# illini-robomaster/irmv_detection

Hardware: AMD Instinct MI355X
Metric: end-to-end FPS (preprocess→NMS→PnP) 640×640 YOLOv8n, 1/2/4/8 MI355X (higher is better)
Workload: dtype f16

## Files before the change

### include/irmv_hip.h

```cpp
#ifndef IRMV_HIP_H
#define IRMV_HIP_H

#include <stddef.h>
#include <stdint.h>

#ifdef __cplusplus
extern "C" {
#endif

#define IRMV_OK 0
#define IRMV_ERR_ARG (-1)
#define IRMV_ERR_HIP (-2)
#define IRMV_ERR_MODEL (-3)

#define IRMV_RESIZE_STRETCH 0
#define IRMV_RESIZE_LETTERBOX 1

#define IRMV_ARMOR_SMALL 0
#define IRMV_ARMOR_LARGE 1

#define IRMV_POINTS_AUTO 0
#define IRMV_POINTS_KEYPOINT_HEAD 1
#define IRMV_POINTS_CLASSICAL 2

// ... 100 lines not shown
int irmv_engine_num_streams(const irmv_engine *e);
int irmv_engine_sync_launch(const irmv_engine *e);

int irmv_engine_numa_node(const irmv_engine *e);
int irmv_engine_numa_placed(const irmv_engine *e);
int irmv_numa_device_node(int device, int *node);
int irmv_numa_bind_thread(int node);
int irmv_numa_page_node(const void *p);
int irmv_numa_parse_cpulist(const char *s, int *cpus, int cap);

uint8_t *irmv_engine_src_buffer(irmv_engine *e, int slot);
void *irmv_engine_src_device_buffer(irmv_engine *e, int slot);
int irmv_engine_set_window(irmv_engine *e, int slot, int x0, int y0);
int irmv_engine_get_window(const irmv_engine *e, int slot, int *x0, int *y0, int *w, int *h);
typedef struct irmv_window_map_t {
    int32_t bx0, by0;
    uint64_t band_offset;
    uint64_t band_bytes;
    double cx, cy;
    int32_t reserved[4];
} irmv_window_map_t;
int irmv_window_map(const irmv_engine_cfg *cfg, int x0, int y0, irmv_window_map_t *out);

int irmv_engine_src_format(const irmv_engine *e);
size_t irmv_engine_src_bytes(const irmv_engine *e);

#define IRMV_SUBMIT_H2D 1u
#define IRMV_SUBMIT_ASYNC_UPLOAD 2u

int irmv_engine_submit(irmv_engine *e, int first_slot, int count, uint32_t flags);
int irmv_engine_wait(irmv_engine *e);
int irmv_engine_wait_upload(irmv_engine *e, int first_slot, int count);
int irmv_engine_wait_slots(irmv_engine *e, int first_slot, int count);
int irmv_engine_results(irmv_engine *e, int slot, irmv_det *out, int cap, int *n);
int irmv_engine_detect(irmv_engine *e, int slot, irmv_det *out, int cap, int *n);
double irmv_engine_last_detect_ms(const irmv_engine *e);

int irmv_engine_rotated_image(irmv_engine *e, int slot, uint8_t *dst_hwc);

int irmv_engine_set_bayer_isp(irmv_engine *e, const uint16_t gain_q8[3], const uint8_t *lut);
int irmv_engine_get_bayer_isp(const irmv_engine *e, uint16_t gain_q8[3], uint8_t *lut);

int irmv_engine_extract_armors(irmv_engine *e, int slot, const float *xyxy, int n, irmv_det *out);
int irmv_engine_set_extract_params(irmv_engine *e, int binary_threshold, float light_min_ratio, float light_max_ratio,
                                   float light_max_angle, const double center_distances[4]);
int irmv_engine_point_source(const irmv_engine *e);

int irmv_engine_read_input(irmv_engine *e, int slot, float *chw);
int irmv_engine_read_head(irmv_engine *e, int slot, float *head);
int irmv_engine_write_head(irmv_engine *e, int slot, const float *head);
int irmv_engine_run_post(irmv_engine *e, int first_slot, int count);
int irmv_engine_debug_poke_candidate_counts(irmv_engine *e, int value);
int irmv_engine_debug_read_cand_bits(irmv_engine *e, int slot, uint32_t *words, int cap, int *n, int *sparse);
int irmv_engine_debug_read_head_rows(irmv_engine *e, int slot, float *rec, size_t bytes);
int irmv_engine_debug_read_head_raw(irmv_engine *e, int slot, float *head);
int irmv_engine_read_tap(irmv_engine *e, int slot, const char *name, float *nhwc, int shape[3]);
int irmv_engine_read_raw(irmv_engine *e, int slot, irmv_raw_dets *out);
int irmv_engine_num_anchors(const irmv_engine *e);
int irmv_engine_head_channels(const irmv_engine *e);
int irmv_engine_net_dims(const irmv_engine *e, int *width, int *height);

typedef struct irmv_conv_seg {
    char tensor[32];
    int32_t coff, C, shift;
} irmv_conv_seg;

typedef struct irmv_conv_op {
    int32_t op;
    char layer[32];
    int32_t ks, stride, act, out_f32, cin, cout, cout_pad;
    int32_t Hin, Win, Hout, Wout;
    irmv_conv_seg s0, s1;
    irmv_conv_seg res;
    char out_tensor[32];
    int32_t out_coff;
    int32_t out_lazy;
    int32_t fused;
    int32_t tune_fused;
    char fuse_layer[32];
    char fuse_tensor[32];
    int32_t fuse_coff, fuse_cout, fuse_cout_pad;
    int32_t reserved;
    char kname[48], kname_one[48];
} irmv_conv_op;

typedef struct irmv_conv_cand {
    char name[48];
    int32_t mt, nt, flags, ipw;
    int32_t forced, reserved;
} irmv_conv_cand;

#define IRMV_DECLINED 1

int irmv_engine_conv_ops(irmv_engine *e, irmv_conv_op *ops, int cap, int *n);
int irmv_engine_conv_candidates(irmv_engine *e, int op, int tune_count, irmv_conv_cand *cands, int cap, int *n);
#define IRMV_RUN_POISON 1u
#define IRMV_RUN_POISON_ONLY 2u
int irmv_engine_run_conv_candidate(irmv_engine *e, int op, int tune_count, int cand, int first_slot, int count, uint32_t flags);
int irmv_engine_read_tensor(irmv_engine *e, const char *name, int first_slot, int count, void *dst, size_t bytes);

typedef struct irmv_graph_op {
    int32_t op;
    char kind[16];
    char layer[48];
    char kname[48];
    irmv_conv_seg s0, s1;
// ... 81 lines not shown
```

### irmv_detection_amd/_build.py

```python
from __future__ import annotations

import os
import shutil
import subprocess

_HERE = os.path.dirname(os.path.abspath(__file__))
CSRC = os.path.join(_HERE, "csrc")
LIB_DIR = os.path.join(_HERE, "lib")
LIB_PATH = os.path.join(LIB_DIR, "libirmv_hip.so")
INCLUDE = os.path.join(os.path.dirname(_HERE), "include")

SOURCES = [
    ("k_pre.hip", []),
    ("k_bayer.hip", []),
    ("k_window.hip", []),
    ("k_front.hip", []),
    ("k_c2f.hip", []),
    ("k_bneck.hip", []),
    ("k_kpt.hip", []),
    ("k_conv.hip", []),
    ("k_post.hip", ["-ffp-contract=off"]),
    ("k_light.hip", ["-ffp-contract=off"]),
    ("k_shuffle.hip", []),
    ("k_debug.hip", []),
    ("engine.cpp", ["-x", "hip"]),
    ("engine_graph.cpp", ["-x", "hip"]),
    ("engine_tune.cpp", ["-x", "hip"]),
    ("engine_plan.cpp", ["-x", "hip"]),
    ("engine_step.cpp", ["-x", "hip"]),
    ("engine_hooks.cpp", ["-x", "hip"]),
]
COMMON = ["-O3", "-std=c++17", "-fPIC", "--offload-arch=gfx950", "-Wall", "-Wno-unused-function",
          "-mllvm", "-amdgpu-mfma-vgpr-form", "-I", INCLUDE]


def source_hash() -> str:
    import hashlib
    h = hashlib.sha256()
    names = sorted(set([s for s, _ in SOURCES] + ["irmv_common.hpp", "pnp_device.hpp", "numa.hpp", "engine_internal.hpp"]))
    for n in names:
        pth = os.path.join(CSRC, n)
        if os.path.exists(pth):
            h.update(n.encode() + b"\0" + open(pth, "rb").read())
    h.update(open(os.path.join(INCLUDE, "irmv_hip.h"), "rb").read())
    h.update(" ".join(COMMON[:-2]).encode())
    for src, extra in SOURCES:
        h.update((src + " " + " ".join(extra)).encode())
    return h.hexdigest()


def hipcc() -> str:
    for cand in (shutil.which("hipcc"), "/opt/rocm/bin/hipcc"):
        if cand and os.path.exists(cand):
            return cand
    raise RuntimeError("hipcc not found: the HIP extension cannot be built")


def _stale(target: str, deps) -> bool:
    if not os.path.exists(target):
        return True
    t = os.path.getmtime(target)
    return any(os.path.getmtime(d) > t for d in deps)


COMM_PATH = os.path.join(LIB_DIR, "libirmv_comm.so")


def build_comm(force: bool = False, verbose: bool = False) -> str:
    os.makedirs(LIB_DIR, exist_ok=True)
    src = os.path.join(CSRC, "comm.cpp")
    deps = [src, os.path.join(INCLUDE, "irmv_comm.h"), os.path.join(INCLUDE, "irmv_hip.h"), __file__]
    if force or _stale(COMM_PATH, deps):
        rocm_lib = os.path.join(os.path.dirname(os.path.dirname(os.path.realpath(hipcc()))), "lib")
        cmd = [hipcc(), "-O2", "-std=c++17", "-fPIC", "-shared", "-Wall", "-I", INCLUDE, src, "-o", COMM_PATH,
               "-L", rocm_lib, "-lrccl", "-Wl,-rpath," + rocm_lib]
        if verbose:
            print(" ".join(cmd))
        subprocess.check_call(cmd)
    return COMM_PATH


def build(force: bool = False, verbose: bool = False) -> str:
    os.makedirs(LIB_DIR, exist_ok=True)
    headers = [os.path.join(CSRC, "irmv_common.hpp"), os.path.join(CSRC, "pnp_device.hpp"), os.path.join(CSRC, "numa.hpp"), os.path.join(CSRC, "engine_internal.hpp"), os.path.join(INCLUDE, "irmv_hip.h"), __file__]
    objs = []
    cc = hipcc()
    for src, extra in SOURCES:
        sp = os.path.join(CSRC, src)
        obj = os.path.join(LIB_DIR, os.path.splitext(src)[0] + ".o")
        if force or _stale(obj, [sp] + headers):
            cmd = [cc] + COMMON + extra + os.environ.get("IRMV_EXTRA_HIPCC_FLAGS", "").split() + ["-c", sp, "-o", obj]
            if verbose:
                print(" ".join(cmd))
            subprocess.check_call(cmd)
        objs.append(obj)
    if force or _stale(LIB_PATH, objs):
        cmd = [cc, "-shared", "-fPIC", "--offload-arch=gfx950", "-o", LIB_PATH] + objs
        if verbose:
            print(" ".join(cmd))
        subprocess.check_call(cmd)
    return LIB_PATH


if __name__ == "__main__":
    print(build(force=False, verbose=True))
    print(build_comm(force=False, verbose=True))
```

### irmv_detection_amd/capi.py

```python
from __future__ import annotations

import ctypes as C
import os

from . import _build

OK, ERR_ARG, ERR_HIP, ERR_MODEL = 0, -1, -2, -3
RESIZE_STRETCH, RESIZE_LETTERBOX = 0, 1
ARMOR_SMALL, ARMOR_LARGE = 0, 1
SUBMIT_H2D = 1
SUBMIT_ASYNC_UPLOAD = 2
POINTS_AUTO, POINTS_KEYPOINT_HEAD, POINTS_CLASSICAL = 0, 1, 2
SRC_HWC8, SRC_BAYER_RGGB8, SRC_BAYER_BGGR8, SRC_BAYER_GRBG8, SRC_BAYER_GBRG8 = 0, 1, 2, 3, 4
BAYER_FORMATS = {"RGGB": SRC_BAYER_RGGB8, "BGGR": SRC_BAYER_BGGR8, "GRBG": SRC_BAYER_GRBG8, "GBRG": SRC_BAYER_GBRG8}
DEMOSAIC_BILINEAR, DEMOSAIC_MHC = 0, 1
DEMOSAIC_ALGOS = {"bilinear": DEMOSAIC_BILINEAR, "mhc": DEMOSAIC_MHC}
NUM_CLASSES = 14
MAX_DET_CAP = 256
CAND_CAP = 8192


class IrmvError(RuntimeError):
    def __init__(self, code: int, msg: str):
        super().__init__(f"irmv_hip error {code}: {msg}")
# ... 107 lines not shown


DECLINED = 1
RUN_POISON, RUN_POISON_ONLY = 1, 2


_P = C.c_void_p
SYMBOLS = [
    ("irmv_last_error", C.c_char_p, []),
    ("irmv_version", C.c_char_p, []),
    ("irmv_device_count", C.c_int, [C.POINTER(C.c_int)]),
    ("irmv_device_synchronize", C.c_int, [C.c_int]),
    ("irmv_engine_cfg_default", None, [C.POINTER(EngineCfg)]),
    ("irmv_engine_create", C.c_int, [C.POINTER(EngineCfg), C.POINTER(_P)]),
    ("irmv_engine_destroy", None, [_P]),
    ("irmv_engine_num_slots", C.c_int, [_P]),
    ("irmv_engine_max_det", C.c_int, [_P]),
    ("irmv_engine_num_streams", C.c_int, [_P]),
    ("irmv_engine_sync_launch", C.c_int, [_P]),
    ("irmv_engine_numa_node", C.c_int, [_P]),
    ("irmv_engine_numa_placed", C.c_int, [_P]),
    ("irmv_numa_device_node", C.c_int, [C.c_int, C.POINTER(C.c_int)]),
    ("irmv_numa_bind_thread", C.c_int, [C.c_int]),
    ("irmv_numa_page_node", C.c_int, [C.c_void_p]),
    ("irmv_numa_parse_cpulist", C.c_int, [C.c_char_p, C.POINTER(C.c_int), C.c_int]),
    ("irmv_engine_src_buffer", C.POINTER(C.c_uint8), [_P, C.c_int]),
    ("irmv_engine_src_device_buffer", C.c_void_p, [_P, C.c_int]),
    ("irmv_engine_set_window", C.c_int, [_P, C.c_int, C.c_int, C.c_int]),
    ("irmv_engine_get_window", C.c_int, [_P, C.c_int, C.POINTER(C.c_int), C.POINTER(C.c_int), C.POINTER(C.c_int), C.POINTER(C.c_int)]),
    ("irmv_window_map", C.c_int, [C.POINTER(EngineCfg), C.c_int, C.c_int, C.POINTER(WindowMap)]),
    ("irmv_engine_src_format", C.c_int, [_P]),
    ("irmv_engine_src_bytes", C.c_size_t, [_P]),
    ("irmv_engine_submit", C.c_int, [_P, C.c_int, C.c_int, C.c_uint32]),
    ("irmv_engine_wait", C.c_int, [_P]),
    ("irmv_engine_wait_slots", C.c_int, [_P, C.c_int, C.c_int]),
    ("irmv_engine_wait_upload", C.c_int, [_P, C.c_int, C.c_int]),
    ("irmv_engine_set_extract_params", C.c_int, [_P, C.c_int, C.c_float, C.c_float, C.c_float, C.POINTER(C.c_double)]),
    ("irmv_engine_point_source", C.c_int, [_P]),
    ("irmv_engine_results", C.c_int, [_P, C.c_int, C.POINTER(Det), C.c_int, C.POINTER(C.c_int)]),
    ("irmv_engine_detect", C.c_int, [_P, C.c_int, C.POINTER(Det), C.c_int, C.POINTER(C.c_int)]),
    ("irmv_engine_last_detect_ms", C.c_double, [_P]),
    ("irmv_engine_rotated_image", C.c_int, [_P, C.c_int, C.POINTER(C.c_uint8)]),
    ("irmv_engine_extract_armors", C.c_int, [_P, C.c_int, C.POINTER(C.c_float), C.c_int, C.POINTER(Det)]),
    ("irmv_engine_set_bayer_isp", C.c_int, [_P, C.POINTER(C.c_uint16), C.POINTER(C.c_uint8)]),
    ("irmv_engine_get_bayer_isp", C.c_int, [_P, C.POINTER(C.c_uint16), C.POINTER(C.c_uint8)]),
    ("irmv_engine_light_trace", C.c_int, [_P, C.c_int, C.POINTER(C.c_float), C.c_int, C.POINTER(LightTrace), C.POINTER(Det)]),
    ("irmv_light_limits", C.c_int, [C.POINTER(C.c_int32)]),
    ("irmv_engine_read_input", C.c_int, [_P, C.c_int, C.POINTER(C.c_float)]),
    ("irmv_engine_read_head", C.c_int, [_P, C.c_int, C.POINTER(C.c_float)]),
    ("irmv_engine_write_head", C.c_int, [_P, C.c_int, C.POINTER(C.c_float)]),
    ("irmv_engine_run_post", C.c_int, [_P, C.c_int, C.c_int]),
    ("irmv_engine_debug_poke_candidate_counts", C.c_int, [_P, C.c_int]),
    ("irmv_engine_debug_read_cand_bits", C.c_int, [_P, C.c_int, C.POINTER(C.c_uint32), C.c_int, C.POINTER(C.c_int), C.POINTER(C.c_int)]),
    ("irmv_engine_debug_read_head_rows", C.c_int, [_P, C.c_int, C.POINTER(C.c_float), C.c_size_t]),
    ("irmv_engine_debug_read_head_raw", C.c_int, [_P, C.c_int, C.POINTER(C.c_float)]),
    ("irmv_engine_read_tap", C.c_int, [_P, C.c_int, C.c_char_p, C.POINTER(C.c_float), C.POINTER(C.c_int)]),
    ("irmv_engine_read_raw", C.c_int, [_P, C.c_int, C.POINTER(RawDets)]),
    ("irmv_engine_num_anchors", C.c_int, [_P]),
    ("irmv_engine_head_channels", C.c_int, [_P]),
    ("irmv_engine_net_dims", C.c_int, [_P, C.POINTER(C.c_int), C.POINTER(C.c_int)]),
    ("irmv_engine_conv_ops", C.c_int, [_P, C.POINTER(ConvOp), C.c_int, C.POINTER(C.c_int)]),
    ("irmv_engine_conv_candidates", C.c_int, [_P, C.c_int, C.c_int, C.POINTER(ConvCand), C.c_int, C.POINTER(C.c_int)]),
    ("irmv_engine_run_conv_candidate", C.c_int, [_P, C.c_int, C.c_int, C.c_int, C.c_int, C.c_int, C.c_uint32]),
    ("irmv_engine_read_tensor", C.c_int, [_P, C.c_char_p, C.c_int, C.c_int, C.c_void_p, C.c_size_t]),
    ("irmv_engine_ops", C.c_int, [_P, C.POINTER(GraphOp), C.c_int, C.POINTER(C.c_int)]),
    ("irmv_engine_run_op", C.c_int, [_P, C.c_int, C.c_int, C.c_int, C.c_uint32]),
    ("irmv_sppf_slab", C.c_int, [C.c_int, C.c_int, C.c_int, C.c_int]),
    ("irmv_front_plan", C.c_int, [C.POINTER(EngineCfg), C.POINTER(FrontPlan)]),
    ("irmv_engine_profile", C.c_int, [_P, C.c_int, C.c_int, C.POINTER(KernelStat), C.c_int, C.POINTER(C.c_int)]),
    ("irmv_debug_lds_fill", C.c_int, [C.c_uint32]),
    ("irmv_debug_lds_probe", C.c_int, [C.c_uint32, C.c_uint32, C.POINTER(C.c_uint32), C.c_int, C.POINTER(C.c_int)]),
    ("irmv_pnp_create", C.c_int, [C.c_int, C.POINTER(C.c_double), C.POINTER(C.c_double), C.POINTER(_P)]),
    ("irmv_pnp_destroy", None, [_P]),
    ("irmv_pnp_solve", C.c_int, [_P, C.POINTER(C.c_float), C.c_int, C.c_int, C.POINTER(C.c_double),
                                 C.POINTER(C.c_double), C.POINTER(C.c_int32)]),
]

_lib = None


def lib_path() -> str:
    return os.environ.get("IRMV_LIB_PATH") or _build.LIB_PATH


def load():
    global _lib
    if _lib is None:
        path = lib_path()
        if not os.path.exists(path):
            raise IrmvError(ERR_HIP, f"{path} is missing: build the HIP extension first "
                                     "(python -m irmv_detection_amd._build); there is no CPU fallback")
        L = C.CDLL(path)
        for name, res, args in SYMBOLS:
            if os.environ.get("IRMV_LIB_PATH") and not hasattr(L, name):
                continue
            fn = getattr(L, name)
            fn.restype = res
            fn.argtypes = args
        _lib = L
    return _lib


def check(rc: int, allow=()):
    if rc != OK and rc not in allow:
        raise IrmvError(rc, load().irmv_last_error().decode(errors="replace"))
    return rc
# ... 80 lines not shown
```

### irmv_detection_amd/csrc/engine.cpp

```cpp
#include "engine_internal.hpp"

static thread_local std::string g_err;
int irmv::fail(int code, const std::string &msg) { g_err = msg; return code; }

extern "C" const char *irmv_last_error(void) { return g_err.c_str(); }
extern "C" const char *irmv_version(void)
{
    static char buf[96];
    static std::once_flag once;
    std::call_once(once, [] {
        int v = 0;
        if (hipRuntimeGetVersion(&v) != hipSuccess) v = 0;
        snprintf(buf, sizeof buf, "irmv_hip 0.3 (gfx950; HIP runtime %d)", v);
    });
    return buf;
}
extern "C" int irmv_device_synchronize(int device)
{
    HIP_TRY(hipSetDevice(device));
    HIP_TRY(hipDeviceSynchronize());
    return IRMV_OK;
}
extern "C" int irmv_device_count(int *count)
{
// ... 168 lines not shown
    cfg->src_width = 1280;
    cfg->src_height = 1024;
    cfg->net_size = 640;
    cfg->resize_mode = IRMV_RESIZE_STRETCH;
    cfg->rotate180 = 1;
    cfg->swap_rb = 0;
    cfg->score_thr = 0.25f;
    cfg->iou_thr = 0.45f;
    cfg->max_det = 100;
    cfg->pre_nms_cap = 4096;
    cfg->num_slots = 3;
    cfg->armor_size = IRMV_ARMOR_SMALL;
    const double K[9] = {957.669211, 0, 345.943891, 0, 969.127115, 284.057302, 0, 0, 1};
    const double D[5] = {-0.405274, 0.126058, -0.026939, -0.006503, 0.0};
    memcpy(cfg->camera_matrix, K, sizeof K);
    memcpy(cfg->dist_coeffs, D, sizeof D);
    cfg->point_source = IRMV_POINTS_AUTO;
    cfg->binary_threshold = 150;
    cfg->light_min_ratio = 0.1f; cfg->light_max_ratio = 0.4f; cfg->light_max_angle = 40.0f;
    cfg->armor_min_small_center_distance = 0.8; cfg->armor_max_small_center_distance = 3.2;
    cfg->armor_min_large_center_distance = 3.2; cfg->armor_max_large_center_distance = 5.5;
    cfg->src_format = IRMV_SRC_HWC8;
    cfg->bayer_gain_q8[0] = cfg->bayer_gain_q8[1] = cfg->bayer_gain_q8[2] = 256;
}

static EngineSwitches read_switches()
{
    auto set = [](const char *name) { return getenv(name) != nullptr; };
    auto starts = [](const char *name, char c) { const char *v = getenv(name); return v && v[0] == c; };
    auto off = [&](const char *name) { return starts(name, '0'); };
    auto is1 = [&](const char *name) { return starts(name, '1'); };
    EngineSwitches s;
    TuneSwitches &t = s.tune;
    t.untuned = off("IRMV_AUTOTUNE"); t.verbose = set("IRMV_AUTOTUNE_VERBOSE"); t.warn = set("IRMV_TUNE_WARN");
    const char *s2 = getenv("IRMV_FORCE_S2"), *wres = getenv("IRMV_FORCE_WRES");
    t.has_s2 = s2 != nullptr; t.force_s2 = s2 ? s2 : "";
    t.has_wres = wres != nullptr; t.force_wres = wres ? wres : "";
    t.force_pw = set("IRMV_FORCE_PW"); t.force_pwn = set("IRMV_FORCE_PWN"); t.force_cm = set("IRMV_FORCE_CM");
    t.force_w8 = set("IRMV_FORCE_W8"); t.force_nt8 = set("IRMV_FORCE_NT8"); t.force_pf4 = set("IRMV_FORCE_PF4");
    t.no_pw = set("IRMV_NO_PW"); t.no_pwn = set("IRMV_NO_PWN"); t.no_pf2 = set("IRMV_NO_PF2"); t.no_pf4 = set("IRMV_NO_PF4");
    t.no_cm = set("IRMV_NO_CM"); t.no_w8 = set("IRMV_NO_W8"); t.no_nt8 = set("IRMV_NO_NT8"); t.no_wres = set("IRMV_NO_WRES");
    t.no_deep = is1("IRMV_NO_DEEP");
    s.front.fastx = !off("IRMV_FRONT_FASTX"); s.front.direct = !off("IRMV_FRONT_DIRECT"); s.front.tall = !off("IRMV_FRONT_TILE8");
    s.fused_front = !off("IRMV_FUSED_FRONT"); s.fused_c2f = !off("IRMV_FUSED_C2F"); s.bneck64 = !off("IRMV_BNECK64"); s.kpt3 = !off("IRMV_KPT3");
    s.fused_head = !off("IRMV_FUSED_HEAD");
    s.merge_head0 = off("IRMV_MERGE_HEAD0") ? 0 : (is1("IRMV_MERGE_HEAD0") ? 1 : -1);
    s.group_head = !off("IRMV_GROUP_HEAD"); s.group_verbose = set("IRMV_GROUP_VERBOSE"); s.group_force = set("IRMV_GROUP_FORCE");
    if (const char *ns = getenv("IRMV_STREAMS")) { s.has_streams = true; s.streams = atoi(ns); }
    s.numa = !off("IRMV_NUMA");
    s.inline_copies = is1("IRMV_INLINE_COPIES"); s.graph_upload = !off("IRMV_GRAPH_UPLOAD"); s.window_upload = !off("IRMV_WINDOW_UPLOAD");
    if (const char *uk = getenv("IRMV_UPLOAD_KERNEL")) s.upload_kernel_blocks = atoi(uk);
    s.sync_launch = starts("IRMV_SYNC_LAUNCH", 'e') ? 1 : (starts("IRMV_SYNC_LAUNCH", 'g') ? 0 : -1);
    s.split_scan = !off("IRMV_SPLIT_SCAN"); s.emit_scan = !off("IRMV_EMIT_SCAN");
    s.sparse_head = !off("IRMV_SPARSE_HEAD"); s.sparse_branch = !off("IRMV_SPARSE_BRANCH");
    s.zero_copy_results = !off("IRMV_ZERO_COPY_RESULTS"); s.post_keys_only = is1("IRMV_POST_KEYS_ONLY");
    s.nms_classwalk = !off("IRMV_NMS_CLASSWALK");
    s.nms_prefilter = off("IRMV_NMS_PREFILTER") ? 0 : 1;
    if (const char *pe = getenv("IRMV_NMS_PRE")) { int hi = 0, lo = 0; if (sscanf(pe, "%d,%d", &hi, &lo) == 2 && hi >= 64 && hi <= 512 && lo >= 32 && lo < hi) s.nms_prefilter = hi | (lo << 16); }
    if (const char *st = getenv("IRMV_NMS_STAMPS")) { s.nms_stamps = true; s.nms_stamps_slots = atoi(st); }
    return s;
}

constexpr size_t kCfgSizeV1 = offsetof(irmv_engine_cfg, src_format);
constexpr size_t kCfgSizeV2 = offsetof(irmv_engine_cfg, reserved2);
static_assert(offsetof(irmv_engine_cfg, net_height) < kCfgSizeV2 && kCfgSizeV2 < sizeof(irmv_engine_cfg), "three distinct cfg sizes");
static_assert(offsetof(irmv_engine_cfg, win_width) == offsetof(irmv_engine_cfg, reserved2) + 4 && offsetof(irmv_engine_cfg, win_height) + 2 == sizeof(irmv_engine_cfg),
              "win_width / win_height fill the tail of irmv_engine_cfg");

static irmv_engine_cfg window_view(const irmv_engine_cfg &c)
{
    irmv_engine_cfg v = c;
    if (c.win_width > 0 && c.win_height > 0) { v.src_width = c.win_width; v.src_height = c.win_height; }
    v.win_width = v.win_height = 0;
    return v;
}

static int resolve_cfg(const irmv_engine_cfg *cfg_in, irmv_engine_cfg *full)
{
    const size_t sz = cfg_in->struct_size;
    if (sz != sizeof(irmv_engine_cfg) && sz != kCfgSizeV1 && sz != kCfgSizeV2) return fail(IRMV_ERR_ARG, "irmv_engine_cfg size mismatch");
    if (sz != sizeof(irmv_engine_cfg)) {
        irmv_engine_cfg_default(full);
        memcpy(full, cfg_in, sz == kCfgSizeV1 ? kCfgSizeV1 : offsetof(irmv_engine_cfg, net_height));
        full->struct_size = sizeof *full;
        full->bayer_demosaic = IRMV_DEMOSAIC_BILINEAR;
    } else {
        *full = *cfg_in;
    }
    const irmv_engine_cfg *cfg = full;
    if (cfg->src_format < IRMV_SRC_HWC8 || cfg->src_format > IRMV_SRC_BAYER_GBRG8) return fail(IRMV_ERR_ARG, "unknown src_format (IRMV_SRC_*)");
    if (cfg->bayer_demosaic > IRMV_DEMOSAIC_MHC) return fail(IRMV_ERR_ARG, "unknown bayer_demosaic (IRMV_DEMOSAIC_*)");
    if (cfg->bayer_demosaic == IRMV_DEMOSAIC_MHC) {
        if (cfg->src_format == IRMV_SRC_HWC8) return fail(IRMV_ERR_ARG, "bayer_demosaic = IRMV_DEMOSAIC_MHC needs a Bayer src_format (IRMV_SRC_BAYER_*8)");
        if (cfg->src_width < 4 || cfg->src_height < 4) return fail(IRMV_ERR_ARG, "bayer_demosaic = IRMV_DEMOSAIC_MHC needs src_width >= 4 and src_height >= 4 (reflect-101 at radius 2)");
    }
    if (cfg->src_format != IRMV_SRC_HWC8) {
        if (cfg->src_width % 2 || cfg->src_height % 2) return fail(IRMV_ERR_ARG, "a Bayer src_format (IRMV_SRC_BAYER_*8) needs an even src_width and src_height");
        for (int i = 0; i < 3; i++)
            if (cfg->bayer_gain_q8[i] > 1023) return fail(IRMV_ERR_ARG, "bayer_gain_q8 must be in [0, 1023] (Q8, 256 = 1.0)");
    }
    if (cfg->net_size < 64 || cfg->net_size % 32 != 0 || cfg->net_size > 2048) return fail(IRMV_ERR_ARG, "net_size must be a multiple of 32 in [64, 2048]");
    if (cfg->net_height != 0 && (cfg->net_height < 64 || cfg->net_height % 32 != 0 || cfg->net_height > 2048))
        return fail(IRMV_ERR_ARG, "net_height must be 0 (square) or a multiple of 32 in [64, 2048]");
    if (cfg->src_width < 2 || cfg->src_height < 2 || cfg->src_width > 4096) return fail(IRMV_ERR_ARG, "src size out of range (width <= 4096)");
    if ((uint64_t)cfg->src_width * (uint64_t)cfg->src_height * 3u > IRMV_MAX_FRAME_BYTES)
        return fail(IRMV_ERR_ARG, "src frame too large: 3 * src_width * src_height must not exceed 4294967296 bytes (32-bit byte offsets into a frame)");
    if (cfg->win_width < 0 || cfg->win_width > cfg->src_width) return fail(IRMV_ERR_ARG, "win_width must be 0 (no window) or in [1, src_width]");
// ... 319 lines not shown
```

### irmv_detection_amd/csrc/engine_graph.cpp

```cpp
#include "engine_internal.hpp"

#pragma pack(push, 1)
struct BlobHeader { char magic[4]; uint32_t version, nc, nk, reg_max, n_layers, dtype, reserved; };
struct BlobLayer { char name[32]; uint32_t cin, cout, k, stride, act, pad; uint64_t w_off, b_off; };
#pragma pack(pop)

static uint16_t float_to_half_bits(float f)
{
    uint32_t x;
    memcpy(&x, &f, 4);
    const uint32_t sign = (x >> 16) & 0x8000u;
    x &= 0x7fffffffu;
    if (x >= 0x7f800000u) return (uint16_t)(sign | 0x7c00u | ((x > 0x7f800000u) ? 0x200u : 0u));
    if (x >= 0x477ff000u) return (uint16_t)(sign | 0x7c00u);
    if (x < 0x33000001u) return (uint16_t)sign;
    if (x < 0x38800000u) {
        const int shift = 126 - (int)(x >> 23);
        const uint32_t man = (x & 0x7fffffu) | 0x800000u;
        uint32_t h = man >> shift;
        const uint32_t rem = man & ((1u << shift) - 1u), half = 1u << (shift - 1);
        if (rem > half || (rem == half && (h & 1u))) h++;
        return (uint16_t)(sign | h);
    }
    uint32_t h = ((x >> 23) - 112u) << 10 | ((x >> 13) & 0x3ffu);
// ... 614 lines not shown
            m.cin = PC[i]; m.cout = cm; m.k = 3; m.stride = 1; m.act = 1;
            m.w = e->merged_w.back().data(); m.b = e->merged_b.back().data();
            e->layers.push_back(m);
            TRY(new_tensor(e, "22.s0." + std::to_string(i), PH[i], PW[i], cm, false, &t_s0[i]));
            TRY(add_conv(e, m.name, SegRef{P[i], 0, PC[i], 0}, SegRef{}, PH[i], PW[i], t_s0[i], 0));
            Op &mo = e->ops.back();
            const double real = nbr == 3 ? 144.0 : 128.0;
            mo.flops *= real / cm;
            mo.level = i;
        }
    }
    for (int b = 0; b < nbr; b++)
        for (int i = 0; i < 3; i++) {
            const std::string pre = std::string("model.22.") + br[b] + "." + std::to_string(i);
            const std::string tn = std::string("22.") + br[b] + "." + std::to_string(i);
            int t1 = -1, t2;
            TRY(new_tensor(e, tn + ".1", PH[i], PW[i], mid[b], false, &t2));
            if (e->merge_head0) {
                TRY(add_conv(e, pre + ".1", SegRef{t_s0[i], coff0[b], mid[b], 0}, SegRef{}, PH[i], PW[i], t2, 0));
            } else {
                TRY(new_tensor(e, tn + ".0", PH[i], PW[i], mid[b], false, &t1));
                TRY(add_conv(e, pre + ".0", SegRef{P[i], 0, PC[i], 0}, SegRef{}, PH[i], PW[i], t1, 0));
                TRY(add_conv(e, pre + ".1", SegRef{t1, 0, mid[b], 0}, SegRef{}, PH[i], PW[i], t2, 0));
            }
            TRY(add_conv(e, pre + ".2", SegRef{t2, 0, mid[b], 0}, SegRef{}, PH[i], PW[i], e->head_t[i], off[b]));
            for (size_t k = e->ops.size() - (e->merge_head0 ? 2 : 3); k < e->ops.size(); k++) e->ops[k].level = i;
            {
                const int i1 = (int)e->ops.size() - 2, i2 = i1 + 1;
                const Op &o1 = e->ops[i1], &o2 = e->ops[i2];
                if (e->sw.fused_head && o1.cout == 64 && o1.cin % 32 == 0 && o1.pair && o1.res_t < 0 && o1.cfg.stride == 1 &&
                    o2.cin == 64 && o2.ksteps == 2 && o2.cfg.ks == 1 && o2.cfg.out_f32 && o2.cfg.act == 0 && (o2.cout_pad == 16 || o2.cout_pad == 64))
                    e->ops[i1].fuse_next = i2;
                if (e->sw.fused_head && o1.cfg.cin16 && o1.cout_pad == 16 && !o1.pair && o1.res_t < 0 && o1.cfg.stride == 1 && o1.cfg.act == 1 && o2.w_k16)
                    e->ops[i1].fuse_next = i2;
            }
            if (b == 2 && !e->merge_head0) TRY(fuse_kpt3(e, i));
        }
    return IRMV_OK;
}

static int build_post_stage(irmv_engine *e)
{
    const irmv_engine_cfg &c = e->cfg;
    const int net_w = c.net_size, net_h = c.net_height, S = c.num_slots;
    const int px = e->front.box[0], py = e->front.box[2], nw = e->front.box[1] - px, nh = e->front.box[3] - py;
    TRY(dev_alloc(e, (void **)&e->boxes, (size_t)S * e->A * 16));
    TRY(dev_alloc(e, (void **)&e->keys, (size_t)S * e->A * e->nc * 8));
    if (e->sw.split_scan) {
        TRY(dev_alloc(e, (void **)&e->cand_counts, (size_t)S * sizeof(int)));
        HIP_TRY(hipMemset(e->cand_counts, 0, (size_t)S * sizeof(int)));
        e->cand_words = (e->A + 31) / 32;
        TRY(dev_alloc(e, (void **)&e->cand_bits, (size_t)S * e->cand_words * sizeof(unsigned int)));
        HIP_TRY(hipMemset(e->cand_bits, 0, (size_t)S * e->cand_words * sizeof(unsigned int)));
    }
    e->head_stale.assign((size_t)S, 0);
    e->branch_stale.assign((size_t)S, 0);
    TRY(dev_alloc(e, (void **)&e->dets_dev, (size_t)S * c.max_det * sizeof(DevDet)));
    TRY(dev_alloc(e, (void **)&e->fout_dev, (size_t)S * sizeof(DevFrameOut)));
    HIP_TRY(hipMemset(e->dets_dev, 0, (size_t)S * c.max_det * sizeof(DevDet)));
    HIP_TRY(hipMemset(e->fout_dev, 0, (size_t)S * sizeof(DevFrameOut)));
    HIP_TRY(hipHostMalloc((void **)&e->dets_host, (size_t)S * c.max_det * sizeof(DevDet), hipHostMallocMapped | hipHostMallocCoherent));
    HIP_TRY(hipHostMalloc((void **)&e->fout_host, (size_t)S * sizeof(DevFrameOut), hipHostMallocMapped | hipHostMallocCoherent));
    HIP_TRY(hipHostGetDevicePointer((void **)&e->dets_host_dev, e->dets_host, 0));
    HIP_TRY(hipHostGetDevicePointer((void **)&e->fout_host_dev, e->fout_host, 0));
    log_range(e, "pinned dets_host", e->dets_host, (size_t)S * c.max_det * sizeof(DevDet));
    log_range(e, "pinned fout_host", e->fout_host, (size_t)S * sizeof(DevFrameOut));
    memset(e->dets_host, 0, (size_t)S * c.max_det * sizeof(DevDet));
    memset(e->fout_host, 0, (size_t)S * sizeof(DevFrameOut));
    if (e->sw.split_scan) {
        Op op; op.kind = OP_SCAN; op.layer = "scan_decode"; snprintf(op.kname, sizeof op.kname, "scan_decode");
        op.bytes = (double)e->A * 64.0; e->ops.push_back(op);
    }
    { Op op; op.kind = OP_NMS; op.layer = "decode_nms_kpt_pnp"; snprintf(op.kname, sizeof op.kname, "nms_pnp");
      op.bytes = (double)e->A * 64.0; e->ops.push_back(op); }
    if (c.point_source == IRMV_POINTS_KEYPOINT_HEAD && e->nk < 8) return fail(IRMV_ERR_MODEL, "point_source = keypoint head, but the model has none");
    e->classical = c.point_source == IRMV_POINTS_CLASSICAL || (c.point_source == IRMV_POINTS_AUTO && e->nk < 8);
    e->zero_copy_results = !e->classical && e->sw.zero_copy_results;
    if (e->classical) {
        Op op; op.kind = OP_LIGHT; op.layer = "extract_armors"; snprintf(op.kname, sizeof op.kname, "light_extract");
        e->ops.push_back(op);
    }
    const size_t SL = e->classical ? (size_t)S : 1;
    e->light_pool = std::max<size_t>((size_t)8 * c.src_width * c.src_height, (size_t)(c.src_width + 2) * (c.src_height + 2) + 16);
    TRY(dev_alloc(e, (void **)&e->light_labels, SL * e->light_pool));
    TRY(dev_alloc(e, (void **)&e->light_points, SL * c.max_det * kLightPointsCap * 2 * sizeof(short)));
    TRY(dev_alloc(e, (void **)&e->light_hulls, SL * c.max_det * kLightPointsCap * 4 * sizeof(short)));
    TRY(dev_alloc(e, (void **)&e->light_boxes, (size_t)c.max_det * 16));
    TRY(dev_alloc(e, (void **)&e->light_dets_dev, (size_t)c.max_det * sizeof(DevDet)));
    HIP_TRY(hipHostMalloc((void **)&e->light_dets_host, (size_t)c.max_det * sizeof(DevDet), hipHostMallocDefault));
    log_range(e, "pinned light_dets", e->light_dets_host, (size_t)c.max_det * sizeof(DevDet));

    PostArgs &p = e->post;
    p.net_w = net_w; p.net_h = net_h; p.A = e->A; p.nc = e->nc; p.nk = e->nk;
    p.logit_thr = (float)std::log((double)c.score_thr / (1.0 - (double)c.score_thr));
    p.iou_thr = c.iou_thr;
    p.max_det = c.max_det;
    p.pre_nms_cap = c.pre_nms_cap;
    p.classwalk = e->sw.nms_classwalk ? 1 : 0;
    p.prefilter = e->sw.nms_prefilter;
    if (c.resize_mode == IRMV_RESIZE_STRETCH) {
        p.scale_x = (float)c.src_width / (float)net_w;
        p.scale_y = (float)c.src_height / (float)net_h;
        p.off_x = p.off_y = 0.f;
    } else {
        p.scale_x = (float)c.src_width / (float)nw;
        p.scale_y = (float)c.src_height / (float)nh;
// ... 115 lines not shown
```

### irmv_detection_amd/csrc/engine_hooks.cpp

```cpp
#include "engine_internal.hpp"

static float half_bits_to_float(uint16_t h)
{
    const uint32_t sign = ((uint32_t)h & 0x8000u) << 16;
    uint32_t exp = (h >> 10) & 0x1fu, man = h & 0x3ffu, x;
    if (exp == 0) {
        if (man == 0) x = sign;
        else {
            int e = -1;
            do { e++; man <<= 1; } while (!(man & 0x400u));
            x = sign | ((uint32_t)(112 - e) << 23) | ((man & 0x3ffu) << 13);
        }
    } else if (exp == 31) x = sign | 0x7f800000u | (man << 13);
    else x = sign | ((exp + 112u) << 23) | (man << 13);
    float f;
    memcpy(&f, &x, 4);
    return f;
}

extern "C" int irmv_engine_debug_poke_candidate_counts(irmv_engine *e, int value)
{
    if (!e) return fail(IRMV_ERR_ARG, "engine is null");
    if (!e->cand_counts) return fail(IRMV_ERR_ARG, "this engine keeps no candidate counters");
    TRY(irmv_engine_wait(e));
    HIP_TRY(hipSetDevice(e->cfg.device));
    std::vector<int> v((size_t)e->cfg.num_slots, value);
    HIP_TRY(hipMemcpy(e->cand_counts, v.data(), v.size() * sizeof(int), hipMemcpyHostToDevice));
    return IRMV_OK;
}

extern "C" int irmv_engine_debug_read_cand_bits(irmv_engine *e, int slot, uint32_t *words, int cap, int *n, int *sparse)
{
    TRY(check_range(e, slot, 1));
    if (!n || !sparse) return fail(IRMV_ERR_ARG, "n / sparse is null");
    *sparse = e->sparse_head ? 1 : 0;
    *n = e->sparse_head ? e->cand_words : 0;
    if (!words || *n == 0) return IRMV_OK;
    if (cap < *n) return fail(IRMV_ERR_ARG, "read_cand_bits: buffer too small");
    TRY(irmv_engine_wait(e));
    HIP_TRY(hipSetDevice(e->cfg.device));
    HIP_TRY(hipMemcpy(words, e->cand_bits + (size_t)slot * e->cand_words, (size_t)e->cand_words * sizeof(unsigned int), hipMemcpyDeviceToHost));
    return IRMV_OK;
}

extern "C" int irmv_engine_rotated_image(irmv_engine *e, int slot, uint8_t *dst)
{
    TRY(check_range(e, slot, 1));
    if (!dst) return fail(IRMV_ERR_ARG, "dst is null");
    HIP_TRY(hipSetDevice(e->cfg.device));
    TRY(load_frame(e, slot, e->stream));
    launch_rotate180(e->src_dev + (size_t)slot * e->frame_bytes, e->rot_dev, e->cfg.src_width, e->cfg.src_height, e->stream);
    HIP_TRY(hipMemcpyAsync(dst, e->rot_dev, e->frame_bytes, hipMemcpyDeviceToHost, e->stream));
    HIP_TRY(hipStreamSynchronize(e->stream));
    return IRMV_OK;
}

static_assert(sizeof(irmv_light_rec) == sizeof(LightTraceRec) && sizeof(irmv_light_trace) == sizeof(LightTrace) &&
                  offsetof(irmv_light_trace, starts) == offsetof(LightTrace, starts) && offsetof(irmv_light_trace, points) == offsetof(LightTrace, points) &&
                  offsetof(irmv_light_trace, recs) == offsetof(LightTrace, recs) && offsetof(irmv_light_rec, length) == offsetof(LightTraceRec, length) &&
                  IRMV_LIGHT_MAX_CONTOURS == kLightMaxContours && IRMV_LIGHT_POINTS_CAP == kLightPointsCap,
              "irmv_light_trace is LightTrace");

static int extract_armors(irmv_engine *e, int slot, const float *xyxy, int n, irmv_light_trace *trace, irmv_det *out)
{
    TRY(check_range(e, slot, 1));
    if (n < 0 || n > e->cfg.max_det || (n > 0 && (!xyxy || !out))) return fail(IRMV_ERR_ARG, "n must be 0..max_det with xyxy/out set");
    if (n == 0) return IRMV_OK;
    HIP_TRY(hipSetDevice(e->cfg.device));
    TRY(irmv_engine_wait(e));
    hipStream_t st = e->stream;
    if (trace && !e->light_trace_dev) TRY(dev_alloc(e, (void **)&e->light_trace_dev, (size_t)e->cfg.max_det * sizeof(LightTrace)));
    if (trace) HIP_TRY(hipMemsetAsync(e->light_trace_dev, 0, (size_t)n * sizeof(LightTrace), st));
    TRY(load_frame(e, slot, st));
    const float ox = e->window ? (float)e->win_org[slot].x : 0.f, oy = e->window ? (float)e->win_org[slot].y : 0.f;
    std::vector<float> local;
    if (e->window) {
        local.assign(xyxy, xyxy + (size_t)n * 4);
        for (size_t j = 0; j < local.size(); j++) local[j] -= (j & 1) ? oy : ox;
        HIP_TRY(hipMemcpyAsync(e->light_boxes, local.data(), (size_t)n * 16, hipMemcpyHostToDevice, st));
        HIP_TRY(hipStreamSynchronize(st));
    } else {
        HIP_TRY(hipMemcpyAsync(e->light_boxes, xyxy, (size_t)n * 16, hipMemcpyHostToDevice, st));
    }
    LightArgs a = light_args(e, slot);
    a.dets = e->light_dets_dev;
    a.labels = e->light_labels;
    a.points = e->light_points;
    a.hulls = e->light_hulls;
    a.num_dets = nullptr;
    a.n_boxes = n;
    a.boxes = e->light_boxes;
    a.trace = trace ? e->light_trace_dev : nullptr;
    launch_light_extract(a, n, 1, st);
    HIP_TRY(hipGetLastError());
// ... 487 lines not shown
```

### irmv_detection_amd/csrc/engine_internal.hpp

```cpp
#pragma once
#include <hip/hip_runtime.h>

#include <algorithm>
#include <chrono>
#include <cmath>
#include <cstdio>
#include <cstring>
#include <fstream>
#include <map>
#include <mutex>
#include <set>
#include <memory>
#include <string>
#include <vector>

#include "../../include/irmv_hip.h"
#include "irmv_common.hpp"
#include "numa.hpp"

using namespace irmv;

namespace irmv { int fail(int code, const std::string &msg); }
#define HIP_TRY(expr)                                                                                 \
    do {                                                                                              \
// ... 8 lines not shown
        if (_rc) return _rc; \
    } while (0)

struct LayerW {
    std::string name;
    int cin, cout, k, stride, act;
    int groups;
    const uint16_t *w;
    const float *b;
};

struct Tensor {
    std::string name;
    void *base = nullptr;
    size_t slot_elems = 0;
    int H = 0, W = 0, C = 0;
    bool f32 = false;
    size_t esize() const { return f32 ? 4 : 2; }
    void *slot(int s) const { return static_cast<char *>(base) + (size_t)s * slot_elems * esize(); }
};

struct SegRef { int t = -1, coff = 0, C = 0, shift = 0; };

struct FrontSwitches { bool fastx = true, direct = true, tall = true; };

struct TuneSwitches {
    bool untuned, verbose, warn;
    bool has_s2, has_wres;
    std::string force_s2, force_wres;
    bool force_pw, force_pwn, force_cm, force_w8, force_nt8, force_pf4;
    bool no_pw, no_pwn, no_pf2, no_pf4, no_cm, no_w8, no_nt8, no_wres, no_deep;
};

struct EngineSwitches {
    TuneSwitches tune{};
    FrontSwitches front;
    bool fused_front = true, fused_c2f = true;
    bool bneck64 = true;
    bool kpt3 = true;
    bool fused_head = true;
    int merge_head0 = -1;
    bool group_head = true;
    bool group_verbose = false;
    bool group_force = false;
    bool has_streams = false; int streams = 0;
    bool numa = true;
    bool inline_copies = false;
    bool graph_upload = true;
    int upload_kernel_blocks = 256;
    bool window_upload = true;
    int sync_launch = -1;
    bool split_scan = true;
    bool emit_scan = true, sparse_head = true, sparse_branch = true;
    bool zero_copy_results = true;
    bool post_keys_only = false;
    bool nms_classwalk = true;
    int nms_prefilter = 1;
    bool nms_stamps = false; int nms_stamps_slots = 0;
};

enum OpKind { OP_PRE, OP_CONV0, OP_CONV, OP_POOL, OP_NMS, OP_LIGHT, OP_FRONT, OP_C2F2, OP_C2F32, OP_DW, OP_SHUF, OP_SCAN, OP_BNECK, OP_KPT3, OP_DEMOSAIC, OP_CROP };

struct Op {
    OpKind kind;
    std::string layer;
    ConvCfg cfg{};
    ConvCfg cfg_one{};
    char kname_one[48] = {0};
    SegRef s0, s1;
    int Hin = 0, Win = 0, Hout = 0, Wout = 0, cin = 0, cout = 0, cout_pad = 0, ksteps = 0;
    int out_t = -1, out_coff = 0, res_t = -1, res_coff = 0;
    half_t *w_packed = nullptr;
    half_t *w_k16 = nullptr;
    half_t *w_lds[4] = {nullptr, nullptr, nullptr, nullptr};
    float *bias = nullptr;
    double flops = 0, bytes = 0;
    double w_bytes = 0;
    double out_bytes = 0;
    bool pair = false;
    int level = -1;
    char kname[48] = {0};
    int sub[4] = {-1, -1, -1, -1};
    int mode = 0;
    bool shortcut = false;
    int fuse_next = -1;
    bool fused_away = false;
    int group = -1;
    int bneck = -1;
    int kpt3 = -1;
    bool gated_first = false;
    int tune_fuse[2] = {-1, -1};
};

enum StepKind { STEP_BATCH, STEP_ONE, STEP_MATERIALIZE, STEP_POST };

struct Launch {
    int op = -1, group = -1;
    bool cfg_one = false;
    bool fused = false;
    unsigned scan = 0;
    bool keys_only = false;
    bool sparse = false;
    int gate = 0;
    bool once = false;
    std::string name, layer;
    double flops = 0, bytes = 0, launch_bytes = 0;
};

struct GraphKey {
    int first, count;
    StepKind kind;
    bool upload;
    bool operator<(const GraphKey &o) const { return std::tie(first, count, kind, upload) < std::tie(o.first, o.count, o.kind, o.upload); }
};

struct SlotGroup {
    int first = 0, count = 0;
    hipEvent_t h2d = nullptr, out = nullptr;
    hipStream_t compute = nullptr;
    bool in_flight = false;
    bool async_up = false;
};

struct irmv_engine {
    irmv_engine_cfg cfg{};
    int nc = 0, nk = 0, A = 0, no = 0;
    int backbone = 0;
    int num_cus = 256;
    int numa_node = -1;
    bool numa_placed = false;
    struct HeadGroup { std::vector<int> members; int family = 0, nt = 1; ConvCfg cfg{}; char name[48] = {0}; };
    std::vector<HeadGroup> head_groups;
    bool emit_scan = false;
    int *cand_counts = nullptr;
    bool sparse_head = false;
    unsigned int *cand_bits = nullptr;
    int cand_words = 0;
    std::vector<char> head_stale;
    bool sparse_branch = false;
    std::vector<char> branch_stale;
    int lvl_hw[3] = {0, 0, 0}, lvl_base[3] = {0, 0, 0};
    size_t frame_bytes = 0;
    size_t src_bytes = 0;
    hipStream_t stream = nullptr;
    hipStream_t extra_streams[7] = {nullptr, nullptr, nullptr, nullptr, nullptr, nullptr, nullptr};
    int num_streams = 1;
    hipStream_t h2d_stream = nullptr;
    std::map<std::pair<int, int>, SlotGroup> groups;
    std::vector<SlotGroup *> slot_owner;
    uint8_t *src_host = nullptr;
    int sync_launch = 0;
    uint8_t *src_host_dev = nullptr;
    uint8_t *src_dev = nullptr;
    uint8_t *raw_dev = nullptr;
    BayerArgs bayer{};
    uint8_t *isp_table_dev = nullptr;
    bool bayer_table = false, bayer_mhc = false;
    uint16_t isp_gain[3] = {256, 256, 256};
    uint8_t isp_lut[kBayerTableBytes] = {0};
    uint8_t *rot_dev = nullptr;
    bool window = false;
    int full_w = 0, full_h = 0;
    size_t full_bytes = 0;
    uint8_t *full_dev = nullptr;
    int2 *win_dev = nullptr;
    std::vector<int2> win_org;
    std::vector<int2> sub_org;
    PnpConst pnp_base{};
    AxisTap *tap_x = nullptr, *tap_y = nullptr;
    std::vector<Tensor> tensors;
    std::map<std::string, int> tensor_idx;
    std::vector<Op> ops;
    std::vector<Launch> plans[STEP_POST + 1];
    std::vector<void *> dev_allocs;
    int head_t[3] = {-1, -1, -1};
    float *head_all = nullptr;
    PnpConst *pnp_dev = nullptr;
    long long *dbg_dev = nullptr;
    std::set<std::string> lazy_tensors;
    bool fused_front = false;
    irmv_front_plan_t front{};
    bool classical = false;
    signed char *light_labels = nullptr;
    size_t light_pool = 0;
    short *light_points = nullptr, *light_hulls = nullptr;
    float *light_boxes = nullptr;
    DevDet *light_dets_dev = nullptr, *light_dets_host = nullptr;
    LightTrace *light_trace_dev = nullptr;
    float *boxes = nullptr;
    unsigned long long *keys = nullptr;
    DevDet *dets_dev = nullptr, *dets_host = nullptr, *dets_host_dev = nullptr;
    DevFrameOut *fout_dev = nullptr, *fout_host = nullptr, *fout_host_dev = nullptr;
    bool zero_copy_results = false;
    half_t *conv0_w = nullptr;
    float *conv0_b = nullptr;
    PostArgs post{};
    std::map<GraphKey, hipGraphExec_t> graphs;
    double last_detect_ms = 0;
    std::vector<uint8_t> blob;
    std::vector<LayerW> layers;
    std::vector<std::vector<uint16_t>> dequant;
    std::vector<std::vector<uint16_t>> merged_w;
    std::vector<std::vector<float>> merged_b;
    bool merge_head0 = false;
    EngineSwitches sw{};

    ~irmv_engine();
};

constexpr int kProfileRepeat = 4;

struct TuneEntry { int mt, nt, flags, ipw; };
struct TuneCand { ConvCfg c; bool forced; };
struct ConvView { ConvArgs a; bool want_fuse, lds_ok; };

inline int stream_share(const irmv_engine *e, int count) { return (count + e->num_streams - 1) / e->num_streams; }
inline uint8_t *upload_dev(const irmv_engine *e) { return e->raw_dev ? e->raw_dev : (e->window ? e->full_dev : e->src_dev); }
inline const char *demosaic_kname(const irmv_engine *e) { return e->bayer_mhc ? "bayer_demosaic_mhc" : (e->bayer_table ? "bayer_demosaic_lut" : "bayer_demosaic"); }
inline ConvWeights conv_weights(const Op &op) { return {op.w_packed, {op.w_lds[0], op.w_lds[1], op.w_lds[2], op.w_lds[3]}, op.w_k16}; }
inline bool run_conv(const Op &op, const ConvCfg &c, const ConvArgs &a, int count, hipStream_t s) { return launch_conv(c, a, conv_weights(op), count, s); }

namespace irmv {
void log_range(const irmv_engine *e, const char *what, const void *p, size_t bytes);
bool upload_aligned(size_t src_bytes, int first, int count);
void front_plan(const irmv_engine_cfg &c, const FrontSwitches &sw, irmv_front_plan_t *p, std::vector<AxisTap> &tx, std::vector<AxisTap> &ty);
int write_window(irmv_engine *e, int slot);
int write_isp_table(irmv_engine *e);
int dev_alloc(irmv_engine *e, void **p, size_t bytes);
int load_blob(irmv_engine *e);
int build_engine(irmv_engine *e);
TuneEntry tune_entry(const ConvCfg &c);
std::vector<TuneCand> tune_candidates(const Op &op, const ConvArgs &a, int count, bool want_fuse, bool lds_ok, const TuneSwitches &sw, int num_cus);
ConvView conv_view(const irmv_engine *e, const Op &op, int first, int count);
int autotune_convs(irmv_engine *e);
int build_head_groups(irmv_engine *e);
int choose_sync_launch(irmv_engine *e);
void finalize_head_fusion(irmv_engine *e);
void build_step_plans(irmv_engine *e);
void fill_conv_args(const irmv_engine *e, const Op &op, int first, int count, ConvArgs &a, bool fused = false);
LightArgs light_args(const irmv_engine *e, int first);
PostArgs post_args(const irmv_engine *e, int first);
bool launch_head_group(const irmv_engine *e, const irmv_engine::HeadGroup &g, int first, const PostArgs *pa, unsigned scan, hipStream_t s);
int launch_op(irmv_engine *e, const Launch &l, int first, int count, const PostArgs &pa, unsigned scan, bool crop_pinned, hipStream_t s);
int enqueue_step(irmv_engine *e, StepKind kind, int first, int count, hipStream_t s, int reps, const std::vector<hipEvent_t> *ev, bool crop_pinned = false);
void mark_stepped(irmv_engine *e, int first, int count);
int copy_out(irmv_engine *e, int first, int count, hipStream_t st = nullptr);
int check_range(const irmv_engine *e, int first, int count);
int load_frame(irmv_engine *e, int slot, hipStream_t st);
void det_pose(const irmv_engine *e, const DevDet &d, float ox, float oy, irmv_det &o);
int ensure_dense_head(irmv_engine *e, int slot);
}
```

### irmv_detection_amd/csrc/engine_plan.cpp

```cpp
#include "engine_internal.hpp"

static bool is_cls_final_carrier(const Op &op) { return op.fuse_next >= 0 && op.level >= 0 && op.layer.rfind("model.22.cv3.", 0) == 0; }

void irmv::finalize_head_fusion(irmv_engine *e)
{
    for (Op &op : e->ops) {
        if (op.fuse_next < 0) continue;
        const bool k16 = op.cfg.cin16 && !op.cfg.lds && !op.cfg_one.lds && !op.cfg.deep && !op.cfg_one.deep && op.cfg.nt == 1 && op.cfg_one.nt == 1 && e->ops[op.fuse_next].w_k16;
        const bool ok = k16 || (op.cfg.lds && op.cfg.nt == 4 && op.cfg_one.lds && op.cfg_one.nt == 4);
        if (!ok) { op.fuse_next = -1; continue; }
        e->ops[op.fuse_next].fused_away = true;
        e->lazy_tensors.insert(e->tensors[op.out_t].name);
        const size_t l = strlen(op.kname), l1 = strlen(op.kname_one);
        snprintf(op.kname + l, sizeof op.kname - l, "+1x1");
        snprintf(op.kname_one + l1, sizeof op.kname_one - l1, "+1x1");
    }
    int fused = 0;
    for (const Op &op : e->ops) fused += is_cls_final_carrier(op);
    e->emit_scan = e->sw.split_scan && fused == 3 && e->sw.emit_scan;
    e->sparse_head = e->emit_scan && e->cand_bits && e->sw.sparse_head;
    e->sparse_branch = e->sparse_head && e->sw.sparse_branch;
}

static bool is_box_final_carrier(const Op &op) { return op.fuse_next >= 0 && op.level >= 0 && op.layer.rfind("model.22.cv2.", 0) == 0; }

static void sparse_head_plan(irmv_engine *e, std::vector<Launch> &plan)
{
    int last_cls = -1;
    bool lvl_cls[3] = {false, false, false};
    for (size_t i = 0; i < plan.size(); i++)
        if (plan[i].scan && plan[i].group < 0) { last_cls = (int)i; lvl_cls[e->ops[plan[i].op].level] = true; }
    auto box_carrier = [&](const Launch &l) {
        const Op &op = e->ops[l.op];
        return l.group < 0 && l.fused && op.kind == OP_CONV && is_box_final_carrier(op) && op.level < 3 && lvl_cls[op.level];
    };
    std::vector<char> first_conv(plan.size(), 0);
    if (e->sparse_branch)
        for (size_t i = 0; i < plan.size(); i++) {
            const Launch &f = plan[i];
            const Op &fo = e->ops[f.op];
            if (f.group >= 0 || f.fused || f.scan || fo.kind != OP_CONV || !(f.cfg_one ? fo.cfg_one : fo.cfg).wr || fo.res_t >= 0) continue;
            int carrier = -1;
            for (size_t j = i + 1; j < plan.size(); j++) {
                const Op &co = e->ops[plan[j].op];
                if (box_carrier(plan[j]) && co.level == fo.level && co.s0.t == fo.out_t && co.s1.C == 0 && co.s0.coff == fo.out_coff && co.Hin == fo.Hout && co.Win == fo.Wout) carrier = plan[j].op;
            }
            bool other = false;
            for (int k = 0; k < (int)e->ops.size(); k++) {
                const Op &o = e->ops[k];
                if (k == carrier || k == f.op) continue;
                other = other || o.s0.t == fo.out_t || o.s1.t == fo.out_t || o.res_t == fo.out_t || o.out_t == fo.out_t;
            }
            first_conv[i] = carrier >= 0 && !other;
        }
    std::vector<Launch> out, moved;
    for (size_t i = 0; i < plan.size(); i++) {
        Launch &l = plan[i];
        Op &op = e->ops[l.op];
        if (l.scan) {
            if (l.group < 0) l.bytes -= e->ops[op.fuse_next].out_bytes;
            else for (size_t m = 0; m < e->head_groups[l.group].members.size(); m++)
                if (l.scan >> m & 1u) l.bytes -= e->ops[e->ops[e->head_groups[l.group].members[m]].fuse_next].out_bytes;
        }
        const bool cls_first = op.level >= 0 && op.level < 3 && lvl_cls[op.level];
        const bool box = box_carrier(l);
        const bool kpt = op.kind == OP_KPT3 && cls_first && (int)i > last_cls;
        if (box || kpt) {
            l.sparse = true;
            l.bytes -= box ? e->ops[op.fuse_next].out_bytes : op.out_bytes;
            if (e->sparse_branch) l.gate = 1;
        }
        if (first_conv[i]) {
            l.gate = 2;
            op.gated_first = true;
            e->lazy_tensors.insert(e->tensors[op.out_t].name);
        }
        if ((box || first_conv[i]) && (int)i < last_cls) moved.push_back(l); else out.push_back(l);
        if ((int)i == last_cls) { out.insert(out.end(), moved.begin(), moved.end()); moved.clear(); }
    }
    plan.swap(out);
}

void irmv::build_step_plans(irmv_engine *e)
{
    for (int k = STEP_BATCH; k <= STEP_POST; k++) {
        const bool one = k == STEP_ONE, mat = k == STEP_MATERIALIZE, post = k == STEP_POST, step = !mat && !post;
        auto emits = [&](const Op &op) { return step && e->emit_scan && is_cls_final_carrier(op); };
        for (int i = 0; i < (int)e->ops.size(); i++) {
            const Op &op = e->ops[i];
            if (post && op.kind != OP_NMS && op.kind != OP_LIGHT && op.kind != OP_SCAN) continue;
            if (op.kind == OP_SCAN && e->emit_scan && !post) continue;
            const bool grouped = one && op.kind == OP_CONV && op.group >= 0;
            if (grouped && e->head_groups[op.group].members[0] != i) continue;
            const bool bneck = one && e->sw.bneck64;
            if (op.kind == OP_BNECK ? !bneck : (op.bneck >= 0 && bneck)) continue;
            if (op.kind == OP_KPT3 ? !step : (op.kpt3 >= 0 && step)) continue;
            if (mat ? !(op.fused_away || op.fuse_next >= 0 || op.gated_first || ((op.bneck >= 0 || op.kpt3 >= 0) && op.kind == OP_CONV)) : op.fused_away) continue;
            Launch l; l.op = i;
            l.once = op.kind == OP_LIGHT || (e->sw.split_scan && (op.kind == OP_SCAN || op.kind == OP_NMS));
            l.keys_only = op.kind == OP_NMS && ((e->emit_scan && !post) || (post && e->sw.post_keys_only));
            l.layer = op.layer;
            if (grouped) {
                const irmv_engine::HeadGroup &g = e->head_groups[op.group];
                l.group = op.group;
                l.name = g.name;
                l.layer += " ... (" + std::to_string(g.members.size()) + " convs)";
                for (size_t m = 0; m < g.members.size(); m++) {
                    const Op &mo = e->ops[g.members[m]];
                    if (emits(mo)) l.scan |= 1u << m;
                    l.flops += mo.flops + (mo.fuse_next >= 0 ? e->ops[mo.fuse_next].flops : 0.0);
                    l.bytes += mo.bytes;
                }
            } else {
                l.cfg_one = op.kind == OP_CONV && (one || mat) && stream_share(e, e->cfg.num_slots) > 1;
                l.fused = !mat && op.fuse_next >= 0;
                l.scan = emits(op) ? 1u : 0u;
                l.name = l.cfg_one ? op.kname_one : op.kname;
                const Op *nx = l.fused ? &e->ops[op.fuse_next] : nullptr;
                l.flops = op.flops + (nx ? nx->flops : 0.0);
                l.launch_bytes = op.w_bytes + (nx ? nx->w_bytes : 0.0);
                l.bytes = op.bytes + (nx ? nx->out_bytes - op.out_bytes + nx->w_bytes : 0.0) - l.launch_bytes;
            }
            e->plans[k].push_back(l);
        }
        if (step && e->sparse_head) sparse_head_plan(e, e->plans[k]);
    }
}
```

### irmv_detection_amd/csrc/engine_step.cpp

```cpp
#include "engine_internal.hpp"

void irmv::fill_conv_args(const irmv_engine *e, const Op &op, int first, int count, ConvArgs &a, bool fused)
{
    a = ConvArgs{};
    auto seg = [&](const SegRef &s) {
        ConvSeg cs{nullptr, 0, 0, 0};
        if (s.t < 0 || s.C == 0) return cs;
        const Tensor &t = e->tensors[s.t];
        cs.p = static_cast<const half_t *>(t.slot(first)) + s.coff;
        cs.ld = t.C;
        cs.C = s.C;
        cs.shift = s.shift;
        return cs;
    };
    a.s0 = seg(op.s0);
    a.s1 = seg(op.s1);
    a.Hin = op.Hin; a.Win = op.Win; a.Hout = op.Hout; a.Wout = op.Wout;
    a.M = count * op.Hout * op.Wout;
    a.Cin = op.cin;
    a.w = op.w_packed;
    a.bias = op.bias;
    const Tensor &ot = e->tensors[op.out_t];
    a.out = static_cast<char *>(ot.slot(first)) + (size_t)op.out_coff * ot.esize();
    a.out_ld = ot.C;
// ... 26 lines not shown
    const irmv_engine_cfg &c = e->cfg;
    a.frames = e->src_dev + (size_t)first * e->frame_bytes;
    a.frame_bytes = e->frame_bytes;
    a.cols = c.src_width; a.rows = c.src_height; a.rotate180 = c.rotate180;
    a.dets = e->dets_dev + (size_t)first * c.max_det;
    a.max_det = c.max_det;
    a.num_dets = reinterpret_cast<const int *>(e->fout_dev + first);
    a.num_dets_stride = (int)(sizeof(DevFrameOut) / sizeof(int));
    a.n_boxes = 0;
    a.boxes = nullptr;
    a.labels = e->light_labels + (size_t)first * e->light_pool;
    a.label_pool = e->light_pool;
    a.points = e->light_points + (size_t)first * c.max_det * kLightPointsCap * 2;
    a.points_cap = kLightPointsCap;
    a.hulls = e->light_hulls + (size_t)first * c.max_det * kLightPointsCap * 4;
    a.binary_threshold = c.binary_threshold;
    a.light_min_ratio = c.light_min_ratio; a.light_max_ratio = c.light_max_ratio; a.light_max_angle = c.light_max_angle;
    a.min_small_cd = c.armor_min_small_center_distance; a.max_small_cd = c.armor_max_small_center_distance;
    a.min_large_cd = c.armor_min_large_center_distance; a.max_large_cd = c.armor_max_large_center_distance;
    a.pnp = e->pnp_dev;
    a.first = first; a.pnp_stride = e->post.pnp_stride;
    a.pnp_armor_size = c.armor_size;
    return a;
}

static BayerArgs bayer_args(const irmv_engine *e, int first)
{
    BayerArgs a = e->bayer;
    a.raw = e->raw_dev + (size_t)first * e->src_bytes; a.dst = (e->window ? e->full_dev : e->src_dev) + (size_t)first * e->full_bytes;
    return a;
}

static void launch_bayer(const irmv_engine *e, int first, int count, hipStream_t s)
{
    if (e->bayer_table) launch_demosaic_table(bayer_args(e, first), e->isp_table_dev, e->bayer_mhc, count, s);
    else launch_demosaic(bayer_args(e, first), count, s);
}

PostArgs irmv::post_args(const irmv_engine *e, int first)
{
    PostArgs p = e->post;
    p.head_all = e->head_all;
    p.slots_total = e->cfg.num_slots;
    p.first = first;
    p.boxes = e->boxes + (size_t)first * e->A * 4;
    p.keys = e->keys + (size_t)first * e->A * e->nc;
    p.key_cap = e->A * e->nc;
    p.dets = (e->zero_copy_results ? e->dets_host_dev : e->dets_dev) + (size_t)first * e->cfg.max_det;
    p.fout = (e->zero_copy_results ? e->fout_host_dev : e->fout_dev) + first;
    if (p.dbg) p.dbg += (size_t)first * 16;
    p.counts = e->sw.split_scan ? e->cand_counts + first : nullptr;
    p.cand_bits = e->sparse_head ? e->cand_bits + (size_t)first * e->cand_words : nullptr;
    p.cand_words = e->cand_words;
    return p;
}

static CropArgs crop_args(const irmv_engine *e, int first, bool pinned)
{
    CropArgs a{};
    a.src = pinned ? e->src_host_dev : e->full_dev; a.src_slot_bytes = e->full_bytes;
    a.dst = e->src_dev; a.dst_slot_bytes = e->frame_bytes;
    a.win = e->win_dev; a.first = first;
    a.full_w = e->full_w; a.full_h = e->full_h; a.win_w = e->cfg.src_width; a.win_h = e->cfg.src_height;
    return a;
}

static void launch_crop(const irmv_engine *e, int first, int count, bool pinned, hipStream_t s) { launch_window_crop(crop_args(e, first, pinned), count, s); }

static PreArgs pre_args(const irmv_engine *e, const Op &op, int first)
{
    PreArgs a;
    a.src = e->src_dev + (size_t)first * e->frame_bytes;
    a.dst = static_cast<half_t *>(e->tensors[op.out_t].slot(first));
    a.tx = e->tap_x; a.ty = e->tap_y;
    a.sw = e->cfg.src_width; a.sh = e->cfg.src_height; a.net_w = e->cfg.net_size; a.net_h = e->cfg.net_height; a.swap_rb = e->cfg.swap_rb;
    a.src_slot_bytes = e->frame_bytes;
    return a;
}

static FrontArgs front_args(const irmv_engine *e, const Op &op, int first)
{
    FrontArgs a;
    a.src = e->src_dev + (size_t)first * e->frame_bytes;
    a.src_slot_bytes = e->frame_bytes;
    a.tx = e->tap_x; a.ty = e->tap_y;
    a.vx0 = e->front.box[0]; a.vx1 = e->front.box[1]; a.vy0 = e->front.box[2]; a.vy1 = e->front.box[3];
    a.sw = e->cfg.src_width; a.sh = e->cfg.src_height; a.net_w = e->cfg.net_size; a.net_h = e->cfg.net_height; a.swap_rb = e->cfg.swap_rb;
    a.fastx = e->front.fastx; a.fx_i0 = e->front.fx_i0; a.fx_step = e->front.fx_step;
    a.w0 = e->conv0_w; a.b0 = e->conv0_b;
    a.w1 = op.w_packed; a.b1 = op.bias;
    const Tensor &ot = e->tensors[op.out_t];
    a.out = static_cast<half_t *>(ot.slot(first));
    a.out_ld = ot.C;
    a.tiles_x = e->front.tiles_x; a.tiles_y = e->front.tiles_y; a.tile_y = e->front.tile_y; a.stage_bytes = e->front.stage_bytes;
    return a;
}

static C2fArgs c2f2_args(const irmv_engine *e, const Op &op, int first)
{
    C2fArgs a;
    const Tensor &xt = e->tensors[op.s0.t], &ot = e->tensors[op.out_t];
    a.x = static_cast<const half_t *>(xt.slot(first)); a.x_ld = xt.C;
    a.out = static_cast<half_t *>(ot.slot(first)); a.out_ld = ot.C;
    a.H = xt.H; a.W = xt.W;
    a.tiles_x = (xt.W + kC2fTile - 1) / kC2fTile; a.tiles_y = (xt.H + kC2fTile - 1) / kC2fTile;
    const Op &c1 = e->ops[op.sub[0]], &m1 = e->ops[op.sub[1]], &m2 = e->ops[op.sub[2]], &c2 = e->ops[op.sub[3]];
    a.w_cv1 = c1.w_packed; a.w_m1 = m1.w_packed; a.w_m2 = m2.w_packed; a.w_cv2 = c2.w_packed;
    a.b_cv1 = c1.bias; a.b_m1 = m1.bias; a.b_m2 = m2.bias; a.b_cv2 = c2.bias;
    return a;
}

static C2f32Args c2f32_args(const irmv_engine *e, const Op &op, int first, int count)
{
    C2f32Args a{};
    const Tensor &ct = e->tensors[op.res_t];
    const Tensor &ot = e->tensors[op.out_t];
    if (op.sub[0] >= 0) {
        ConvArgs ca;
        fill_conv_args(e, e->ops[op.sub[0]], first, count, ca, false);
        a.s0 = ca.s0; a.s1 = ca.s1; a.cin1 = ca.Cin;
        a.w_cv1 = e->ops[op.sub[0]].w_packed; a.b_cv1 = e->ops[op.sub[0]].bias;
    } else {
        a.cin1 = 32;
    }
    a.cat = static_cast<half_t *>(ct.slot(first)); a.cat_ld = ct.C; a.prev_coff = 64;
    a.out = static_cast<half_t *>(ot.slot(first)); a.out_ld = ot.C;
    a.H = op.Hin; a.W = op.Win;
    a.tiles_x = (op.Win + kC2f32TileW - 1) / kC2f32TileW; a.tiles_y = (op.Hin + kC2f32TileH - 1) / kC2f32TileH;
    a.w_m1 = e->ops[op.sub[1]].w_packed; a.b_m1 = e->ops[op.sub[1]].bias;
    a.w_m2 = e->ops[op.sub[2]].w_packed; a.b_m2 = e->ops[op.sub[2]].bias;
    if (op.sub[3] >= 0) { a.w_cv2 = e->ops[op.sub[3]].w_packed; a.b_cv2 = e->ops[op.sub[3]].bias; }
    return a;
}

static BneckArgs bneck_args(const irmv_engine *e, const Op &op, int first)
{
    const Op &m1 = e->ops[op.sub[0]], &m2 = e->ops[op.sub[1]];
    const Tensor &ct = e->tensors[op.res_t];
    BneckArgs a{};
    a.yin = static_cast<const half_t *>(ct.slot(first)) + m1.s0.coff; a.yin_ld = ct.C;
    a.ynext = static_cast<half_t *>(ct.slot(first)) + m2.out_coff; a.ynext_ld = ct.C;
    a.cat = static_cast<const half_t *>(ct.slot(first)); a.cat_ld = ct.C;
    a.H = op.Hin; a.W = op.Win;
    a.tiles_x = (op.Win + kBneckTile - 1) / kBneckTile; a.tiles_y = (op.Hin + kBneckTile - 1) / kBneckTile;
    a.w_m1 = m1.w_lds[0]; a.b_m1 = m1.bias; a.w_m2 = m2.w_lds[0]; a.b_m2 = m2.bias;
    if (op.sub[2] >= 0) {
        const Op &c2 = e->ops[op.sub[2]];
        const Tensor &ot = e->tensors[c2.out_t];
        a.out = static_cast<half_t *>(ot.slot(first)) + c2.out_coff; a.out_ld = ot.C;
        a.w_cv2 = c2.w_packed; a.b_cv2 = c2.bias;
    }
    return a;
}

static Kpt3Args kpt3_args(const irmv_engine *e, const Op &op, const Launch &l, int first, const PostArgs &pa)
{
    const Op &o0 = e->ops[op.sub[0]], &o1 = e->ops[op.sub[1]], &o2 = e->ops[op.sub[2]];
    const Tensor &xt = e->tensors[o0.s0.t], &ht = e->tensors[o2.out_t];
    Kpt3Args a{};
    a.x = static_cast<const half_t *>(xt.slot(first)) + o0.s0.coff; a.x_ld = xt.C;
    a.H = op.Hin; a.W = op.Win;
    a.tiles_x = (op.Win + kKpt3Tile - 1) / kKpt3Tile; a.tiles_y = (op.Hin + kKpt3Tile - 1) / kKpt3Tile;
    a.w1 = o0.w_lds[0]; a.b1 = o0.bias;
    a.w2 = o1.w_packed; a.b2 = o1.bias;
    a.w3 = o2.w_k16; a.b3 = o2.bias;
    a.out = static_cast<float *>(ht.slot(first)) + o2.out_coff; a.out_ld = ht.C;
    if (l.sparse) { a.cand_bits = pa.cand_bits; a.cand_words = pa.cand_words; a.abase = e->lvl_base[op.level]; a.tile_gate = l.gate; }
    return a;
}

static DwArgs dw_args(const irmv_engine *e, const Op &op, int first)
{
    DwArgs a;
    const Tensor &xt = e->tensors[op.s0.t], &ot = e->tensors[op.out_t];
    a.x = static_cast<const half_t *>(xt.slot(first)) + op.s0.coff; a.x_ld = xt.C;
    a.y = static_cast<half_t *>(ot.slot(first)) + op.out_coff; a.y_ld = ot.C;
    a.w = op.w_packed; a.b = op.bias;
    a.Hin = op.Hin; a.Win = op.Win; a.Hout = op.Hout; a.Wout = op.Wout; a.C = op.cout; a.stride = op.cfg.stride;
    return a;
}

static ShufArgs shuf_args(const irmv_engine *e, const Op &op, int first, int count)
{
    ShufArgs a;
    const Tensor &at = e->tensors[op.s0.t], &bt = e->tensors[op.s1.t], &ot = e->tensors[op.out_t];
    a.a = static_cast<const half_t *>(at.slot(first)) + op.s0.coff; a.a_ld = at.C;
    a.b = static_cast<const half_t *>(bt.slot(first)) + op.s1.coff; a.b_ld = bt.C;
    a.out = static_cast<half_t *>(ot.slot(first)); a.out_ld = ot.C;
    a.bc = op.s0.C;
    a.pixels = (size_t)count * op.Hin * op.Win;
    return a;
}

static Conv0Args conv0_args(const irmv_engine *e, const Op &op, int first, int count)
{
    Conv0Args a;
    a.x = static_cast<const half_t *>(e->tensors[op.s0.t].slot(first));
    a.y = static_cast<half_t *>(e->tensors[op.out_t].slot(first));
    a.w = e->conv0_w; a.b = e->conv0_b; a.net_w = e->cfg.net_size; a.net_h = e->cfg.net_height; a.batch = count;
    return a;
}


static void scan_args_for(const irmv_engine *e, const Op &op, const PostArgs &pa, ConvArgs &a)
{
    a.scan_keys = pa.keys; a.scan_counts = pa.counts; a.scan_thr = pa.logit_thr; a.scan_nc = pa.nc;
    a.scan_key_cap = pa.key_cap;
    a.scan_abase = e->lvl_base[op.level];
    a.cand_bits = pa.cand_bits; a.cand_words = pa.cand_words;
}

bool irmv::launch_head_group(const irmv_engine *e, const irmv_engine::HeadGroup &g, int first, const PostArgs *pa, unsigned scan, hipStream_t s)
{
    ConvArgs a[kMultiMax];
    ConvWeights w[kMultiMax];
    const int n = (int)g.members.size();
    for (int k = 0; k < n; k++) {
        const Op &op = e->ops[g.members[k]];
        fill_conv_args(e, op, first, 1, a[k], true);
        if (scan >> k & 1u) scan_args_for(e, op, *pa, a[k]);
        w[k] = conv_weights(op);
    }
    return g.family == 0 ? launch_conv_lds_multi(g.nt, a, w, n, 1, s) : launch_conv_direct_multi(g.cfg, a, n, s);
}

int irmv::launch_op(irmv_engine *e, const Launch &l, int first, int count, const PostArgs &pa, unsigned scan, bool crop_pinned, hipStream_t s)
{
    const Op &op = e->ops[l.op];
    switch (op.kind) {
    case OP_DEMOSAIC: launch_bayer(e, first, count, s); break;
    case OP_CROP: launch_crop(e, first, count, crop_pinned, s); break;
    case OP_PRE: launch_preprocess(pre_args(e, op, first), count, s); break;
    case OP_FRONT: if (!launch_front(front_args(e, op, first), count, s)) return fail(IRMV_ERR_HIP, "fused front kernel: LDS request refused"); break;
    case OP_C2F2: launch_c2f2(c2f2_args(e, op, first), count, s); break;
    case OP_C2F32: if (!launch_c2f32(op.mode, op.shortcut, c2f32_args(e, op, first, count), count, s)) return fail(IRMV_ERR_ARG, "no fused C2f kernel for " + op.layer); break;
    case OP_BNECK:
        if (!launch_bneck64(op.mode, op.sub[2] >= 0 ? e->ops[op.sub[2]].ksteps : 6, op.shortcut, bneck_args(e, op, first), count, s)) return fail(IRMV_ERR_ARG, "no fused bottleneck kernel for " + op.layer);
        break;
    case OP_KPT3: if (!launch_kpt3(kpt3_args(e, op, l, first, pa), op.cin, count, s)) return fail(IRMV_ERR_ARG, "no fused keypoint-branch kernel for " + op.layer); break;
    case OP_DW: launch_dwconv3x3(dw_args(e, op, first), count, s); break;
    case OP_SHUF: launch_shuffle_cat(shuf_args(e, op, first, count), s); break;
    case OP_CONV0: launch_conv0(conv0_args(e, op, first, count), s); break;
    case OP_POOL: { const Tensor &t = e->tensors[op.out_t]; launch_sppf_pool(static_cast<half_t *>(t.slot(first)), count, t.H, t.W, t.C / 4, s); break; }
    case OP_CONV: {
        if (l.group >= 0) {
            if (!launch_head_group(e, e->head_groups[l.group], first, &pa, scan, s)) return fail(IRMV_ERR_ARG, "grouped launch refused: " + l.name);
            break;
        }
        ConvArgs a;
        fill_conv_args(e, op, first, count, a, l.fused);
        if (scan) scan_args_for(e, op, pa, a);
        if (l.sparse || l.gate) { a.cand_bits = pa.cand_bits; a.cand_words = pa.cand_words; a.scan_abase = e->lvl_base[op.level]; a.tile_gate = l.gate; }
        if (!run_conv(op, l.cfg_one ? op.cfg_one : op.cfg, a, count, s)) return fail(IRMV_ERR_ARG, std::string("no conv kernel for ") + op.kname + " (" + op.layer + ")");
        break;
    }
    case OP_SCAN: launch_scan_decode(pa, count, s); break;
    case OP_NMS: { PostArgs pn = pa; pn.keys_only = l.keys_only ? 1 : 0; launch_nms_pnp(pn, count, s); break; }
    case OP_LIGHT: launch_light_extract(light_args(e, first), e->cfg.max_det, count, s); break;
    }
    HIP_TRY(hipGetLastError());
    return IRMV_OK;
}

int irmv::enqueue_step(irmv_engine *e, StepKind kind, int first, int count, hipStream_t s, int reps, const std::vector<hipEvent_t> *ev, bool crop_pinned)
{
    const std::vector<Launch> &plan = e->plans[kind];
    const PostArgs pa = post_args(e, first);
    PostArgs mute = pa;
    mute.logit_thr = INFINITY;
    for (size_t i = 0; i < plan.size(); i++) {
        const Launch &l = plan[i];
        if (ev) HIP_TRY(hipEventRecord((*ev)[2 * i], s));
        const int n = l.once ? 1 : reps;
        for (int rep = 0; rep < n; rep++) {
            const bool last = rep == n - 1, muted = !last && l.scan && e->sparse_head;
            TRY(launch_op(e, l, first, count, muted ? mute : pa, last || muted ? l.scan : 0u, crop_pinned, s));
        }
        if (ev) HIP_TRY(hipEventRecord((*ev)[2 * i + 1], s));
    }
    return IRMV_OK;
}

void irmv::mark_stepped(irmv_engine *e, int first, int count)
{
    if (e->sparse_head) std::fill(e->head_stale.begin() + first, e->head_stale.begin() + first + count, 1);
    if (e->sparse_branch) std::fill(e->branch_stale.begin() + first, e->branch_stale.begin() + first + count, 1);
    if (e->window) std::copy(e->win_org.begin() + first, e->win_org.begin() + first + count, e->sub_org.begin() + first);
}

constexpr int kBandUploadMaxSlots = 8;
static int copy_in(irmv_engine *e, int first, int count, hipStream_t st, bool bands = false)
{
    if (bands && e->window && !e->raw_dev && count <= kBandUploadMaxSlots) {
        const size_t pitch = (size_t)e->full_w * 3, len = (size_t)e->cfg.src_height * pitch;
        for (int s = first; s < first + count; s++) {
            const int by0 = e->cfg.rotate180 ? e->full_h - e->win_org[s].y - e->cfg.src_height : e->win_org[s].y;
            const size_t off = (size_t)s * e->src_bytes + (size_t)by0 * pitch;
            HIP_TRY(hipMemcpyAsync(e->full_dev + off, e->src_host + off, len, hipMemcpyHostToDevice, st));
        }
        return IRMV_OK;
    }
    HIP_TRY(hipMemcpyAsync(upload_dev(e) + (size_t)first * e->src_bytes, e->src_host + (size_t)first * e->src_bytes,
                           e->src_bytes * count, hipMemcpyHostToDevice, st));
    return IRMV_OK;
}
// ... 241 lines not shown
```

### irmv_detection_amd/csrc/irmv_common.hpp

```cpp
#pragma once

#include <hip/hip_runtime.h>

#include <cstdint>
#include <cstdlib>

namespace irmv {

typedef _Float16 half_t;
typedef _Float16 half8 __attribute__((ext_vector_type(8)));
typedef _Float16 half4 __attribute__((ext_vector_type(4)));
typedef float f32x4 __attribute__((ext_vector_type(4)));

constexpr float kActScale = 1.44269504088896341f;
constexpr float kActUnscale = 0.693147180559945309f;
typedef unsigned int u32x4_t __attribute__((ext_vector_type(4)));
__device__ __forceinline__ float silu_rcp(float y) { return __builtin_amdgcn_rcpf(1.0f + __builtin_amdgcn_exp2f(-y)); }
__device__ __forceinline__ unsigned int silu_pack2(float y0, float y1)
{
    const float r0 = silu_rcp(y0), r1 = silu_rcp(y1);
    unsigned int o;
    asm("v_fma_mixlo_f16 %0, %1, %2, 0" : "=v"(o) : "v"(y0), "v"(r0));
    asm("v_fma_mixhi_f16 %0, %1, %2, 0" : "+v"(o) : "v"(y1), "v"(r1));
    return o;
}
__device__ __forceinline__ half8 silu_pack8(float y0, float y1, float y2, float y3, float y4, float y5, float y6, float y7)
{
    return __builtin_bit_cast(half8, (u32x4_t){silu_pack2(y0, y1), silu_pack2(y2, y3), silu_pack2(y4, y5), silu_pack2(y6, y7)});
}
__device__ __forceinline__ half4 silu_pack4(float y0, float y1, float y2, float y3)
{
    typedef unsigned int u32x2_t __attribute__((ext_vector_type(2)));
    return __builtin_bit_cast(half4, (u32x2_t){silu_pack2(y0, y1), silu_pack2(y2, y3)});
}
__device__ __forceinline__ void mfma_operand_fence(half4 &x) { asm volatile("s_nop 1" : "+v"(x)); }
__device__ __forceinline__ void mfma_operand_fence(half8 &x, half8 &y) { asm volatile("s_nop 1" : "+v"(x), "+v"(y)); }
__device__ __forceinline__ half_t silu_add_res(float y, float res)
{
    float p = y * silu_rcp(y);
    asm("" : "+v"(p));
    float s = p + res;
    asm("" : "+v"(s));
    return (half_t)s;
}

__device__ __forceinline__ void tile_image(int id, int tiles, int batch, int xcd, int &tile, int &image)
{
    const int full = xcd ? (batch >> 3) * 8 * tiles : 0;
    if (id < full) {
        const int j = id >> 3;
        image = (j / tiles) * 8 + (id & 7);
        tile = j % tiles;
    } else {
        const int r = id - full;
        image = (full / tiles) + r / tiles;
        tile = r % tiles;
    }
}

inline int xcd_image_order()
{
    const char *v = getenv("IRMV_XCD_IMAGES");
    return (v && v[0] == '0') ? 0 : 1;
}

inline int wres_stagger()
{
    const char *v = getenv("IRMV_WRES_STAGGER");
    return (v && v[0] == '0') ? 0 : 1;
}

constexpr int kHeadRec = 96;
constexpr int kClsOff = 64;
constexpr int kKptOff = 80;
constexpr int kCandCap = 8192;
constexpr int kMaxDetCap = 256;

struct AxisTap { int32_t i0, i1, w1, pad; };

struct PreArgs {
    const uint8_t *src;
    half_t *dst;
    const AxisTap *tx, *ty;
    int sw, sh, net_w, net_h, swap_rb;
    size_t src_slot_bytes;
};
void launch_preprocess(const PreArgs &a, int batch, hipStream_t s);
void launch_rotate180(const uint8_t *src, uint8_t *dst, int sw, int sh, hipStream_t s);
void launch_upload_frames(const uint8_t *src_host_mapped, uint8_t *dst, size_t bytes, int blocks, hipStream_t s);

constexpr int kBayerBandRows = 8;
constexpr int kBayerTableBytes = 3 * 256;
struct BayerArgs {
    const uint8_t *raw;
    uint8_t *dst;
    size_t raw_slot_bytes, dst_slot_bytes;
    int W, H;
    int ry, rx;
    uint32_t gain[3];
};
void launch_demosaic(const BayerArgs &a, int batch, hipStream_t s);
void launch_demosaic_table(const BayerArgs &a, const uint8_t *table, bool mhc, int batch, hipStream_t s);

struct CropArgs {
    const uint8_t *src;
    uint8_t *dst;
    size_t src_slot_bytes, dst_slot_bytes;
    const int2 *win;
    int first;
    int full_w, full_h, win_w, win_h;
// ... 71 lines not shown
    int shift;
};

constexpr int kC2f32TileH = 8, kC2f32TileW = 16;
struct C2f32Args {
    ConvSeg s0, s1;
    int cin1;
    half_t *cat;
    int cat_ld, prev_coff;
    half_t *out;
    int out_ld;
    int H, W, tiles_x, tiles_y;
    const half_t *w_cv1, *w_m1, *w_m2, *w_cv2;
    const float *b_cv1, *b_m1, *b_m2, *b_cv2;
};
size_t c2f32_lds_bytes(int mode);
bool launch_c2f32(int mode, bool shortcut, const C2f32Args &a, int batch, hipStream_t s);

constexpr int kBneckTile = 8;
struct BneckArgs {
    const half_t *yin;
    int yin_ld;
    half_t *ynext;
    int ynext_ld;
    const half_t *cat;
    int cat_ld;
    half_t *out;
    int out_ld;
    int H, W, tiles_x, tiles_y;
    const half_t *w_m1, *w_m2;
    const float *b_m1, *b_m2;
    const half_t *w_cv2;
    const float *b_cv2;
};
size_t bneck64_lds_bytes(int mode, int ks2);
bool launch_bneck64(int mode, int ks2, bool shortcut, const BneckArgs &a, int batch, hipStream_t s);

constexpr int kKpt3Tile = 10;
struct Kpt3Args {
    const half_t *x;
    int x_ld;
    int H, W, tiles_x, tiles_y;
    const half_t *w1;
    const float *b1;
    const half_t *w2;
    const float *b2;
    const half_t *w3;
    const float *b3;
    float *out;
    int out_ld;
    const unsigned int *cand_bits;
    int cand_words, abase;
    int tile_gate;
};
bool kpt3_eligible(int cin);
bool launch_kpt3(const Kpt3Args &a, int cin, int batch, hipStream_t s);

struct ConvArgs {
    ConvSeg s0, s1;
    int Hin, Win;
    int Hout, Wout;
    int M;
    int Cin;
    const half_t *w;
    const float *bias;
    void *out;
    int out_ld;
    const half_t *res;
    int res_ld;
    int cout_pad;
    int ksteps;
    int pair;
    const half_t *w2;
    const float *bias2;
    float *out2;
    int out2_ld, n2;
    unsigned long long *scan_keys;
    int *scan_counts;
    float scan_thr;
    int scan_nc, scan_abase, scan_key_cap;
    unsigned int *cand_bits;
    int cand_words;
    int tile_gate;
};

constexpr int kMultiMax = 6;
struct LdsMember {
    ConvArgs a;
    const half_t *wl;
    int tiles_x, tiles_y, twc_log2, patch_bytes, batch, tile2d;
    int gx, gy;
};
struct LdsMultiArgs {
    int n;
    int start[kMultiMax + 1];
    LdsMember m[kMultiMax];
};
struct DirectMultiArgs {
    int n;
    int start[kMultiMax + 1], gx[kMultiMax], gy[kMultiMax];
    ConvArgs a[kMultiMax];
};

struct ConvCfg {
    int ks, stride, mt, nt; bool cin16; int act; bool out_f32; bool lds; int ipw;
    bool deep;
    bool ct;
    bool pw;
    bool pf2;
    bool pf4;
    bool w8;
    int cm;
    bool wr;
    bool pp;
};
struct ConvWeights { const half_t *w_packed; const half_t *w_lds[4]; const half_t *w_k16; };
struct ConvLaunch;
bool resolve_conv(const ConvCfg &cfg, const ConvArgs &a, const ConvWeights &w, int batch, ConvLaunch *out = nullptr);
bool launch_conv(const ConvCfg &cfg, const ConvArgs &a, const ConvWeights &w, int batch, hipStream_t s);
const char *conv_cfg_name(const ConvCfg &cfg, char *buf, int n);
bool conv_pw_eligible(const ConvCfg &cfg, const ConvArgs &a);
bool conv_lds_fits(const ConvArgs &a, const ConvWeights &w, int stride, int mt, int nt);
int conv_wres_tiles(const ConvArgs &a, int stride, bool pp);
bool launch_conv_lds_multi(int nt, const ConvArgs *a, const ConvWeights *w, int n, int batch, hipStream_t s);
bool launch_conv_direct_multi(const ConvCfg &cfg, const ConvArgs *a, int n, hipStream_t s);

void launch_sppf_pool(half_t *buf, int batch, int H, int W, int C, hipStream_t s);
int sppf_slab(int batch, int H, int W, int C);

struct DevDet {
    float box_net[4];
    float xyxy[4];
    float score;
    int32_t cls, anchor, pnp_ok;
    float kpts_net[8];
    float kpts[8];
    double rvec[3], tvec[3], quat[4];
    int32_t armor_valid;
    int32_t armor_size;
    int32_t n_lights;
    int32_t pad_;
};
struct DevFrameOut { int32_t num_dets, n_candidates, overflow, pad; };

struct PnpConst {
    double fx, fy, cx, cy, k1, k2, p1, p2, k3;
    double hy[2], hz[2];
};

struct PostArgs {
    const float *head_all;
    int slots_total, first;
    float *boxes;
    unsigned long long *keys;
    int key_cap;
    DevDet *dets;
    DevFrameOut *fout;
    int net_w, net_h, A, nc, nk;
    float logit_thr, iou_thr;
    int max_det, pre_nms_cap;
    float scale_x, scale_y, off_x, off_y;
    int armor_size;
    const PnpConst *pnp;
    long long *dbg;
    int keys_only;
    int prefilter;
    int classwalk;
    int *counts;
    unsigned int *cand_bits;
    int cand_words;
    int pnp_stride;
};
void launch_nms_pnp(const PostArgs &a, int batch, hipStream_t s);
constexpr int kScanBlocks = 16;
constexpr size_t kScanLdsMax = 159 * 1024;
void launch_scan_decode(const PostArgs &a, int batch, hipStream_t s);
constexpr int kLightLdsPoints = 256;
constexpr int kLightLdsImage = 40 * 1024;
constexpr int kLightMaxContours = 1024;
constexpr int kLightPointsCap = 4096;

struct LightTraceRec {
    float corners[8];
    float top[2], bottom[2], center[2];
    double length;
    int32_t measured, ok, hull_edges, in_lds;
};
struct LightTrace {
    int32_t n_contours, n_found, n_points, too_large;
    int32_t pool_fit, in_lds, rx, ry, rw, rh;
    int32_t max_contours, points_cap, lds_image, lds_points;
    uint64_t label_pool, pool_offset;
    int32_t starts[kLightMaxContours + 1];
    int16_t points[kLightPointsCap][2];
    int32_t pad_;
    LightTraceRec recs[kLightMaxContours];
};

struct LightArgs {
    const uint8_t *frames;
    size_t frame_bytes;
    int cols, rows, rotate180;
    DevDet *dets;
    int max_det;
    const int *num_dets;
    int num_dets_stride, n_boxes;
    const float *boxes;
    signed char *labels;
    size_t label_pool;
    short *points;
    int points_cap;
    short *hulls;
    int binary_threshold;
    float light_min_ratio, light_max_ratio, light_max_angle;
    double min_small_cd, max_small_cd, min_large_cd, max_large_cd;
    const PnpConst *pnp;
    int pnp_armor_size;
    LightTrace *trace;
    int first, pnp_stride;
};
void launch_light_extract(const LightArgs &a, int n_boxes_max, int batch, hipStream_t s);

constexpr int kDebugLdsWords = 160 * 1024 / 4;
// ... 9 lines not shown
```

### irmv_detection_amd/csrc/k_conv.hip

```cpp
#include "irmv_common.hpp"

#include <algorithm>
#include <cstdio>
#include <cstring>
#include <iterator>
#include <mutex>
#include <type_traits>

namespace irmv {

template <int MT, int NT>
struct PrefetchDepth { static constexpr int value = (MT * NT >= 8) ? 2 : ((MT * NT >= 4) ? 3 : 4); };
template <int MT, int NT>
struct DeepPrefetchDepth { static constexpr int value = (MT + NT <= 2) ? 12 : ((MT + NT <= 3) ? 10 : 6); };


template <int KS, int STRIDE, int MT, int NT, bool CIN16, int ACT, bool OUT_F32, bool CT = false, bool DEEP = false>
__device__ __forceinline__ void conv_mfma_body(const ConvArgs &a, int wg_x, int wg_y, int grid_x, int grid_y)
{
    constexpr int PAD = KS / 2;
    constexpr int PF = DEEP ? DeepPrefetchDepth<MT, NT>::value : PrefetchDepth<MT, NT>::value;
    static_assert(!CT || (KS == 3 && !CIN16), "chunk-major order is the 3x3 LDS family's");
    const int lane = threadIdx.x & 63, wave = threadIdx.x >> 6;
    const int g = lane >> 4, r = lane & 15;
// ... 585 lines not shown
}

template <int KS, int NBW>
static void launch_pwn_inst(const ConvLaunch &l, hipStream_t s)
{
    static unsigned long long attr_done = 0;
    static int per_cu[64], cus[64];
    const ConvArgs &a = l.a;
    const size_t lds = l.g.bytes;
    int dev = 0;
    (void)hipGetDevice(&dev);
    dev &= 63;
    once_per_device(attr_done, [lds, dev] {
        (void)hipFuncSetAttribute(reinterpret_cast<const void *>(conv1x1_pwn_kernel<KS, NBW>), hipFuncAttributeMaxDynamicSharedMemorySize, 160 * 1024);
        int nb = 0, nc = 0;
        per_cu[dev] = 1; cus[dev] = 256;
        if (hipOccupancyMaxActiveBlocksPerMultiprocessor(&nb, reinterpret_cast<const void *>(conv1x1_pwn_kernel<KS, NBW>), 512, lds) == hipSuccess && nb >= 1) per_cu[dev] = nb > 2 ? 2 : nb;
        if (hipDeviceGetAttribute(&nc, hipDeviceAttributeMultiprocessorCount, dev) == hipSuccess && nc > 0) cus[dev] = nc;
    });
    const int groups = a.cout_pad / 64 / NBW;
    const int units = (a.M + 15) / 16;
    int wg = (cus[dev] * per_cu[dev] + groups - 1) / groups;
    if (wg > (units + 7) / 8) wg = (units + 7) / 8;
    if (wg < 1) wg = 1;
    hipLaunchKernelGGL((conv1x1_pwn_kernel<KS, NBW>), dim3(wg, groups), dim3(512), lds, s, a, wg);
}

static constexpr struct { int ksteps, nbw; ConvLauncher launch; } k_pw[] = {
    {4, 1, launch_pw_inst<4>}, {6, 1, launch_pw_inst<6>}, {8, 1, launch_pw_inst<8>}, {12, 1, launch_pw_inst<12>}, {16, 1, launch_pw_inst<16>},
    {4, 2, launch_pwn_inst<4, 2>}, {6, 2, launch_pwn_inst<6, 2>}, {8, 2, launch_pwn_inst<8, 2>}, {12, 2, launch_pwn_inst<12, 2>}, {16, 2, launch_pwn_inst<16, 2>},
    {4, 4, launch_pwn_inst<4, 4>}, {6, 4, launch_pwn_inst<6, 4>}, {8, 4, launch_pwn_inst<8, 4>},
};

static ConvLauncher pick_pw(const ConvCfg &c, const ConvArgs &a, LdsGeom &g)
{
    const int nbw = c.ipw > 1 ? c.ipw : 1;
    if (!conv_pw_eligible(c, a) || a.cout_pad % (64 * nbw) != 0) return nullptr;
    for (const auto &v : k_pw)
        if (v.ksteps == a.ksteps && v.nbw == nbw) {
            g.bytes = (size_t)nbw * 4 * a.ksteps * 1024 + (nbw > 1 ? (size_t)nbw * 64 * 4 : 0);
            return v.launch;
        }
    return nullptr;
}

constexpr int lds_pmax(int stride, int mt, bool tile2d, int wr = 0, int pf = 0)
{
    return pf == 2 ? (stride == 1 ? 4 : 8) : (wr ? 4 : ((tile2d && stride == 1) ? (mt == 4 ? 8 : 4) : 12));
}

#ifndef IRMV_LDS_WAVES
#define IRMV_LDS_WAVES 2
#endif
template <int STRIDE, int MT, int NT, bool TILE2D, int N2, int PF = 0, int CM = 0, int NWV = 4, int WR = 0, bool PP = false>
__device__ __forceinline__ void conv3x3_lds_body(const ConvArgs &a, const half_t *wl, int tiles_x, int tiles_y, int twc_log2, int a_patch_bytes, int ipw, int batch,
                                                 int wg_x, int wg_y, int grid_x, int grid_y, int stagger = 0)
{
    extern __shared__ __attribute__((aligned(16))) unsigned char smem[];
    const int lane = threadIdx.x & 63, wave = threadIdx.x >> 6, tid = threadIdx.x;
    constexpr bool PF2 = PF != 0;
    constexpr int NPF = PF == 2 ? 4 : (PF == 1 ? 2 : 1);
    constexpr int NTH = 64 * NWV;
    static_assert(!PP || (WR > 0 && NWV % 2 == 0), "ping-pong groups share resident weights");
    constexpr int NWP = PP ? NWV / 2 : NWV;
    constexpr int NTP = 64 * NWP;
    const int sub = PP ? wave / NWP : 0, wv = wave - sub * NWP, tidp = tid - sub * NTP;
    const int g = lane >> 4, r = lane & 15;
    const int bx = wg_x, by = wg_y;
    (void)grid_x; (void)grid_y;
    const int wg_tiles = PP ? (tiles_x * tiles_y + 1) / 2 : tiles_x * tiles_y;
    const int grp = bx / wg_tiles;
    int tile = PP ? 2 * (bx - grp * wg_tiles) + sub : bx - grp * wg_tiles;
    const bool active = tile < tiles_x * tiles_y;
    if (!active) tile = 0;
    const int img = grp * ipw, nimg = min(ipw, batch - img);
    const int nblk = by;
    const int HWo = a.Hout * a.Wout;
    bool gated = false;
    unsigned int l_mask = 0u;
    int l_pos = 0;
    int n_mine = nimg, n_max = nimg;
    if constexpr (WR > 0) {
        auto gate_images = [&](int t) -> unsigned int {
            const int h = a.tile_gate - 1;
            int nseg, lo0, len, pitch;
            if constexpr (TILE2D) {
                const int TWc = 1 << twc_log2, RH = NWP * MT * (16 >> twc_log2);
                const int tyi = t / tiles_x, txi = t - tyi * tiles_x;
                const int ya = max(tyi * RH - h, 0), yb = min(tyi * RH + RH + h, a.Hout);
                const int xa = max(txi * TWc - h, 0), xb = min(txi * TWc + TWc + h, a.Wout);
                nseg = yb - ya; lo0 = ya * a.Wout + xa; len = xb - xa; pitch = a.Wout;
            } else {
                constexpr int TPX = 16 * NWP * MT;
                const int lo = max(t * TPX - h * (a.Wout + 1), 0), hi = min(min(t * TPX + TPX, HWo) + h * (a.Wout + 1), HWo);
                nseg = 1; lo0 = lo; len = hi - lo; pitch = 0;
            }
            const int wps = (len + 62) >> 5, items = nseg * wps;
            unsigned int m = 0u;
            for (int j0 = 0; j0 < items; j0 += 64) {
                const int it = j0 + lane, sg = it / wps, bl = a.scan_abase + lo0 + sg * pitch, wd = (bl >> 5) + (it - sg * wps);
                const int s0 = max(bl - wd * 32, 0), s1 = min(bl + len - wd * 32, 32);
                const bool item = it < items && s1 > s0;
                const unsigned int bm = item ? (0xffffffffu >> (32 - (s1 - s0))) << s0 : 0u;
                for (int i0 = 0; i0 < nimg; i0 += 16) {
                    unsigned int cw[16];
#pragma unroll
                    for (int i = 0; i < 16; i++) cw[i] = i0 + i < nimg ? a.cand_bits[(unsigned int)((img + i0 + i) * a.cand_words + (item ? wd : 0))] : 0u;
#pragma unroll
                    for (int i = 0; i < 16; i++) m |= __ballot((cw[i] & bm) != 0u) != 0ull ? 1u << ((i0 + i) & 31) : 0u;
                }
            }
            return (unsigned int)__builtin_amdgcn_readfirstlane((int)m);
        };
        gated = a.tile_gate != 0 && a.cand_bits != nullptr && nimg <= 32;
        if (gated) {
            l_mask = (unsigned int)__builtin_amdgcn_readfirstlane((int)(active ? gate_images(tile) : 0u));
            n_mine = n_max = __builtin_popcount(l_mask);
            if constexpr (PP) {
                const int other = 2 * (bx - grp * wg_tiles) + 1 - sub;
                const unsigned int o_mask = gate_images(other < tiles_x * tiles_y ? other : 0);
                n_max = __builtin_amdgcn_readfirstlane(other < tiles_x * tiles_y ? max(n_mine, __builtin_popcount(o_mask)) : n_mine);
            }
            if (n_max == 0) return;
        }
    }
    int PW, PR, iy_base, ix_base;
    int poff[MT], mloc[MT];
    bool mv[MT];
    if constexpr (TILE2D) {
        const int TWc = 1 << twc_log2, trows = 16 >> twc_log2;
        const int RH = NWP * MT * trows;
        const int tyi = tile / tiles_x, txi = tile - tyi * tiles_x;
        const int y0 = tyi * RH, x0 = txi * TWc;
        PW = TWc * STRIDE + 2; PR = RH * STRIDE + 2;
        iy_base = y0 * STRIDE - 1; ix_base = x0 * STRIDE - 1;
#pragma unroll
        for (int mt = 0; mt < MT; mt++) {
            const int ly = (wv * MT + mt) * trows + (r >> twc_log2), lx = r & (TWc - 1);
            const int oy = y0 + ly, ox = x0 + lx;
            mv[mt] = active && oy < a.Hout && ox < a.Wout;
            mloc[mt] = mv[mt] ? oy * a.Wout + ox : 0;
            poff[mt] = ((ly * STRIDE) * PW + lx * STRIDE) * pix_stride(STRIDE) + g * 16;
        }
    } else {
        constexpr int TPX = 16 * NWP * MT;
        const int m0 = tile * TPX, m1 = min(m0 + TPX, HWo);
        const int y0 = m0 / a.Wout, y1 = (m1 - 1) / a.Wout;
        PW = a.Win + 2; PR = (y1 - y0) * STRIDE + 3;
        iy_base = y0 * STRIDE - 1; ix_base = -1;
#pragma unroll
        for (int mt = 0; mt < MT; mt++) {
            const int m = m0 + (wv * MT + mt) * 16 + r;
            mv[mt] = active && m < m1;
            mloc[mt] = mv[mt] ? m : m0;
            const int oy = mloc[mt] / a.Wout, ox = mloc[mt] - oy * a.Wout;
            poff[mt] = (((oy - y0) * STRIDE) * PW + ox * STRIDE) * pix_stride(STRIDE) + g * 16;
        }
    }
    constexpr int NPL = WR > 0 ? WR : 1;
    static_assert(WR == 0 || (!PF2 && CM == 0), "resident weights: image-major steps, one step of staging lead");
    constexpr int NPB = PP ? 2 * NPL : NPL;
    unsigned char *s_patch = smem + (size_t)sub * NPL * a_patch_bytes;
    half8 *s_w = reinterpret_cast<half8 *>(smem + (size_t)NPB * a_patch_bytes);
    float *s_bias = reinterpret_cast<float *>(smem + (size_t)NPB * a_patch_bytes + (size_t)NPL * 9 * NT * 1024);
    float *s_bias2 = s_bias + 64;
    half8 *s_w2 = reinterpret_cast<half8 *>(s_bias + 128);
    if constexpr (NT % 2 == 0) {
        if (tid < NT * 16) s_bias[tid] = a.bias[by * NT * 16 + tid];
    } else {
        const int t = by;
        if (tid < 16) s_bias[tid] = a.bias[a.pair ? ((t >> 1) * 32 + (tid >> 2) * 8 + (t & 1) * 4 + (tid & 3)) : (t * 16 + tid)];
    }
    if constexpr (N2 > 0) {
        if (tid < N2 * 16) s_bias2[tid] = a.bias2[tid];
        for (int e = tid; e < N2 * 2 * 64; e += NTH) s_w2[e] = reinterpret_cast<const half8 *>(a.w2)[e];
    }
    const int chunks = a.Cin >> 5;
    const half8 zero8 = (half8){0, 0, 0, 0, 0, 0, 0, 0};

    constexpr int PMAX = lds_pmax(STRIDE, MT, TILE2D, WR, PF);
    constexpr int WPT = (9 * NT * 64 + NTH - 1) / NTH;
    const int n_pe = PR * PW * 4;
    const float inv_pw = 1.0f / (float)PW;
    const half_t *src_p[PMAX];
    int dst_p[PMAX];
    bool val_p[PMAX], use_p[PMAX];
#pragma unroll
    for (int i = 0; i < PMAX; i++) {
        const int e = tidp + i * NTP;
        use_p[i] = e < n_pe;
        val_p[i] = false;
        src_p[i] = a.s0.p;
        dst_p[i] = 0;
        if (i * NTP >= n_pe) continue;
        const int pix = use_p[i] ? (e >> 2) : 0, q = e & 3;
        int pr = (int)((float)pix * inv_pw);
        pr -= (pr * PW > pix) ? 1 : 0;
        pr += ((pr + 1) * PW <= pix) ? 1 : 0;
        const int pc = pix - pr * PW;
        const int iy = iy_base + pr, ix = ix_base + pc;
        val_p[i] = active && use_p[i] && (unsigned)iy < (unsigned)a.Hin && (unsigned)ix < (unsigned)a.Win;
        src_p[i] = a.s0.p + ((size_t)(img * a.Hin + (val_p[i] ? iy : 0)) * a.Win + (val_p[i] ? ix : 0)) * a.s0.ld + q * 8;
        dst_p[i] = pix * pix_stride(STRIDE) + q * 16;
    }
    const half8 *wsrc = reinterpret_cast<const half8 *>(wl) + (size_t)nblk * chunks * (9 * NT * 64);

    const half8 *w2 = s_w2 + lane;

    half8 rp[NPF][PMAX], rw[NPF][WPT];
    const size_t img_stride = (size_t)a.Hin * a.Win * a.s0.ld;
    int l_im = 0, l_chunk = 0;
    int c_im = 0, c_chunk = 0;
    auto issue_loads = [&](half8 (&p)[PMAX], half8 (&w)[WPT]) {
        const size_t off = (size_t)l_im * img_stride + (size_t)l_chunk * 32;
#pragma unroll
        for (int i = 0; i < PMAX; i++) {
            p[i] = zero8;
            if (val_p[i]) p[i] = *reinterpret_cast<const half8 *>(src_p[i] + off);
        }
#pragma unroll
        for (int i = 0; i < WPT; i++) {
            if (CM > 0 && l_im != 0) break;
            const int e = tid + i * NTH;
            if (e < 9 * NT * 64) w[i] = wsrc[(size_t)l_chunk * (9 * NT * 64) + e];
        }
        if constexpr (CM > 0) {
            if (++l_im == nimg) { l_im = 0; l_chunk++; }
        } else {
            if (++l_chunk == chunks) { l_chunk = 0; l_im++; }
        }
    };
    auto write_lds = [&](const half8 (&p)[PMAX], const half8 (&w)[WPT]) {
#pragma unroll
        for (int i = 0; i < PMAX; i++) {
            if (use_p[i]) *reinterpret_cast<half8 *>(s_patch + dst_p[i]) = p[i];
        }
#pragma unroll
        for (int i = 0; i < WPT; i++) {
            if (CM > 0 && c_im != 0) break;
            const int e = tid + i * NTH;
            if (e < 9 * NT * 64) s_w[e] = w[i];
        }
    };

    constexpr int NA = CM > 0 ? CM : 1;
    f32x4 acc[NA][MT][NT];
#pragma unroll
    for (int nt = 0; nt < NT; nt++) {
        const int ch = (NT % 2 == 0) ? (by * NT * 16 + (nt >> 1) * 32 + g * 8 + (nt & 1) * 4) : (a.pair ? ((by >> 1) * 32 + g * 8 + (by & 1) * 4) : (by * 16 + g * 4));
        const f32x4 b0 = *reinterpret_cast<const f32x4 *>(a.bias + ch);
#pragma unroll
        for (int ai = 0; ai < NA; ai++)
#pragma unroll
            for (int mt = 0; mt < MT; mt++) acc[ai][mt][nt] = b0;
    }

    const int nt0 = nblk * NT;
    auto store_tile = [&](int im, auto ai_) {
        auto &accx = acc[decltype(ai_)::value];
        half8 W2[N2 > 0 ? N2 : 1][2];
        if constexpr (N2 > 0) {
#pragma unroll
            for (int t2 = 0; t2 < N2; t2++) { W2[t2][0] = w2[(t2 * 2 + 0) * 64]; W2[t2][1] = w2[(t2 * 2 + 1) * 64]; }
        }
        float bs[NT % 2 == 0 ? NT / 2 : 1][8];
        if constexpr (NT % 2 == 0) {
#pragma unroll
            for (int u = 0; u < NT / 2; u++) {
                const f32x4 b0 = *reinterpret_cast<const f32x4 *>(s_bias + u * 32 + g * 8), b1 = *reinterpret_cast<const f32x4 *>(s_bias + u * 32 + g * 8 + 4);
#pragma unroll
                for (int i = 0; i < 4; i++) { bs[u][i] = b0[i]; bs[u][4 + i] = b1[i]; }
            }
        } else {
            const f32x4 b0 = *reinterpret_cast<const f32x4 *>(s_bias + g * 4);
#pragma unroll
            for (int i = 0; i < 4; i++) bs[0][i] = b0[i];
        }
        half8 rv8[NT % 2 == 0 ? MT : 1][NT % 2 == 0 ? NT / 2 : 1];
        half4 rv4[MT];
        if (a.res) {
#pragma unroll
            for (int mt = 0; mt < MT; mt++) {
                const size_t m = (size_t)im * HWo + mloc[mt];
                if constexpr (NT % 2 == 0) {
#pragma unroll
                    for (int u = 0; u < NT / 2; u++) rv8[mt][u] = *reinterpret_cast<const half8 *>(a.res + m * a.res_ld + (nt0 / 2 + u) * 32 + g * 8);
                } else {
                    const int c0 = a.pair ? ((nt0 >> 1) * 32 + g * 8 + (nt0 & 1) * 4) : (nt0 * 16 + g * 4);
                    rv4[mt] = *reinterpret_cast<const half4 *>(a.res + m * a.res_ld + c0);
                }
            }
        }
#pragma unroll
        for (int mt = 0; mt < MT; mt++) {
            if (N2 > 0 || mv[mt]) {
                const size_t m = (size_t)im * HWo + mloc[mt];
                bool st2 = mv[mt];
                if constexpr (N2 > 0) {
                    const bool gate = a.cand_bits != nullptr && a.scan_keys == nullptr;
                    const int an = a.scan_abase + mloc[mt];
                    const unsigned int *cb = gate ? a.cand_bits : reinterpret_cast<const unsigned int *>(a.bias2);
                    const unsigned int cw = cb[gate ? (unsigned int)(im * a.cand_words + (an >> 5)) : 0u];
                    st2 = mv[mt] && (a.cand_bits == nullptr || (gate && ((cw >> (an & 31)) & 1u)));
                }
                if constexpr (NT % 2 == 0) {
                    half8 ov[NT / 2];
#pragma unroll
                    for (int u = 0; u < NT / 2; u++) {
                        const int c0 = (nt0 / 2 + u) * 32 + g * 8;
                        float vals[8];
#pragma unroll
                        for (int i = 0; i < 4; i++) {
                            vals[i] = accx[mt][2 * u][i];
                            vals[4 + i] = accx[mt][2 * u + 1][i];
                        }
                        if (a.res) {
#pragma unroll
                            for (int i = 0; i < 8; i++) ov[u][i] = silu_add_res(vals[i], (float)rv8[mt][u][i]);
                        } else {
                            ov[u] = silu_pack8(vals[0], vals[1], vals[2], vals[3], vals[4], vals[5], vals[6], vals[7]);
                        }
                        if constexpr (N2 == 0) *reinterpret_cast<half8 *>(static_cast<half_t *>(a.out) + m * a.out_ld + c0) = ov[u];
                    }
                    if constexpr (N2 > 0) {
                        mfma_operand_fence(ov[0], ov[1]);
#pragma unroll
                        for (int t2 = 0; t2 < N2; t2++) {
                            f32x4 c2 = (f32x4){0.f, 0.f, 0.f, 0.f};
                            c2 = __builtin_amdgcn_mfma_f32_16x16x32_f16(W2[t2][0], ov[0], c2, 0, 0, 0);
                            c2 = __builtin_amdgcn_mfma_f32_16x16x32_f16(W2[t2][1], ov[1], c2, 0, 0, 0);
                            const int co = t2 * 16 + g * 4;
                            const f32x4 b2 = *reinterpret_cast<const f32x4 *>(s_bias2 + co);
                            const f32x4 v2 = (f32x4){c2[0] * kActUnscale + b2[0], c2[1] * kActUnscale + b2[1], c2[2] * kActUnscale + b2[2], c2[3] * kActUnscale + b2[3]};
                            if (st2) *reinterpret_cast<f32x4 *>(a.out2 + m * a.out2_ld + co) = v2;
                            if (a.scan_keys) {
                                bool hit = false;
#pragma unroll
                                for (int i = 0; i < 4; i++) hit = hit || (mv[mt] && co + i < a.scan_nc && v2[i] > a.scan_thr);
                                if (hit) {
                                    const int an = a.scan_abase + mloc[mt];
                                    if (a.cand_bits) atomicOr(&a.cand_bits[(size_t)im * a.cand_words + (an >> 5)], 1u << (an & 31));
#pragma unroll
                                    for (int i = 0; i < 4; i++) {
                                        if (co + i < a.scan_nc && v2[i] > a.scan_thr) {
                                            const int idx = atomicAdd(&a.scan_counts[im], 1);
                                            const unsigned int u = __float_as_uint(v2[i]);
                                            const unsigned int ord = (u & 0x80000000u) ? ~u : (u | 0x80000000u);
                                            if (idx >= 0 && idx < a.scan_key_cap)
                                                a.scan_keys[(size_t)im * a.scan_key_cap + idx] =
                                                    ((unsigned long long)ord << 32) | (unsigned long long)(0xffffffffu - (unsigned int)(an * a.scan_nc + co + i));
                                        }
                                    }
                                }
                            }
                        }
                    }
                } else {
                    const int t = nt0;
                    const int c0 = a.pair ? ((t >> 1) * 32 + g * 8 + (t & 1) * 4) : (t * 16 + g * 4);
                    half4 o;
                    if (a.res) {
#pragma unroll
                        for (int i = 0; i < 4; i++) o[i] = silu_add_res(accx[mt][0][i], (float)rv4[mt][i]);
                    } else {
                        o = silu_pack4(accx[mt][0][0], accx[mt][0][1], accx[mt][0][2], accx[mt][0][3]);
                    }
                    *reinterpret_cast<half4 *>(static_cast<half_t *>(a.out) + m * a.out_ld + c0) = o;
                }
            }
#pragma unroll
            for (int nt = 0; nt < NT; nt++)
                accx[mt][nt] = (NT % 2 == 0) ? (f32x4){bs[nt >> 1][(nt & 1) * 4 + 0], bs[nt >> 1][(nt & 1) * 4 + 1], bs[nt >> 1][(nt & 1) * 4 + 2], bs[nt >> 1][(nt & 1) * 4 + 3]}
                                             : (f32x4){bs[0][0], bs[0][1], bs[0][2], bs[0][3]};
        }
    };

    using I0 = std::integral_constant<int, 0>;
    const int steps = nimg * chunks;
    constexpr int NPIECE = PMAX + WPT, PER_TAP = (NPIECE + 8) / 9;
    auto taps = [&](auto spread, auto ai_, int plane = 0) {
        constexpr bool SPREAD = decltype(spread)::value;
        auto &accx = acc[decltype(ai_)::value];
        const unsigned char *s_pl = s_patch + (size_t)plane * a_patch_bytes;
        const half8 *s_wc = s_w + plane * (9 * NT * 64);
        size_t off = 0;
        if constexpr (SPREAD) {
            if (l_im == nimg) { l_im = nimg - 1; l_chunk = chunks - 1; }
            off = (size_t)l_im * img_stride + (size_t)l_chunk * 32;
        }
#pragma unroll
        for (int tap = 0; tap < 9; tap++) {
            if constexpr (SPREAD) {
#pragma unroll
                for (int k = 0; k < PER_TAP; k++) {
                    const int j = tap * PER_TAP + k;
                    if (j < PMAX) {
                        rp[0][j] = zero8;
                        if (val_p[j]) rp[0][j] = *reinterpret_cast<const half8 *>(src_p[j] + off);
                    } else if (j < NPIECE) {
                        const int e = tid + (j - PMAX) * NTH;
                        if (e < 9 * NT * 64) rw[0][j - PMAX] = wsrc[(size_t)l_chunk * (9 * NT * 64) + e];
                    }
                }
            }
            const int kh = tap / 3, kw = tap - kh * 3;
            const int toff = (kh * PW + kw) * pix_stride(STRIDE);
            half8 A[NT], B[MT];
#pragma unroll
            for (int nt = 0; nt < NT; nt++) A[nt] = s_wc[(tap * NT + nt) * 64 + lane];
#pragma unroll
            for (int mt = 0; mt < MT; mt++) B[mt] = *reinterpret_cast<const half8 *>(s_pl + poff[mt] + toff);
#pragma unroll
            for (int mt = 0; mt < MT; mt++)
#pragma unroll
                for (int nt = 0; nt < NT; nt++)
                    accx[mt][nt] = __builtin_amdgcn_mfma_f32_16x16x32_f16(A[nt], B[mt], accx[mt][nt], 0, 0, 0);
            if constexpr (SPREAD) __builtin_amdgcn_sched_barrier(0x38f);
        }
        if constexpr (SPREAD) {
            if (++l_chunk == chunks) { l_chunk = 0; l_im++; }
        }
    };
    auto ksteps_wr = [&]() {
        constexpr int KS = (WR > 0 ? WR : 1) * 9;
        auto &accx = acc[0];
        half8 A[2][NT], B[2][MT];
        auto frag = [&](auto ks_, half8 (&Af)[NT], half8 (&Bf)[MT]) {
// ... 23 lines not shown
        };
        run(run, std::integral_constant<int, 0>{});
    };
    auto mma_step = [&]() {
        taps(std::false_type{}, I0{});
        __syncthreads();
        if (++c_chunk == chunks) {
            store_tile(img + c_im, I0{});
            c_chunk = 0;
            c_im++;
        }
    };
    if constexpr (WR > 0) {
        auto next_image = [&]() {
            if (!gated) return l_pos++;
            const int i = __builtin_ctz(l_mask);
            l_mask &= l_mask - 1u;
            return i;
        };
        {
            constexpr int WALL = WR * 9 * NT * 64, WPA = (WALL + NTH - 1) / NTH;
            half8 wr_[WPA];
#pragma unroll
            for (int i = 0; i < WPA; i++) {
                const int e = tid + i * NTH;
                wr_[i] = wsrc[e < WALL ? e : WALL - 1];
            }
#pragma unroll
            for (int i = 0; i < WPA; i++) {
                const int e = tid + i * NTH;
                if (e < WALL) s_w[e] = wr_[i];
            }
        }
        half8 rq[WR][PMAX];
        auto issue_wr = [&](int im) {
            const size_t off = (size_t)im * img_stride;
#pragma unroll
            for (int c = 0; c < WR; c++)
#pragma unroll
                for (int i = 0; i < PMAX; i++) {
                    rq[c][i] = zero8;
                    if (val_p[i]) rq[c][i] = *reinterpret_cast<const half8 *>(src_p[i] + off + c * 32);
                }
        };
        auto write_wr = [&]() {
#pragma unroll
            for (int c = 0; c < WR; c++)
#pragma unroll
                for (int i = 0; i < PMAX; i++)
                    if (use_p[i]) *reinterpret_cast<half8 *>(s_patch + (size_t)c * a_patch_bytes + dst_p[i]) = rq[c][i];
        };
        if constexpr (PP) {
            int cur = 0, pend = 0;
            if (n_mine > 0) { cur = next_image(); issue_wr(cur); }
            if (sub == 1) {
                __builtin_amdgcn_fence(__ATOMIC_RELEASE, "workgroup");
                __builtin_amdgcn_s_barrier();
            }
            if (n_mine > 0) write_wr();
            if (n_mine > 1) { pend = next_image(); issue_wr(pend); }
            __syncthreads();
            for (int s = 0; s < n_max; s++) {
                if (s < n_mine) ksteps_wr();
                __syncthreads();
                if (s < n_mine) {
                    store_tile(img + cur, I0{});
                    if (s + 1 < n_mine) {
                        write_wr();
                        cur = pend;
                        if (s + 2 < n_mine) { pend = next_image(); issue_wr(pend); }
                    }
                }
                __syncthreads();
            }
            if (sub == 0) __builtin_amdgcn_s_barrier();
            return;
        }
        const bool late = stagger && wave >= NWV / 2;
        int cur = next_image(), prev = cur;
        issue_wr(cur);
        for (int s = 0; s < n_mine; s++) {
            write_wr();
            __syncthreads();
            if (late && s > 0) store_tile(img + prev, I0{});
            int nxt = cur;
            if (s + 1 < n_mine) { nxt = next_image(); issue_wr(nxt); }
            ksteps_wr();
            __syncthreads();
            if (!late) store_tile(img + cur, I0{});
            prev = cur; cur = nxt;
        }
        if (late) store_tile(img + prev, I0{});
    } else if constexpr (CM > 0) {
        static_assert(!PF2 && CM <= 4, "chunk-major order: one step of staging lead, at most four images");
        auto each_image = [&](auto f) {
            f(std::integral_constant<int, 0>{});
            if constexpr (CM > 1) f(std::integral_constant<int, 1>{});
            if constexpr (CM > 2) f(std::integral_constant<int, 2>{});
            if constexpr (CM > 3) f(std::integral_constant<int, 3>{});
        };
        issue_loads(rp[0], rw[0]);
        for (int c = 0; c < chunks; c++) {
            each_image([&](auto ai) {
                constexpr int AI = decltype(ai)::value;
                if (AI < nimg) {
                    write_lds(rp[0], rw[0]);
                    __syncthreads();
                    if (!(c == chunks - 1 && AI == nimg - 1)) issue_loads(rp[0], rw[0]);
                    taps(std::false_type{}, ai);
                    __syncthreads();
                    if (++c_im == nimg) { c_im = 0; c_chunk++; }
                }
            });
        }
        each_image([&](auto ai) {
            if (decltype(ai)::value < nimg) store_tile(img + decltype(ai)::value, ai);
        });
    } else if constexpr (!PF2) {
        issue_loads(rp[0], rw[0]);
        for (int s = 0; s < steps; s++) {
            write_lds(rp[0], rw[0]);
            __syncthreads();
            if constexpr (MT == 4) {
                taps(std::true_type{}, I0{});
            } else {
                if (s + 1 < steps) issue_loads(rp[0], rw[0]);
                taps(std::false_type{}, I0{});
            }
            __syncthreads();
            if (++c_chunk == chunks) {
                store_tile(img + c_im, I0{});
                c_chunk = 0;
                c_im++;
            }
        }
    } else {
#pragma unroll
        for (int k = 0; k < NPF; k++)
            if (k < steps) issue_loads(rp[k], rw[k]);
        for (int s = 0; s < steps; s += NPF) {
#pragma unroll
            for (int k = 0; k < NPF; k++) {
                if (s + k < steps) {
                    write_lds(rp[k], rw[k]);
                    __syncthreads();
                    if (s + k + NPF < steps) issue_loads(rp[k], rw[k]);
                    mma_step();
                }
            }
        }
    }
}

template <int STRIDE, int MT, int NT, bool TILE2D, int N2, int PF = 0, int CM = 0, int NWV = 4, int WR = 0, bool PP = false>
__global__ __launch_bounds__(64 * NWV) __attribute__((amdgpu_waves_per_eu(IRMV_LDS_WAVES))) void conv3x3_lds_kernel(ConvArgs a, const half_t *wl, int tiles_x, int tiles_y, int twc_log2, int a_patch_bytes, int ipw, int batch, int nblocks, int xcd)
{
    const int wg_tiles = PP ? (tiles_x * tiles_y + 1) / 2 : tiles_x * tiles_y, groups = (batch + ipw - 1) / ipw;
    int rem, grp;
    tile_image(blockIdx.x, wg_tiles * nblocks, groups, xcd & 1, rem, grp);
    const int nblk = rem / wg_tiles, tile = rem - nblk * wg_tiles;
    conv3x3_lds_body<STRIDE, MT, NT, TILE2D, N2, PF, CM, NWV, WR, PP>(a, wl, tiles_x, tiles_y, twc_log2, a_patch_bytes, ipw, batch, grp * wg_tiles + tile, nblk, wg_tiles * groups, nblocks, (xcd >> 1) & 1);
}

template <int STRIDE, int MT, int NT>
__global__ __launch_bounds__(256) __attribute__((amdgpu_waves_per_eu(IRMV_LDS_WAVES))) void conv3x3_lds_multi(LdsMultiArgs m)
{
    int id = blockIdx.x, k = 0;
    while (k + 1 < m.n && id >= m.start[k + 1]) k++;
    id -= m.start[k];
    const LdsMember &l = m.m[k];
    const int wx = id % l.gx, wy = id / l.gx;
#define IRMV_BODY(T2D_, N2_) conv3x3_lds_body<STRIDE, MT, NT, T2D_, N2_>(l.a, l.wl, l.tiles_x, l.tiles_y, l.twc_log2, l.patch_bytes, 1, l.batch, wx, wy, l.gx, l.gy)
    if constexpr (NT == 4) {
        if (l.a.n2 == 4) { if (l.tile2d) IRMV_BODY(true, 4); else IRMV_BODY(false, 4); return; }
        if (l.a.n2 == 1) { if (l.tile2d) IRMV_BODY(true, 1); else IRMV_BODY(false, 1); return; }
    }
    if (l.tile2d) IRMV_BODY(true, 0); else IRMV_BODY(false, 0);
#undef IRMV_BODY
}

static LdsGeom lds_geom(const ConvArgs &a, int stride, int mt, int nt, int nwv = 4, int wr = 0, bool pp = false, int pf = 0)
{
    LdsGeom g{false, 0, 0, 0, 0, 0};
    if (a.Cin % 32 != 0 || a.s1.C != 0 || a.s0.shift != 0) return g;
    if (!((nt == 1) || ((nt == 2 || nt == 4) && a.pair) || (nt == 8 && a.pair && nwv == 8 && stride == 2 && mt == 1))) return g;
    if (a.cout_pad % (16 * nt) != 0) return g;
    int pr, pw;
    const int l2 = a.Wout % 16 == 0 ? 4 : (a.Wout % 8 == 0 ? 3 : (a.Wout % 4 == 0 ? 2 : -1));
    const int rh = l2 >= 0 ? nwv * mt * (16 >> l2) : 0;
    if (l2 >= 0 && a.Hout % rh == 0) {
        g.tile2d = true;
        g.twc_log2 = l2;
        g.tiles_x = a.Wout >> l2;
        g.tiles_y = a.Hout / rh;
        pr = rh * stride + 2;
        pw = (1 << l2) * stride + 2;
    } else {
        const int tpx = 16 * nwv * mt;
        g.tiles_x = (a.Hout * a.Wout + tpx - 1) / tpx;
        g.tiles_y = 1;
        const int rows = (tpx + a.Wout - 2) / a.Wout + 1;
        pr = (rows - 1) * stride + 3;
        pw = a.Win + 2;
    }
    if ((size_t)pr * pw * 4 > (size_t)lds_pmax(stride, mt, g.tile2d, wr, pf) * 64 * nwv) return g;
    g.patch_bytes = pr * pw * pix_stride(stride);
    const int planes = wr ? wr : 1;
    const size_t bytes = (size_t)planes * (pp ? 2 : 1) * g.patch_bytes + (size_t)planes * 9 * nt * 1024 + 512 + (size_t)a.n2 * 2048;
    if (bytes > (size_t)(wr ? 160 : (nwv == 8 ? 150 : 80)) * 1024) return g;
    g.bytes = bytes;
    return g;
}

static const half_t *lds_weights(const ConvWeights &w, int nt) { return w.w_lds[nt == 8 ? 3 : (nt == 4 ? 2 : (nt == 2 ? 1 : 0))]; }

bool conv_lds_fits(const ConvArgs &a, const ConvWeights &w, int stride, int mt, int nt)
{
    return lds_weights(w, nt) && lds_geom(a, stride, mt, nt).bytes > 0;
}

template <int STRIDE, int MT, int NT, bool TILE2D, int N2, int PF = 0, int CM = 0, int NWV = 4, int WR = 0, bool PP = false>
static void launch_lds_inst(const ConvLaunch &l, hipStream_t s)
{
    static unsigned long long attr_done = 0;
    once_per_device(attr_done, [] {
        (void)hipFuncSetAttribute(reinterpret_cast<const void *>(conv3x3_lds_kernel<STRIDE, MT, NT, TILE2D, N2, PF, CM, NWV, WR, PP>), hipFuncAttributeMaxDynamicSharedMemorySize, 160 * 1024);
    });
    const LdsGeom &g = l.g;
    const int groups = (l.batch + l.ipw - 1) / l.ipw;
    const int wg_tiles = PP ? (g.tiles_x * g.tiles_y + 1) / 2 : g.tiles_x * g.tiles_y;
    const int nblocks = l.a.cout_pad / (16 * NT);
    hipLaunchKernelGGL((conv3x3_lds_kernel<STRIDE, MT, NT, TILE2D, N2, PF, CM, NWV, WR, PP>), dim3(wg_tiles * groups * nblocks), dim3(64 * NWV), g.bytes, s, l.a,
                       l.w, g.tiles_x, g.tiles_y, g.twc_log2, g.patch_bytes, l.ipw, l.batch, nblocks, xcd_image_order() | (wres_stagger() << 1));
}

static LdsGeom wres_geom(const ConvArgs &a, int stride, bool pp)
{
    if (stride != 1 || a.Cin != 64 || a.cout_pad != 64 || !a.pair || (a.n2 > 0 && a.res) || !(a.n2 == 0 || a.n2 == 1 || a.n2 == 4)) return LdsGeom{false, 0, 0, 0, 0, 0};
    LdsGeom g = pp ? lds_geom(a, 1, 2, 4, 4, 2, true) : lds_geom(a, 1, 2, 4, 8, 2);
    if (pp && !g.tile2d) g.bytes = 0;
    return g;
}
int conv_wres_tiles(const ConvArgs &a, int stride, bool pp)
{
    const LdsGeom g = wres_geom(a, stride, pp);
    if (!g.bytes) return 0;
    return pp ? (g.tiles_x * g.tiles_y + 1) / 2 : g.tiles_x * g.tiles_y;
}

struct LdsKey { int stride, mt, nt, n2, pf, cm, nwv, wr, pp; };
struct LdsVariant { LdsKey key; ConvLauncher launch[2]; };

template <int ST, int MT, int NT, int N2 = 0, int PF = 0, int CM = 0, int NWV = 4, int WR = 0, bool PP = false>
constexpr LdsVariant lds_variant()
{
    LdsVariant v{{ST, MT, NT, N2, PF, CM, NWV, WR, PP}, {nullptr, launch_lds_inst<ST, MT, NT, true, N2, PF, CM, NWV, WR, PP>}};
    if constexpr (!PP) v.launch[0] = launch_lds_inst<ST, MT, NT, false, N2, PF, CM, NWV, WR, PP>;
    return v;
}

static constexpr LdsVariant k_lds[] = {
    lds_variant<1, 1, 1>(), lds_variant<1, 2, 1>(), lds_variant<1, 4, 1>(),
    lds_variant<1, 1, 2>(), lds_variant<1, 2, 2>(), lds_variant<1, 4, 2>(),
    lds_variant<1, 1, 4>(), lds_variant<1, 2, 4>(), lds_variant<1, 4, 4>(),
    lds_variant<2, 1, 1>(), lds_variant<2, 2, 1>(), lds_variant<2, 4, 1>(),
    lds_variant<2, 1, 2>(), lds_variant<2, 2, 2>(), lds_variant<2, 4, 2>(),
    lds_variant<2, 1, 4>(), lds_variant<2, 2, 4>(), lds_variant<2, 4, 4>(),
    lds_variant<1, 1, 4, 1>(), lds_variant<1, 2, 4, 1>(), lds_variant<1, 4, 4, 1>(),
    lds_variant<1, 1, 4, 4>(), lds_variant<1, 2, 4, 4>(), lds_variant<1, 4, 4, 4>(),
    lds_variant<1, 1, 1, 0, 1>(), lds_variant<1, 1, 2, 0, 1>(), lds_variant<1, 1, 4, 0, 1>(),
    lds_variant<2, 1, 1, 0, 1>(), lds_variant<2, 1, 2, 0, 1>(), lds_variant<2, 1, 4, 0, 1>(),
    lds_variant<1, 1, 1, 0, 2>(), lds_variant<2, 1, 1, 0, 2>(),
    lds_variant<1, 1, 4, 0, 0, 4>(), lds_variant<1, 1, 4, 0, 0, 2>(), lds_variant<1, 2, 4, 0, 0, 2>(),
    lds_variant<2, 1, 4, 0, 0, 4>(), lds_variant<2, 1, 4, 0, 0, 2>(), lds_variant<2, 2, 4, 0, 0, 2>(),
    lds_variant<1, 1, 4, 1, 0, 4>(), lds_variant<1, 2, 4, 1, 0, 2>(), lds_variant<1, 1, 4, 4, 0, 4>(), lds_variant<1, 2, 4, 4, 0, 2>(),
    lds_variant<2, 2, 4, 0, 0, 0, 8>(), lds_variant<2, 2, 4, 0, 0, 2, 8>(), lds_variant<2, 1, 4, 0, 0, 0, 8>(), lds_variant<2, 1, 4, 0, 0, 4, 8>(),
    lds_variant<2, 1, 8, 0, 0, 0, 8>(), lds_variant<2, 1, 8, 0, 0, 2, 8>(),
    lds_variant<1, 2, 4, 0, 0, 0, 8, 2>(), lds_variant<1, 2, 4, 1, 0, 0, 8, 2>(), lds_variant<1, 2, 4, 4, 0, 0, 8, 2>(),
    lds_variant<1, 2, 4, 0, 0, 0, 8, 2, true>(), lds_variant<1, 2, 4, 1, 0, 0, 8, 2, true>(), lds_variant<1, 2, 4, 4, 0, 0, 8, 2, true>(),
};

static ConvLauncher pick_lds(const ConvCfg &c, const ConvArgs &a, int ipw, LdsGeom &g)
{
    const int pf = c.pf4 ? 2 : (c.pf2 ? 1 : 0), nwv = c.w8 || c.wr ? 8 : 4;
    if (c.cm && c.cm != ipw) return nullptr;
    if (a.n2 > 0 && (a.cout_pad != 64 || !a.pair || a.res)) return nullptr;
    g = c.wr ? wres_geom(a, c.stride, c.pp) : lds_geom(a, c.stride, c.mt, c.nt, nwv, 0, false, pf);
    if (!g.bytes) return nullptr;
    const LdsKey key{c.stride, c.mt, c.nt, a.n2, pf, c.cm, nwv, c.wr ? 2 : 0, c.pp};
    for (const LdsVariant &v : k_lds)
        if (!memcmp(&v.key, &key, sizeof key)) return v.launch[g.tile2d];
    return nullptr;
}

// ... 236 lines not shown
```

### irmv_detection_amd/csrc/k_kpt.hip

```cpp
#include "irmv_common.hpp"

namespace irmv {

namespace {
constexpr int KT = kKpt3Tile;
constexpr int K1W = KT + 4, K1N = K1W * K1W;
constexpr int K2W = KT + 2, K2N = K2W * K2W;
constexpr int KPL = K1N * 64;
constexpr int KQS = 32;
constexpr int KNT = 192;
constexpr int KNP = (K1N * 8 + KNT - 1) / KNT;
static_assert(K2N == 9 * 16, "the halo region is nine MFMA tiles");
typedef unsigned int u32x4 __attribute__((ext_vector_type(4)));
}

template <int STEPS>
__global__ __launch_bounds__(KNT) __attribute__((amdgpu_waves_per_eu(3))) void kpt3_kernel(Kpt3Args a, int batch, int ipw, int xcd)
{
    extern __shared__ __attribute__((aligned(16))) uint8_t smem[];
    uint8_t *s_in = smem;
    uint8_t *s_t = smem + 2 * KPL;
    half8 *s_w2 = reinterpret_cast<half8 *>(smem + 2 * KPL + K2N * KQS);
    const int tid = threadIdx.x, lane = tid & 63, wave = tid >> 6;
    const int g = lane >> 4, r = lane & 15;
    const int tiles = a.tiles_x * a.tiles_y, groups = (batch + ipw - 1) / ipw;
    int tile, grp;
    tile_image(blockIdx.x, tiles, groups, xcd, tile, grp);
    const int img0 = grp * ipw, nimg = min(ipw, batch - img0);
    const int tyi = tile / a.tiles_x, txi = tile - tyi * a.tiles_x;
    const int oy0 = tyi * KT, ox0 = txi * KT;
    const int H = a.H, W = a.W;
    constexpr int KSTEPS = STEPS * 18;

    int src[KNP];
    static_assert(KNT % 8 == 0 && (KNP - 1) * KNT < K1N * 8, "piece i of a thread: pixel (tid >> 3) + i * KNT / 8, eighth tid & 7; only the last i can fall off the region");
    const int dstA = (tid >> 3) * 64 + ((tid & 7) >> 2) * KPL + (tid & 3) * 16, dstB = dstA ^ 32;
    bool odd[KNP];
    const bool last_piece = tid + (KNP - 1) * KNT < K1N * 8;
#pragma unroll
    for (int i = 0; i < KNP; i++) {
        const int e = tid + i * KNT, px = e >> 3, q = e & 7;
        const int ly = px / K1W, lx = px - ly * K1W;
        const int gy = oy0 - 2 + ly, gx = ox0 - 2 + lx;
        const bool in = e < K1N * 8 && (unsigned)gy < (unsigned)H && (unsigned)gx < (unsigned)W;
        odd[i] = (ly & 1) != 0;
        src[i] = in ? (((img0 * H + gy) * W + gx) * a.x_ld + q * 8) * 2 : 0x7fffffff;
    }
    const int img_stride = H * W * a.x_ld * 2;
    const auto rs_x = __builtin_amdgcn_make_buffer_rsrc(const_cast<half_t *>(a.x), 0, batch * img_stride, 0x00020000);
    const auto rs_w = __builtin_amdgcn_make_buffer_rsrc(const_cast<half_t *>(a.w1), 0, KSTEPS * 1024, 0x00020000);
    auto load_w = [&](int k) { return __builtin_bit_cast(half8, __builtin_amdgcn_raw_buffer_load_b128(rs_w, lane * 16, k * 1024, 0)); };
    u32x4 v[KNP];
    unsigned int amask = nimg >= 32 ? 0xffffffffu : (1u << nimg) - 1u;
    if (a.tile_gate && a.cand_bits) {
        const int rows = min(KT, H - oy0), cols = min(KT, W - ox0);
        const int row = lane >> 1, bl = a.abase + (oy0 + row) * W + ox0, wd = (bl >> 5) + (lane & 1);
        const int s0 = max(bl - wd * 32, 0), s1 = min(bl + cols - wd * 32, 32);
        const bool item = row < rows && s1 > s0;
        const unsigned int bm = item ? (0xffffffffu >> (32 - (s1 - s0))) << s0 : 0u;
        unsigned int cwd[8];
#pragma unroll
        for (int i = 0; i < 8; i++) cwd[i] = i < nimg ? a.cand_bits[(unsigned int)((img0 + i) * a.cand_words + (item ? wd : 0))] : 0u;
        amask = 0u;
#pragma unroll
        for (int i = 0; i < 8; i++) amask |= __ballot((cwd[i] & bm) != 0u) != 0ull ? 1u << i : 0u;
        amask = __builtin_amdgcn_readfirstlane(amask);
        if (amask == 0u) return;
    }
    int l_im = __builtin_ctz(amask), l_s = 0;
    unsigned int l_rest = amask & (amask - 1u);
    auto issue_slab = [&]() {
        const int off = __builtin_amdgcn_readfirstlane(l_im * img_stride + l_s * 128);
#pragma unroll
        for (int i = 0; i < KNP; i++) v[i] = __builtin_bit_cast(u32x4, __builtin_amdgcn_raw_buffer_load_b128(rs_x, src[i], off, 0));
        if (!(l_rest == 0u && l_s == STEPS - 1)) { if (++l_s == STEPS) { l_s = 0; l_im = __builtin_ctz(l_rest); l_rest &= l_rest - 1u; } }
    };
    auto write_slab = [&]() {
#pragma unroll
        for (int i = 0; i < KNP; i++)
            if (i + 1 < KNP || last_piece) *reinterpret_cast<u32x4 *>(s_in + (odd[i] ? dstB : dstA) + i * (KNT / 8) * 64) = v[i];
    };

    issue_slab();
    __builtin_amdgcn_sched_barrier(0);
    half8 A[6];
#pragma unroll
    for (int k = 0; k < 6; k++) A[k] = load_w(k);
    const f32x4 b1 = *reinterpret_cast<const f32x4 *>(a.b1 + g * 4);
    __builtin_amdgcn_sched_barrier(0);
    {
        const half8 *w2p = reinterpret_cast<const half8 *>(a.w2);
        const half8 t0 = w2p[tid], t1 = w2p[tid + KNT < 288 ? tid + KNT : 287];
        s_w2[tid] = t0;
        if (tid + KNT < 288) s_w2[tid + KNT] = t1;
    }
    const f32x4 b2 = *reinterpret_cast<const f32x4 *>(a.b2 + g * 4);
    const half4 w3f = *reinterpret_cast<const half4 *>(a.w3 + lane * 4);
    const f32x4 b3 = *reinterpret_cast<const f32x4 *>(a.b3 + g * 4);
    __builtin_amdgcn_sched_barrier(0);

    const int bly = wave * 4 + (r >> 2), blx = r & 3;
    const int baseE = (bly * K1W + blx) * 64 + ((g ^ (2 * (bly & 1))) & 3) * 16;
    const int baseO = (bly * K1W + blx) * 64 + ((g ^ (2 * (~bly & 1))) & 3) * 16;
    const int tap_lo = g >> 1;
    int toff2[5];
#pragma unroll
    for (int ks = 0; ks < 5; ks++) {
        const int tap = 2 * ks + tap_lo, tc = tap < 9 ? tap : 0, kh = tc / 3, kw = tc - kh * 3;
        toff2[ks] = ((bly + kh) * K2W + blx + kw) * KQS + (g & 1) * 16;
    }
    half8 Bf[2][3];
    auto frag = [&](int kk, half8 (&B)[3]) {
        const int c = kk / 9, tap = kk - c * 9, kh = tap / 3, kw = tap - kh * 3;
        const int off = (kh * K1W + kw) * 64 + c * KPL;
#pragma unroll
        for (int i = 0; i < 3; i++) B[i] = *reinterpret_cast<const half8 *>(s_in + (kh == 1 ? baseO : baseE) + off + i * 256);
    };

    for (unsigned int c_rest = amask; c_rest; c_rest &= c_rest - 1u) {
        const int im = __builtin_ctz(c_rest);
        unsigned int cw[3];
#pragma unroll
        for (int i = 0; i < 3; i++) {
            const int gy = oy0 + bly, gx = ox0 + i * 4 + blx;
            const int an = a.abase + ((gy < H && gx < W) ? gy * W + gx : 0);
            const unsigned int *cb = a.cand_bits ? a.cand_bits : reinterpret_cast<const unsigned int *>(a.b3);
            const unsigned int w = cb[a.cand_bits ? (unsigned int)((img0 + im) * a.cand_words + (an >> 5)) : 0u];
            cw[i] = a.cand_bits ? (w >> (an & 31)) & 1u : 1u;
        }
        f32x4 acc[3] = {b1, b1, b1};
#pragma unroll
        for (int s = 0; s < STEPS; s++) {
            write_slab();
            __syncthreads();
            frag(0, Bf[0]);
#pragma unroll
            for (int kk = 0; kk < 18; kk++) {
                const int k = s * 18 + kk;
                if (kk + 1 < 18) frag(kk + 1, Bf[(kk + 1) & 1]);
                __builtin_amdgcn_sched_barrier(0);
#pragma unroll
                for (int i = 0; i < 3; i++) acc[i] = __builtin_amdgcn_mfma_f32_16x16x32_f16(A[kk % 6], Bf[kk & 1][i], acc[i], 0, 0, 0);
                __builtin_amdgcn_sched_barrier(0);
                if (kk == 12) issue_slab();
                A[kk % 6] = load_w((k + 6) % KSTEPS);
                __builtin_amdgcn_sched_barrier(0);
            }
            if (s + 1 < STEPS) __syncthreads();
        }
#pragma unroll
        for (int i = 0; i < 3; i++) {
            const int lx = i * 4 + blx;
            const int gy = oy0 - 1 + bly, gx = ox0 - 1 + lx;
            half4 o = (half4){0, 0, 0, 0};
            if ((unsigned)gy < (unsigned)H && (unsigned)gx < (unsigned)W) o = silu_pack4(acc[i][0], acc[i][1], acc[i][2], acc[i][3]);
            *reinterpret_cast<half4 *>(s_t + (bly * K2W + lx) * KQS + g * 8) = o;
        }
        __syncthreads();

        half8 A2[5];
#pragma unroll
        for (int ks = 0; ks < 5; ks++) A2[ks] = s_w2[ks * 64 + (ks == 4 ? (lane & 31) : lane)];
        if (g >= 2) A2[4] = (half8){0, 0, 0, 0, 0, 0, 0, 0};
#pragma unroll
        for (int i = 0; i < 3; i++) {
            const int ly = bly, lx = i * 4 + blx;
            const bool valid = ly < KT && lx < KT;
            f32x4 c1 = b2;
            half8 B2[5];
#pragma unroll
            for (int ks = 0; ks < 5; ks++) {
                const u32x4 q = *reinterpret_cast<const u32x4 *>(s_t + toff2[ks] + i * 4 * KQS);
                B2[ks] = __builtin_bit_cast(half8, 2 * ks + tap_lo < 9 ? q : (u32x4){0u, 0u, 0u, 0u});
            }
#pragma unroll
            for (int ks = 0; ks < 5; ks++) c1 = __builtin_amdgcn_mfma_f32_16x16x32_f16(A2[ks], B2[ks], c1, 0, 0, 0);
            half4 o = silu_pack4(c1[0], c1[1], c1[2], c1[3]);
            mfma_operand_fence(o);
            const f32x4 c2 = __builtin_amdgcn_mfma_f32_16x16x16f16(w3f, o, (f32x4){0.f, 0.f, 0.f, 0.f}, 0, 0, 0);
            const f32x4 v2 = (f32x4){c2[0] * kActUnscale + b3[0], c2[1] * kActUnscale + b3[1], c2[2] * kActUnscale + b3[2], c2[3] * kActUnscale + b3[3]};
            const int gy = oy0 + ly, gx = ox0 + lx;
            if (valid && gy < H && gx < W && cw[i]) *reinterpret_cast<f32x4 *>(a.out + ((size_t)((img0 + im) * H + gy) * W + gx) * a.out_ld + g * 4) = v2;
        }
    }
}

bool kpt3_eligible(int cin) { return cin == 64 || cin == 128 || cin == 256; }

bool launch_kpt3(const Kpt3Args &a, int cin, int batch, hipStream_t s)
{
    const int tiles = a.tiles_x * a.tiles_y;
    int ipw = 1;
    while (ipw < 8 && (long long)tiles * batch >= 2048LL * ipw) ipw *= 2;
    const dim3 grid(tiles * ((batch + ipw - 1) / ipw)), block(KNT);
    constexpr size_t lds = (size_t)2 * KPL + (size_t)K2N * KQS + 4608;
    static_assert(lds <= 40 * 1024, "four workgroups per CU");
    const int xcd = xcd_image_order();
    switch (cin) {
    case 64: hipLaunchKernelGGL((kpt3_kernel<1>), grid, block, lds, s, a, batch, ipw, xcd); return true;
    case 128: hipLaunchKernelGGL((kpt3_kernel<2>), grid, block, lds, s, a, batch, ipw, xcd); return true;
    case 256: hipLaunchKernelGGL((kpt3_kernel<4>), grid, block, lds, s, a, batch, ipw, xcd); return true;
    default: return false;
    }
}

}
```

### irmv_detection_amd/csrc/k_post.hip

```cpp
#include "irmv_common.hpp"
#include "pnp_device.hpp"

#include <mutex>

namespace irmv {

__device__ __forceinline__ float irmv_expf(float x)
{
    x = x < -87.0f ? -87.0f : x;
    x = x > 88.0f ? 88.0f : x;
    const float n = rintf(x * 1.44269504088896341f);
    float r = fmaf(n, -0.693145751953125f, x);
    r = fmaf(n, -1.42860682030941723212e-6f, r);
    float p = 1.0f / 720.0f;
    p = fmaf(p, r, 1.0f / 120.0f);
    p = fmaf(p, r, 1.0f / 24.0f);
    p = fmaf(p, r, 1.0f / 6.0f);
    p = fmaf(p, r, 0.5f);
    p = fmaf(p, r, 1.0f);
    p = fmaf(p, r, 1.0f);
    return __int_as_float(__float_as_int(p) + ((int)n << 23));
}

__device__ __forceinline__ uint32_t orderable(float f)
// ... 285 lines not shown
#pragma unroll 8
    for (int j = 0; j < 64; j++) {
        const f32x4 bj = sbox[j];
        const int cj = scls[j];
        if (j < lane && cj == cls && cls >= 0 && iou_gt(bj, box, iou_thr)) sup |= 1ull << j;
    }
    wave_lds_sync();
    return sup;
}

__global__ __launch_bounds__(1024) void nms_pnp_kernel(PostArgs a)
{
    __shared__ __attribute__((aligned(16))) unsigned long long skeys[kCandCap];
    __shared__ unsigned long long srank[kRankSortMax];
    __shared__ __attribute__((aligned(16))) unsigned long long ssup[kSupCap];
    __shared__ f32x4 stage_box[16][64];
    __shared__ __attribute__((aligned(16))) int stage_cls[16][64];
    __shared__ f32x4 kept_box[kMaxDetCap];
    __shared__ int kept_cls[kMaxDetCap];
    __shared__ unsigned long long kept_key[kMaxDetCap];
    __shared__ unsigned short cls_list[16][kMaxDetCap];
    __shared__ int cls_cnt[16];
    __shared__ int s_kept;

    const int b = blockIdx.x, tid = threadIdx.x, lane = tid & 63, wave = tid >> 6;
#define IRMV_STAMP(k) do { if (a.dbg && tid == 0) a.dbg[b * 16 + (k)] = clock64(); } while (0)
    IRMV_STAMP(0);
    __shared__ int s_ncand, s_nanch;
    unsigned long long *gk = a.keys + (size_t)b * a.key_cap;
    const unsigned long long *sorted;
    unsigned short *alist = a.A <= 4 * kSupCap ? reinterpret_cast<unsigned short *>(ssup) : nullptr;
    if (tid < 16) cls_cnt[tid] = 0;
    if (tid == 0) { s_ncand = 0; s_nanch = 0; }
    __syncthreads();
    if (a.counts) {
        constexpr int KPL = kCandCap / 1024;
        unsigned long long k_mine[KPL];
#pragma unroll
        for (int k = 0; k < KPL; k++) {
            const int i = tid + k * 1024;
            k_mine[k] = gk[i < a.key_cap ? i : a.key_cap - 1];
        }
        int n = a.counts[b];
        n = n < 0 ? 0 : (n > a.key_cap ? a.key_cap : n);
        if (n <= kCandCap) {
#pragma unroll
            for (int k = 0; k < KPL; k++)
                if (tid + k * 1024 < n) skeys[tid + k * 1024] = k_mine[k];
        }
        __syncthreads();
        if (tid == 0) { s_ncand = n; a.counts[b] = 0; }
        if (a.cand_bits)
            for (int i = tid; i < a.cand_words; i += blockDim.x) a.cand_bits[(size_t)b * a.cand_words + i] = 0u;
    } else {
    {
        constexpr int U = 8;
        int lbase = 0;
#pragma unroll 1
        for (int l = 0; l < 3; l++) {
            const int lhw = (a.net_w / (8 << l)) * (a.net_h / (8 << l));
            const float *lrec = a.head_all + ((size_t)lbase * a.slots_total + (size_t)(a.first + b) * lhw) * kHeadRec;
            const int quads = lhw * 4;
            for (int q0 = 0; q0 < quads; q0 += 1024 * U) {
                f32x4 cl[U];
#pragma unroll
                for (int u = 0; u < U; u++) {
                    const int t = q0 + u * 1024 + tid;
                    const int rin = t < quads ? (t >> 2) : 0;
                    cl[u] = reinterpret_cast<const f32x4 *>(lrec + (size_t)rin * kHeadRec + kClsOff)[tid & 3];
                }
#pragma unroll
                for (int u = 0; u < U; u++) {
                    if (q0 + u * 1024 >= quads) break;
                    const int t = q0 + u * 1024 + tid;
                    scan_quad(a, lbase + (t >> 2), t < quads, cl[u], skeys, gk, &s_ncand, alist, &s_nanch);
                }
            }
            lbase += lhw;
        }
    }
    __syncthreads();
    decode_boxes(a, b, alist, alist ? s_nanch : a.A);
    }
    __syncthreads();
    IRMV_STAMP(7);
    const int n_total = s_ncand;
    __shared__ unsigned int hist[256];
    __shared__ int s_digit, s_rem, s_fill;
    auto decode_keys = [&](const unsigned long long *keys, int cnt) {
        const int q = tid & 3, base = lane & ~3;
        for (int i0 = 0; i0 < cnt; i0 += 512) {
            f32x4 v[2][4];
            int an_[2];
            bool live_[2];
#pragma unroll
            for (int u = 0; u < 2; u++) {
                const int ci = i0 + u * 256 + (tid >> 2);
                live_[u] = ci < cnt;
                const unsigned long long key = live_[u] ? keys[ci] : 0ull;
                const uint32_t id = 0xffffffffu - (uint32_t)(key & 0xffffffffu);
                an_[u] = live_[u] ? anchor_of(id, a.nc, a.A) : 0;
                int ix, iy, st, lbase, lhw, rin;
                anchor_geom(an_[u], a.net_w, a.net_h, ix, iy, st, lbase, lhw, rin);
                const float *rec = head_rec(a.head_all, a.slots_total, a.first + b, lbase, lhw, rin);
#pragma unroll
                for (int i = 0; i < 4; i++) v[u][i] = reinterpret_cast<const f32x4 *>(rec + 16 * q)[i];
// ... 761 lines not shown
```

### irmv_detection_amd/engine.py

```python
from __future__ import annotations

import ctypes as C
import enum
import os
from dataclasses import dataclass, field
from typing import List, Optional, Sequence, Tuple

import numpy as np

from . import capi
from .capi import IrmvError


class ArmorClass(enum.IntEnum):
    B1 = 0; B2 = 1; B3 = 2; B4 = 3; B5 = 4; BO = 5; BS = 6
    R1 = 7; R2 = 8; R3 = 9; R4 = 10; R5 = 11; RO = 12; RS = 13
    UNKNOWN = 14


class ArmorSize(enum.IntEnum):
    SMALL = 0; LARGE = 1; UNKNOWN = 2


@dataclass
# ... 285 lines not shown
        return int(self._L.irmv_engine_src_device_buffer(self._h, slot))

    def read_input(self, slot: int = 0) -> np.ndarray:
        out = np.empty((3, self.net_height, self.net_width), np.float32)
        capi.check(self._L.irmv_engine_read_input(self._h, slot, out.ctypes.data_as(C.POINTER(C.c_float))))
        return out

    def read_head(self, slot: int = 0) -> np.ndarray:
        out = np.empty((self.num_anchors, self.head_channels), np.float32)
        capi.check(self._L.irmv_engine_read_head(self._h, slot, out.ctypes.data_as(C.POINTER(C.c_float))))
        return out

    def write_head(self, head: np.ndarray, slot: int = 0) -> None:
        head = np.ascontiguousarray(head, np.float32)
        assert head.shape == (self.num_anchors, self.head_channels)
        capi.check(self._L.irmv_engine_write_head(self._h, slot, head.ctypes.data_as(C.POINTER(C.c_float))))

    def run_post(self, first_slot: int = 0, count: int = 1) -> None:
        capi.check(self._L.irmv_engine_run_post(self._h, first_slot, count))

    def read_tap(self, name: str, slot: int = 0) -> np.ndarray:
        shape = (C.c_int * 3)()
        capi.check(self._L.irmv_engine_read_tap(self._h, slot, name.encode(), None, shape))
        out = np.empty(tuple(shape), np.float32)
        capi.check(self._L.irmv_engine_read_tap(self._h, slot, name.encode(),
                                                out.ctypes.data_as(C.POINTER(C.c_float)), shape))
        return out

    def read_raw(self, slot: int = 0) -> dict:
        md = self.max_det
        boxes = np.zeros((md, 4), np.float32); scores = np.zeros(md, np.float32)
        classes = np.zeros(md, np.int32); anchors = np.zeros(md, np.int32); kpts = np.zeros((md, 8), np.float32)
        raw = capi.RawDets(0, 0, boxes.ctypes.data_as(C.POINTER(C.c_float)), scores.ctypes.data_as(C.POINTER(C.c_float)),
                           classes.ctypes.data_as(C.POINTER(C.c_int32)), anchors.ctypes.data_as(C.POINTER(C.c_int32)),
                           kpts.ctypes.data_as(C.POINTER(C.c_float)))
        capi.check(self._L.irmv_engine_read_raw(self._h, slot, C.byref(raw)))
        n = raw.num_dets
        return dict(num_dets=n, n_candidates=raw.n_candidates, boxes=boxes[:n], scores=scores[:n],
                    classes=classes[:n], anchors=anchors[:n], kpts=kpts[:n],
                    boxes_padded=boxes, scores_padded=scores)

    def debug_poke_candidate_counts(self, value: int) -> None:
        capi.check(self._L.irmv_engine_debug_poke_candidate_counts(self._h, int(value)))

    def debug_cand_bits(self, slot: int = 0):
        n, sparse = C.c_int(0), C.c_int(0)
        capi.check(self._L.irmv_engine_debug_read_cand_bits(self._h, slot, None, 0, C.byref(n), C.byref(sparse)))
        words = np.zeros(n.value, np.uint32)
        if n.value:
            capi.check(self._L.irmv_engine_debug_read_cand_bits(self._h, slot, words.ctypes.data_as(C.POINTER(C.c_uint32)), n.value,
                                                                 C.byref(n), C.byref(sparse)))
        return bool(sparse.value), words

    def debug_head_rows(self, slot: int = 0) -> np.ndarray:
        out = np.empty((self.num_anchors, 96), np.float32)
        capi.check(self._L.irmv_engine_debug_read_head_rows(self._h, slot, out.ctypes.data_as(C.POINTER(C.c_float)), out.nbytes))
        return out

    def debug_read_head_raw(self, slot: int = 0) -> np.ndarray:
        out = np.empty((self.num_anchors, self.head_channels), np.float32)
        capi.check(self._L.irmv_engine_debug_read_head_raw(self._h, slot, out.ctypes.data_as(C.POINTER(C.c_float))))
        return out

    def profile(self, first_slot: int = 0, count: Optional[int] = None) -> List[dict]:
        count = self.num_slots - first_slot if count is None else count
        stats = (capi.KernelStat * 256)()
        n = C.c_int(0)
        capi.check(self._L.irmv_engine_profile(self._h, first_slot, count, stats, 256, C.byref(n)))
        return [dict(name=stats[i].name.decode(), layer=stats[i].layer.decode(), flops=stats[i].flops,
                     bytes=stats[i].bytes, ms=stats[i].ms) for i in range(min(n.value, 256))]

    def _detect_raw(self, slot):
        slot = self.slot if slot is None else slot
        n = C.c_int(0)
        capi.check(self._L.irmv_engine_detect(self._h, slot, self._dets, self.max_det, C.byref(n)))
        return [self._dets[i] for i in range(n.value)]

    @staticmethod
    def _to_armor(d) -> Armor:
        k = list(d.kpts)
        a = Armor(left_light=Light(top=(k[2], k[3]), bottom=(k[0], k[1])),
                  right_light=Light(top=(k[4], k[5]), bottom=(k[6], k[7])),
                  size=ArmorSize(d.armor_size) if d.armor_size in (0, 1) else ArmorSize.UNKNOWN,
                  armor_class=ArmorClass(d.class_id), confidence=d.score, valid=d.armor_valid == 1, n_lights=d.n_lights, no_answer=d.armor_valid < 0,
                  bbox_xyxy=tuple(d.xyxy), pnp_ok=bool(d.pnp_ok),
                  rvec=np.array(d.rvec), tvec=np.array(d.tvec), quat_xyzw=np.array(d.quat))
        a.center = ((k[0] + k[2] + k[4] + k[6]) / 4.0, (k[1] + k[3] + k[5] + k[7]) / 4.0)
        return a


class PnPSolver:

    def __init__(self, camera_matrix: Sequence[float], distortion_coefficients: Sequence[float], *, device: int = 0):
        self._L = capi.load()
        self.camera_matrix = np.asarray(camera_matrix, np.float64).reshape(9).copy()
        d = list(distortion_coefficients) + [0.0] * 5
        self.dist_coeffs = np.asarray(d[:5], np.float64)
        self._h = C.c_void_p()
        capi.check(self._L.irmv_pnp_create(device, self.camera_matrix.ctypes.data_as(C.POINTER(C.c_double)),
                                           self.dist_coeffs.ctypes.data_as(C.POINTER(C.c_double)), C.byref(self._h)))

    def close(self):
        if getattr(self, "_h", None):
            self._L.irmv_pnp_destroy(self._h)
            self._h = None

# ... 21 lines not shown
```

Baseline: 66040.

## Balance sparse head tiles across workgroups using per-image tile masks

The class-scan kernel now writes per-image bitmasks of tiles that contain candidates. Gated keypoint and box convolutions launch a balanced variant that spreads the active (image, tile) pairs evenly over workgroups through a wave-level prefix scan, instead of assigning fixed tiles and letting empty ones exit early. The aim is to cut wasted workgroups and load imbalance when candidates are sparse. The cost is extra mask writes and clears, a second compiled copy of the kpt kernel, and more complex indexing that applies only to small batches and small tile counts.

```diff
diff --git a/include/irmv_hip.h b/include/irmv_hip.h
--- a/include/irmv_hip.h
+++ b/include/irmv_hip.h
@@ -176,6 +176,8 @@
 int irmv_engine_run_post(irmv_engine *e, int first_slot, int count);
 int irmv_engine_debug_poke_candidate_counts(irmv_engine *e, int value);
 int irmv_engine_debug_read_cand_bits(irmv_engine *e, int slot, uint32_t *words, int cap, int *n, int *sparse);
+int irmv_engine_debug_gate_plan(irmv_engine *e, int count, int32_t *flags, int cap, int *n);
+int irmv_engine_debug_read_tile_masks(irmv_engine *e, int slot, uint64_t *masks, int cap, int *n);
 int irmv_engine_debug_read_head_rows(irmv_engine *e, int slot, float *rec, size_t bytes);
 int irmv_engine_debug_read_head_raw(irmv_engine *e, int slot, float *head);
 int irmv_engine_read_tap(irmv_engine *e, int slot, const char *name, float *nhwc, int shape[3]);
diff --git a/irmv_detection_amd/_build.py b/irmv_detection_amd/_build.py
--- a/irmv_detection_amd/_build.py
+++ b/irmv_detection_amd/_build.py
@@ -18,6 +18,7 @@
     ("k_c2f.hip", []),
     ("k_bneck.hip", []),
     ("k_kpt.hip", []),
+    ("k_kpt_bal.hip", []),
     ("k_conv.hip", []),
     ("k_post.hip", ["-ffp-contract=off"]),
     ("k_light.hip", ["-ffp-contract=off"]),
@@ -88,7 +89,7 @@
     for src, extra in SOURCES:
         sp = os.path.join(CSRC, src)
         obj = os.path.join(LIB_DIR, os.path.splitext(src)[0] + ".o")
-        if force or _stale(obj, [sp] + headers):
+        if force or _stale(obj, [sp] + headers + ([os.path.join(CSRC, "k_kpt.hip")] if src == "k_kpt_bal.hip" else [])):
             cmd = [cc] + COMMON + extra + os.environ.get("IRMV_EXTRA_HIPCC_FLAGS", "").split() + ["-c", sp, "-o", obj]
             if verbose:
                 print(" ".join(cmd))
diff --git a/irmv_detection_amd/capi.py b/irmv_detection_amd/capi.py
--- a/irmv_detection_amd/capi.py
+++ b/irmv_detection_amd/capi.py
@@ -183,6 +183,8 @@
     ("irmv_engine_run_post", C.c_int, [_P, C.c_int, C.c_int]),
     ("irmv_engine_debug_poke_candidate_counts", C.c_int, [_P, C.c_int]),
     ("irmv_engine_debug_read_cand_bits", C.c_int, [_P, C.c_int, C.POINTER(C.c_uint32), C.c_int, C.POINTER(C.c_int), C.POINTER(C.c_int)]),
+    ("irmv_engine_debug_gate_plan", C.c_int, [_P, C.c_int, C.POINTER(C.c_int32), C.c_int, C.POINTER(C.c_int)]),
+    ("irmv_engine_debug_read_tile_masks", C.c_int, [_P, C.c_int, C.POINTER(C.c_uint64), C.c_int, C.POINTER(C.c_int)]),
     ("irmv_engine_debug_read_head_rows", C.c_int, [_P, C.c_int, C.POINTER(C.c_float), C.c_size_t]),
     ("irmv_engine_debug_read_head_raw", C.c_int, [_P, C.c_int, C.POINTER(C.c_float)]),
     ("irmv_engine_read_tap", C.c_int, [_P, C.c_int, C.c_char_p, C.POINTER(C.c_float), C.POINTER(C.c_int)]),
diff --git a/irmv_detection_amd/csrc/engine.cpp b/irmv_detection_amd/csrc/engine.cpp
--- a/irmv_detection_amd/csrc/engine.cpp
+++ b/irmv_detection_amd/csrc/engine.cpp
@@ -244,7 +244,7 @@
     if (const char *uk = getenv("IRMV_UPLOAD_KERNEL")) s.upload_kernel_blocks = atoi(uk);
     s.sync_launch = starts("IRMV_SYNC_LAUNCH", 'e') ? 1 : (starts("IRMV_SYNC_LAUNCH", 'g') ? 0 : -1);
     s.split_scan = !off("IRMV_SPLIT_SCAN"); s.emit_scan = !off("IRMV_EMIT_SCAN");
-    s.sparse_head = !off("IRMV_SPARSE_HEAD"); s.sparse_branch = !off("IRMV_SPARSE_BRANCH");
+    s.sparse_head = !off("IRMV_SPARSE_HEAD"); s.sparse_branch = !off("IRMV_SPARSE_BRANCH"); s.sparse_balance = !off("IRMV_SPARSE_BALANCE");
     s.zero_copy_results = !off("IRMV_ZERO_COPY_RESULTS"); s.post_keys_only = is1("IRMV_POST_KEYS_ONLY");
     s.nms_classwalk = !off("IRMV_NMS_CLASSWALK");
     s.nms_prefilter = off("IRMV_NMS_PREFILTER") ? 0 : 1;
diff --git a/irmv_detection_amd/csrc/engine_graph.cpp b/irmv_detection_amd/csrc/engine_graph.cpp
--- a/irmv_detection_amd/csrc/engine_graph.cpp
+++ b/irmv_detection_amd/csrc/engine_graph.cpp
@@ -690,6 +690,8 @@
         e->cand_words = (e->A + 31) / 32;
         TRY(dev_alloc(e, (void **)&e->cand_bits, (size_t)S * e->cand_words * sizeof(unsigned int)));
         HIP_TRY(hipMemset(e->cand_bits, 0, (size_t)S * e->cand_words * sizeof(unsigned int)));
+        TRY(dev_alloc(e, (void **)&e->tile_masks, (size_t)S * kTileMaskWords * sizeof(unsigned long long)));
+        HIP_TRY(hipMemset(e->tile_masks, 0, (size_t)S * kTileMaskWords * sizeof(unsigned long long)));
     }
     e->head_stale.assign((size_t)S, 0);
     e->branch_stale.assign((size_t)S, 0);
diff --git a/irmv_detection_amd/csrc/engine_hooks.cpp b/irmv_detection_amd/csrc/engine_hooks.cpp
--- a/irmv_detection_amd/csrc/engine_hooks.cpp
+++ b/irmv_detection_amd/csrc/engine_hooks.cpp
@@ -40,6 +40,29 @@
     TRY(irmv_engine_wait(e));
     HIP_TRY(hipSetDevice(e->cfg.device));
     HIP_TRY(hipMemcpy(words, e->cand_bits + (size_t)slot * e->cand_words, (size_t)e->cand_words * sizeof(unsigned int), hipMemcpyDeviceToHost));
+    return IRMV_OK;
+}
+
+extern "C" int irmv_engine_debug_gate_plan(irmv_engine *e, int count, int32_t *flags, int cap, int *n)
+{
+    TRY(check_range(e, 0, count));
+    if (!n) return fail(IRMV_ERR_ARG, "n is null");
+    const std::vector<Launch> &plan = e->plans[count == 1 ? STEP_ONE : STEP_BATCH];
+    *n = (int)plan.size();
+    for (int i = 0; flags && i < cap && i < *n; i++) flags[i] = (plan[i].sparse ? 1 : 0) | (plan[i].gate << 1) | (plan[i].balanced ? 8 : 0);
+    return IRMV_OK;
+}
+
+extern "C" int irmv_engine_debug_read_tile_masks(irmv_engine *e, int slot, uint64_t *masks, int cap, int *n)
+{
+    TRY(check_range(e, slot, 1));
+    if (!n) return fail(IRMV_ERR_ARG, "n is null");
+    *n = e->sparse_balance && e->tile_masks ? kTileMaskWords : 0;
+    if (!masks || *n == 0) return IRMV_OK;
+    if (cap < *n) return fail(IRMV_ERR_ARG, "read_tile_masks: buffer too small");
+    TRY(irmv_engine_wait(e));
+    HIP_TRY(hipSetDevice(e->cfg.device));
+    HIP_TRY(hipMemcpy(masks, e->tile_masks + (size_t)slot * kTileMaskWords, (size_t)kTileMaskWords * sizeof(unsigned long long), hipMemcpyDeviceToHost));
     return IRMV_OK;
 }
 
diff --git a/irmv_detection_amd/csrc/engine_internal.hpp b/irmv_detection_amd/csrc/engine_internal.hpp
--- a/irmv_detection_amd/csrc/engine_internal.hpp
+++ b/irmv_detection_amd/csrc/engine_internal.hpp
@@ -84,6 +84,7 @@
     int sync_launch = -1;
     bool split_scan = true;
     bool emit_scan = true, sparse_head = true, sparse_branch = true;
+    bool sparse_balance = true;
     bool zero_copy_results = true;
     bool post_keys_only = false;
     bool nms_classwalk = true;
@@ -134,6 +135,7 @@
     bool keys_only = false;
     bool sparse = false;
     int gate = 0;
+    bool balanced = false;
     bool once = false;
     std::string name, layer;
     double flops = 0, bytes = 0, launch_bytes = 0;
@@ -171,6 +173,9 @@
     std::vector<char> head_stale;
     bool sparse_branch = false;
     std::vector<char> branch_stale;
+    bool sparse_balance = false;
+    unsigned long long *tile_masks = nullptr;
+    TileMaskDesc tmask_desc[3][3] = {};
     int lvl_hw[3] = {0, 0, 0}, lvl_base[3] = {0, 0, 0};
     size_t frame_bytes = 0;
     size_t src_bytes = 0;
@@ -240,6 +245,7 @@
     ~irmv_engine();
 };
 
+constexpr int kTileMaskKinds = 3, kTileMaskWords = 3 * kTileMaskKinds;
 constexpr int kProfileRepeat = 4;
 
 struct TuneEntry { int mt, nt, flags, ipw; };
diff --git a/irmv_detection_amd/csrc/engine_plan.cpp b/irmv_detection_amd/csrc/engine_plan.cpp
--- a/irmv_detection_amd/csrc/engine_plan.cpp
+++ b/irmv_detection_amd/csrc/engine_plan.cpp
@@ -27,9 +27,13 @@
 static void sparse_head_plan(irmv_engine *e, std::vector<Launch> &plan)
 {
     int last_cls = -1;
-    bool lvl_cls[3] = {false, false, false};
+    bool lvl_cls[3] = {false, false, false}, lvl_masks[3] = {false, false, false};
     for (size_t i = 0; i < plan.size(); i++)
-        if (plan[i].scan && plan[i].group < 0) { last_cls = (int)i; lvl_cls[e->ops[plan[i].op].level] = true; }
+        if (plan[i].scan && plan[i].group < 0) {
+            const Op &co = e->ops[plan[i].op];
+            last_cls = (int)i; lvl_cls[co.level] = true;
+            lvl_masks[co.level] = (plan[i].cfg_one ? co.cfg_one : co.cfg).wr && e->nc <= 16;
+        }
     auto box_carrier = [&](const Launch &l) {
         const Op &op = e->ops[l.op];
         return l.group < 0 && l.fused && op.kind == OP_CONV && is_box_final_carrier(op) && op.level < 3 && lvl_cls[op.level];
@@ -74,6 +78,26 @@
             l.gate = 2;
             op.gated_first = true;
             e->lazy_tensors.insert(e->tensors[op.out_t].name);
+        }
+        if (l.gate && e->sw.sparse_balance && op.level >= 0 && op.level < 3 && lvl_masks[op.level]) {
+            TileMaskDesc d{};
+            int tiles = 0, kind = 0;
+            if (op.kind == OP_KPT3) {
+                d = tile_mask_desc(kKpt3Tile, kKpt3Tile, (op.Win + kKpt3Tile - 1) / kKpt3Tile, 0);
+                tiles = d.tiles_x * ((op.Hin + kKpt3Tile - 1) / kKpt3Tile);
+            } else {
+                const ConvCfg &cfg = l.cfg_one ? op.cfg_one : op.cfg;
+                ConvArgs ca;
+                fill_conv_args(e, op, 0, 1, ca, l.fused);
+                if (cfg.wr && cfg.pp) tiles = conv_wres_pp_blocks(ca, cfg.stride, d);
+                d.halo = l.gate - 1;
+                kind = l.gate;
+            }
+            if (tiles > 0 && tiles <= kBalanceMaxTiles && op.Hout * op.Wout < (1 << 15)) {
+                l.balanced = true;
+                e->sparse_balance = true;
+                e->tmask_desc[op.level][kind] = d;
+            }
         }
         if ((box || first_conv[i]) && (int)i < last_cls) moved.push_back(l); else out.push_back(l);
         if ((int)i == last_cls) { out.insert(out.end(), moved.begin(), moved.end()); moved.clear(); }
diff --git a/irmv_detection_amd/csrc/engine_step.cpp b/irmv_detection_amd/csrc/engine_step.cpp
--- a/irmv_detection_amd/csrc/engine_step.cpp
+++ b/irmv_detection_amd/csrc/engine_step.cpp
@@ -102,6 +102,8 @@
     p.counts = e->sw.split_scan ? e->cand_counts + first : nullptr;
     p.cand_bits = e->sparse_head ? e->cand_bits + (size_t)first * e->cand_words : nullptr;
     p.cand_words = e->cand_words;
+    p.tile_masks = e->sparse_balance && e->tile_masks ? e->tile_masks + (size_t)first * kTileMaskWords : nullptr;
+    p.tile_mask_words = kTileMaskWords;
     return p;
 }
 
@@ -203,7 +205,7 @@
     return a;
 }
 
-static Kpt3Args kpt3_args(const irmv_engine *e, const Op &op, const Launch &l, int first, const PostArgs &pa)
+static Kpt3Args kpt3_args(const irmv_engine *e, const Op &op, const Launch &l, int first, int count, const PostArgs &pa)
 {
     const Op &o0 = e->ops[op.sub[0]], &o1 = e->ops[op.sub[1]], &o2 = e->ops[op.sub[2]];
     const Tensor &xt = e->tensors[o0.s0.t], &ht = e->tensors[o2.out_t];
@@ -216,6 +218,7 @@
     a.w3 = o2.w_k16; a.b3 = o2.bias;
     a.out = static_cast<float *>(ht.slot(first)) + o2.out_coff; a.out_ld = ht.C;
     if (l.sparse) { a.cand_bits = pa.cand_bits; a.cand_words = pa.cand_words; a.abase = e->lvl_base[op.level]; a.tile_gate = l.gate; }
+    if (l.balanced && a.tile_gate && pa.tile_masks && count <= kBalanceMaxImages) { a.tmask = pa.tile_masks + op.level * kTileMaskKinds; a.tmask_stride = kTileMaskWords; }
     return a;
 }
 
@@ -258,6 +261,11 @@
     a.scan_key_cap = pa.key_cap;
     a.scan_abase = e->lvl_base[op.level];
     a.cand_bits = pa.cand_bits; a.cand_words = pa.cand_words;
+    if (pa.tile_masks && pa.cand_bits && op.level >= 0 && op.level < 3) {
+        bool any = false;
+        for (int k = 0; k < kTileMaskKinds; k++) { a.tm[k] = e->tmask_desc[op.level][k]; any = any || a.tm[k].rows > 0; }
+        if (any) { a.tmask = pa.tile_masks + op.level * kTileMaskKinds; a.tmask_stride = kTileMaskWords; a.tm_inv_w = 1.0f / (float)op.Wout; }
+    }
 }
 
 bool irmv::launch_head_group(const irmv_engine *e, const irmv_engine::HeadGroup &g, int first, const PostArgs *pa, unsigned scan, hipStream_t s)
@@ -287,7 +295,7 @@
     case OP_BNECK:
         if (!launch_bneck64(op.mode, op.sub[2] >= 0 ? e->ops[op.sub[2]].ksteps : 6, op.shortcut, bneck_args(e, op, first), count, s)) return fail(IRMV_ERR_ARG, "no fused bottleneck kernel for " + op.layer);
         break;
-    case OP_KPT3: if (!launch_kpt3(kpt3_args(e, op, l, first, pa), op.cin, count, s)) return fail(IRMV_ERR_ARG, "no fused keypoint-branch kernel for " + op.layer); break;
+    case OP_KPT3: if (!launch_kpt3(kpt3_args(e, op, l, first, count, pa), op.cin, count, s)) return fail(IRMV_ERR_ARG, "no fused keypoint-branch kernel for " + op.layer); break;
     case OP_DW: launch_dwconv3x3(dw_args(e, op, first), count, s); break;
     case OP_SHUF: launch_shuffle_cat(shuf_args(e, op, first, count), s); break;
     case OP_CONV0: launch_conv0(conv0_args(e, op, first, count), s); break;
@@ -301,6 +309,7 @@
         fill_conv_args(e, op, first, count, a, l.fused);
         if (scan) scan_args_for(e, op, pa, a);
         if (l.sparse || l.gate) { a.cand_bits = pa.cand_bits; a.cand_words = pa.cand_words; a.scan_abase = e->lvl_base[op.level]; a.tile_gate = l.gate; }
+        if (l.balanced && l.gate && pa.tile_masks && count <= kBalanceMaxImages) { a.tgate = pa.tile_masks + op.level * kTileMaskKinds + l.gate; a.tmask_stride = kTileMaskWords; }
         if (!run_conv(op, l.cfg_one ? op.cfg_one : op.cfg, a, count, s)) return fail(IRMV_ERR_ARG, std::string("no conv kernel for ") + op.kname + " (" + op.layer + ")");
         break;
     }
diff --git a/irmv_detection_amd/csrc/irmv_common.hpp b/irmv_detection_amd/csrc/irmv_common.hpp
--- a/irmv_detection_amd/csrc/irmv_common.hpp
+++ b/irmv_detection_amd/csrc/irmv_common.hpp
@@ -56,6 +56,82 @@
         image = (full / tiles) + r / tiles;
         tile = r % tiles;
     }
+}
+
+constexpr int kBalanceMaxImages = 128, kBalanceMaxTiles = 64;
+struct TileMaskDesc { int rows, cols, tiles_x, halo; float inv_rows, inv_cols; };
+inline TileMaskDesc tile_mask_desc(int rows, int cols, int tiles_x, int halo) { return TileMaskDesc{rows, cols, tiles_x, halo, 1.0f / (float)rows, 1.0f / (float)cols}; }
+struct TileShare {
+    const unsigned long long *masks; int stride;
+    unsigned long long m0, m1;
+    unsigned long long nz0, nz1;
+    unsigned long long bits;
+    int img, T, incl;
+
+    __device__ __forceinline__ void load(const unsigned long long *masks_, int stride_, int batch, int lane)
+    {
+        masks = masks_; stride = stride_;
+        const unsigned long long a = masks[(size_t)min(lane, batch - 1) * stride], b = masks[(size_t)min(64 + lane, batch - 1) * stride];
+        m0 = lane < batch ? a : 0ull;
+        m1 = 64 + lane < batch ? b : 0ull;
+    }
+    __device__ __forceinline__ static unsigned long long lane_u64(unsigned long long v, int l)
+    {
+        const unsigned int lo = __builtin_amdgcn_readlane((int)(unsigned int)v, l), hi = __builtin_amdgcn_readlane((int)(unsigned int)(v >> 32), l);
+        return ((unsigned long long)hi << 32) | lo;
+    }
+    __device__ __forceinline__ void count(int lane)
+    {
+        int s = __builtin_popcountll(m0) | (__builtin_popcountll(m1) << 16);
+#pragma unroll
+        for (int d = 1; d < 64; d <<= 1) {
+            const int t = __shfl_up(s, d);
+            s += lane >= d ? t : 0;
+        }
+        incl = s;
+        const int tot = __builtin_amdgcn_readlane(s, 63);
+        T = (tot & 0xffff) + (tot >> 16);
+    }
+    __device__ __forceinline__ int first_entry(int k, int K) const { return (int)(((unsigned int)k * (unsigned int)T) / (unsigned int)K); }
+    __device__ __forceinline__ int length(int k, int K) const { return first_entry(k + 1, K) - first_entry(k, K); }
+    __device__ __forceinline__ int begin(int k, int K)
+    {
+        const int e0 = first_entry(k, K), n = first_entry(k + 1, K) - e0;
+        if (n == 0) return 0;
+        const int tot0 = __builtin_amdgcn_readlane(incl, 63) & 0xffff;
+        const int i0 = incl & 0xffff, i1 = tot0 + (incl >> 16);
+        const unsigned long long b0 = __ballot(i0 > e0), b1 = __ballot(i1 > e0);
+        int before;
+        if (b0 != 0ull) {
+            const int i = __builtin_ctzll(b0);
+            bits = lane_u64(m0, i);
+            before = __builtin_amdgcn_readlane(i0, i) - __builtin_popcountll(bits);
+            img = i; nz0 = __ballot(m0 != 0ull) & ~((2ull << i) - 1ull); nz1 = __ballot(m1 != 0ull);
+        } else {
+            const int i = __builtin_ctzll(b1);
+            bits = lane_u64(m1, i);
+            before = __builtin_amdgcn_readlane(i1, i) - __builtin_popcountll(bits);
+            img = 64 + i; nz0 = 0ull; nz1 = __ballot(m1 != 0ull) & ~((2ull << i) - 1ull);
+        }
+        for (int j = before; j < e0; j++) bits &= bits - 1ull;
+        return n;
+    }
+    __device__ __forceinline__ void next(int &image, int &tile)
+    {
+        if (bits == 0ull) {
+            if (nz0 != 0ull) { img = __builtin_ctzll(nz0); nz0 &= nz0 - 1ull; }
+            else { img = 64 + __builtin_ctzll(nz1); nz1 &= nz1 - 1ull; }
+            bits = ((const __attribute__((address_space(4))) unsigned long long *)masks)[(size_t)img * stride];
+        }
+        image = img;
+        tile = __builtin_ctzll(bits);
+        bits &= bits - 1ull;
+    }
+};
+__device__ __forceinline__ int share_of_workgroup(int id, int n, int xcd)
+{
+    const int x = id & 7;
+    return xcd ? x * (n >> 3) + min(x, n & 7) + (id >> 3) : id;
 }
 
 inline int xcd_image_order()
@@ -233,9 +309,12 @@
     const unsigned int *cand_bits;
     int cand_words, abase;
     int tile_gate;
+    const unsigned long long *tmask;
+    int tmask_stride;
 };
 bool kpt3_eligible(int cin);
 bool launch_kpt3(const Kpt3Args &a, int cin, int batch, hipStream_t s);
+bool launch_kpt3_balanced(const Kpt3Args &a, int cin, int batch, hipStream_t s);
 
 struct ConvArgs {
     ConvSeg s0, s1;
@@ -263,6 +342,11 @@
     unsigned int *cand_bits;
     int cand_words;
     int tile_gate;
+    unsigned long long *tmask;
+    const unsigned long long *tgate;
+    int tmask_stride;
+    TileMaskDesc tm[3];
+    float tm_inv_w;
 };
 
 constexpr int kMultiMax = 6;
@@ -303,6 +387,7 @@
 bool conv_pw_eligible(const ConvCfg &cfg, const ConvArgs &a);
 bool conv_lds_fits(const ConvArgs &a, const ConvWeights &w, int stride, int mt, int nt);
 int conv_wres_tiles(const ConvArgs &a, int stride, bool pp);
+int conv_wres_pp_blocks(const ConvArgs &a, int stride, TileMaskDesc &d);
 bool launch_conv_lds_multi(int nt, const ConvArgs *a, const ConvWeights *w, int n, int batch, hipStream_t s);
 bool launch_conv_direct_multi(const ConvCfg &cfg, const ConvArgs *a, int n, hipStream_t s);
 
@@ -350,6 +435,8 @@
     int *counts;
     unsigned int *cand_bits;
     int cand_words;
+    unsigned long long *tile_masks;
+    int tile_mask_words;
     int pnp_stride;
 };
 void launch_nms_pnp(const PostArgs &a, int batch, hipStream_t s);
diff --git a/irmv_detection_amd/csrc/k_conv.hip b/irmv_detection_amd/csrc/k_conv.hip
--- a/irmv_detection_amd/csrc/k_conv.hip
+++ b/irmv_detection_amd/csrc/k_conv.hip
@@ -661,12 +661,16 @@
 #ifndef IRMV_LDS_WAVES
 #define IRMV_LDS_WAVES 2
 #endif
-template <int STRIDE, int MT, int NT, bool TILE2D, int N2, int PF = 0, int CM = 0, int NWV = 4, int WR = 0, bool PP = false>
+template <int STRIDE, int MT, int NT, bool TILE2D, int N2, int PF = 0, int CM = 0, int NWV = 4, int WR = 0, bool PP = false, bool BAL = false>
 __device__ __forceinline__ void conv3x3_lds_body(const ConvArgs &a, const half_t *wl, int tiles_x, int tiles_y, int twc_log2, int a_patch_bytes, int ipw, int batch,
-                                                 int wg_x, int wg_y, int grid_x, int grid_y, int stagger = 0)
+                                                 int wg_x, int wg_y, int grid_x, int grid_y, int stagger = 0, int xcd_shares = 0)
 {
     extern __shared__ __attribute__((aligned(16))) unsigned char smem[];
     const int lane = threadIdx.x & 63, wave = threadIdx.x >> 6, tid = threadIdx.x;
+    static_assert(!BAL || PP, "balanced gate: ping-pong form");
+    constexpr bool bal = BAL;
+    TileShare sh;
+    if constexpr (BAL) sh.load(a.tgate, a.tmask_stride, batch, lane);
     constexpr bool PF2 = PF != 0;
     constexpr int NPF = PF == 2 ? 4 : (PF == 1 ? 2 : 1);
     constexpr int NTH = 64 * NWV;
@@ -680,7 +684,7 @@
     const int wg_tiles = PP ? (tiles_x * tiles_y + 1) / 2 : tiles_x * tiles_y;
     const int grp = bx / wg_tiles;
     int tile = PP ? 2 * (bx - grp * wg_tiles) + sub : bx - grp * wg_tiles;
-    const bool active = tile < tiles_x * tiles_y;
+    bool active = tile < tiles_x * tiles_y;
     if (!active) tile = 0;
     const int img = grp * ipw, nimg = min(ipw, batch - img);
     const int nblk = by;
@@ -721,7 +725,15 @@
             }
             return (unsigned int)__builtin_amdgcn_readfirstlane((int)m);
         };
-        gated = a.tile_gate != 0 && a.cand_bits != nullptr && nimg <= 32;
+        if constexpr (BAL) {
+            sh.count(lane);
+            const int K = 2 * (int)gridDim.x, k = __builtin_amdgcn_readfirstlane(2 * share_of_workgroup(blockIdx.x, gridDim.x, xcd_shares) + sub);
+            n_mine = __builtin_amdgcn_readfirstlane(sh.begin(k, K));
+            n_max = __builtin_amdgcn_readfirstlane(max(n_mine, sh.length(k ^ 1, K)));
+            if (n_max == 0) return;
+            tile = 0; active = true;
+        }
+        gated = !bal && a.tile_gate != 0 && a.cand_bits != nullptr && nimg <= 32;
         if (gated) {
             l_mask = (unsigned int)__builtin_amdgcn_readfirstlane((int)(active ? gate_images(tile) : 0u));
             n_mine = n_max = __builtin_popcount(l_mask);
@@ -794,6 +806,9 @@
     const half_t *src_p[PMAX];
     int dst_p[PMAX];
     bool val_p[PMAX], use_p[PMAX];
+    static_assert(!BAL || (PMAX <= 8 && STRIDE == 1), "balanced gate: border bits of at most eight pieces");
+    int rel_p[BAL ? PMAX : 1];
+    unsigned int edge_p = 0u;
 #pragma unroll
     for (int i = 0; i < PMAX; i++) {
         const int e = tidp + i * NTP;
@@ -801,6 +816,7 @@
         val_p[i] = false;
         src_p[i] = a.s0.p;
         dst_p[i] = 0;
+        if constexpr (BAL) rel_p[i] = 0;
         if (i * NTP >= n_pe) continue;
         const int pix = use_p[i] ? (e >> 2) : 0, q = e & 3;
         int pr = (int)((float)pix * inv_pw);
@@ -811,6 +827,10 @@
         val_p[i] = active && use_p[i] && (unsigned)iy < (unsigned)a.Hin && (unsigned)ix < (unsigned)a.Win;
         src_p[i] = a.s0.p + ((size_t)(img * a.Hin + (val_p[i] ? iy : 0)) * a.Win + (val_p[i] ? ix : 0)) * a.s0.ld + q * 8;
         dst_p[i] = pix * pix_stride(STRIDE) + q * 16;
+        if constexpr (BAL) {
+            rel_p[i] = ((pr - 1) * a.Win + (pc - 1)) * a.s0.ld + q * 8;
+            edge_p |= (pr == 0 ? 1u << i : 0u) | (pr == PR - 1 ? 0x100u << i : 0u) | (pc == 0 ? 0x10000u << i : 0u) | (pc == PW - 1 ? 0x1000000u << i : 0u);
+        }
     }
     const half8 *wsrc = reinterpret_cast<const half8 *>(wl) + (size_t)nblk * chunks * (9 * NT * 64);
 
@@ -900,6 +920,7 @@
                 }
             }
         }
+        unsigned int hit_mt = 0u;
 #pragma unroll
         for (int mt = 0; mt < MT; mt++) {
             if (N2 > 0 || mv[mt]) {
@@ -949,6 +970,7 @@
                                 if (hit) {
                                     const int an = a.scan_abase + mloc[mt];
                                     if (a.cand_bits) atomicOr(&a.cand_bits[(size_t)im * a.cand_words + (an >> 5)], 1u << (an & 31));
+                                    if constexpr (N2 == 1 && WR > 0) hit_mt |= 1u << mt;
 #pragma unroll
                                     for (int i = 0; i < 4; i++) {
                                         if (co + i < a.scan_nc && v2[i] > a.scan_thr) {
@@ -982,6 +1004,25 @@
                 accx[mt][nt] = (NT % 2 == 0) ? (f32x4){bs[nt >> 1][(nt & 1) * 4 + 0], bs[nt >> 1][(nt & 1) * 4 + 1], bs[nt >> 1][(nt & 1) * 4 + 2], bs[nt >> 1][(nt & 1) * 4 + 3]}
                                              : (f32x4){bs[0][0], bs[0][1], bs[0][2], bs[0][3]};
         }
+        if constexpr (N2 == 1 && WR > 0) {
+            if (a.tmask && hit_mt) {
+#pragma unroll
+                for (int mt = 0; mt < MT; mt++) {
+                    if (!((hit_mt >> mt) & 1u)) continue;
+                    const int oy = (int)(((float)mloc[mt] + 0.5f) * a.tm_inv_w), ox = mloc[mt] - oy * a.Wout;
+#pragma unroll
+                    for (int k = 0; k < 3; k++) {
+                        if (a.tm[k].rows == 0) continue;
+                        const int h = a.tm[k].halo;
+                        const int ty0 = (int)(((float)max(oy - h, 0) + 0.5f) * a.tm[k].inv_rows), ty1 = (int)(((float)min(oy + h, a.Hout - 1) + 0.5f) * a.tm[k].inv_rows);
+                        const int tx0 = (int)(((float)max(ox - h, 0) + 0.5f) * a.tm[k].inv_cols), tx1 = (int)(((float)min(ox + h, a.Wout - 1) + 0.5f) * a.tm[k].inv_cols);
+                        const int r0 = ty0 * a.tm[k].tiles_x, r1 = ty1 * a.tm[k].tiles_x;
+                        const unsigned long long m = (1ull << (r0 + tx0)) | (1ull << (r0 + tx1)) | (1ull << (r1 + tx0)) | (1ull << (r1 + tx1));
+                        atomicOr(&a.tmask[(size_t)im * a.tmask_stride + k], m);
+                    }
+                }
+            }
+        }
     };
 
     using I0 = std::integral_constant<int, 0>;
@@ -1111,23 +1152,54 @@
         };
         if constexpr (PP) {
             int cur = 0, pend = 0;
-            if (n_mine > 0) { cur = next_image(); issue_wr(cur); }
+            int cur_t = 0, pend_t = 0;
+            int mrel[MT];
+#pragma unroll
+            for (int mt = 0; mt < MT; mt++) mrel[mt] = mloc[mt];
+            const int TWc = 1 << twc_log2, RH = NWP * MT * (16 >> twc_log2);
+            auto fetch = [&](int &im, int &t) {
+                if constexpr (!BAL) { im = next_image(); issue_wr(im); return; }
+                sh.next(im, t);
+                im = __builtin_amdgcn_readfirstlane(im); t = __builtin_amdgcn_readfirstlane(t);
+                const int ty = t / tiles_x, tx = t - ty * tiles_x;
+                const unsigned int hit = edge_p & ((ty == 0 ? 0xffu : 0u) | (ty == tiles_y - 1 ? 0xff00u : 0u) | (tx == 0 ? 0xff0000u : 0u) | (tx == tiles_x - 1 ? 0xff000000u : 0u));
+                const unsigned int out = hit | (hit >> 8) | (hit >> 16) | (hit >> 24);
+                const half_t *base = a.s0.p + ((size_t)(im * a.Hin + ty * RH) * a.Win + tx * TWc) * a.s0.ld;
+#pragma unroll
+                for (int c = 0; c < WR; c++)
+#pragma unroll
+                    for (int i = 0; i < PMAX; i++) {
+                        rq[c][i] = zero8;
+                        if (use_p[i] && !((out >> i) & 1u)) rq[c][i] = *reinterpret_cast<const half8 *>(base + rel_p[i] + c * 32);
+                    }
+            };
+            auto finish = [&]() {
+                if constexpr (BAL) {
+                    const int ty = cur_t / tiles_x, tx = cur_t - ty * tiles_x;
+#pragma unroll
+                    for (int mt = 0; mt < MT; mt++) mloc[mt] = mrel[mt] + ty * RH * a.Wout + tx * TWc;
+                    store_tile(cur, I0{});
+                } else {
+                    store_tile(img + cur, I0{});
+                }
+            };
+            if (n_mine > 0) fetch(cur, cur_t);
             if (sub == 1) {
                 __builtin_amdgcn_fence(__ATOMIC_RELEASE, "workgroup");
                 __builtin_amdgcn_s_barrier();
             }
             if (n_mine > 0) write_wr();
-            if (n_mine > 1) { pend = next_image(); issue_wr(pend); }
+            if (n_mine > 1) fetch(pend, pend_t);
             __syncthreads();
             for (int s = 0; s < n_max; s++) {
                 if (s < n_mine) ksteps_wr();
                 __syncthreads();
                 if (s < n_mine) {
-                    store_tile(img + cur, I0{});
+                    finish();
                     if (s + 1 < n_mine) {
                         write_wr();
-                        cur = pend;
-                        if (s + 2 < n_mine) { pend = next_image(); issue_wr(pend); }
+                        cur = pend; cur_t = pend_t;
+                        if (s + 2 < n_mine) fetch(pend, pend_t);
                     }
                 }
                 __syncthreads();
@@ -1211,14 +1283,14 @@
     }
 }
 
-template <int STRIDE, int MT, int NT, bool TILE2D, int N2, int PF = 0, int CM = 0, int NWV = 4, int WR = 0, bool PP = false>
+template <int STRIDE, int MT, int NT, bool TILE2D, int N2, int PF = 0, int CM = 0, int NWV = 4, int WR = 0, bool PP = false, bool BAL = false>
 __global__ __launch_bounds__(64 * NWV) __attribute__((amdgpu_waves_per_eu(IRMV_LDS_WAVES))) void conv3x3_lds_kernel(ConvArgs a, const half_t *wl, int tiles_x, int tiles_y, int twc_log2, int a_patch_bytes, int ipw, int batch, int nblocks, int xcd)
 {
     const int wg_tiles = PP ? (tiles_x * tiles_y + 1) / 2 : tiles_x * tiles_y, groups = (batch + ipw - 1) / ipw;
     int rem, grp;
     tile_image(blockIdx.x, wg_tiles * nblocks, groups, xcd & 1, rem, grp);
     const int nblk = rem / wg_tiles, tile = rem - nblk * wg_tiles;
-    conv3x3_lds_body<STRIDE, MT, NT, TILE2D, N2, PF, CM, NWV, WR, PP>(a, wl, tiles_x, tiles_y, twc_log2, a_patch_bytes, ipw, batch, grp * wg_tiles + tile, nblk, wg_tiles * groups, nblocks, (xcd >> 1) & 1);
+    conv3x3_lds_body<STRIDE, MT, NT, TILE2D, N2, PF, CM, NWV, WR, PP, BAL>(a, wl, tiles_x, tiles_y, twc_log2, a_patch_bytes, ipw, batch, grp * wg_tiles + tile, nblk, wg_tiles * groups, nblocks, (xcd >> 1) & 1, xcd & 1);
 }
 
 template <int STRIDE, int MT, int NT>
@@ -1289,6 +1361,17 @@
     const int groups = (l.batch + l.ipw - 1) / l.ipw;
     const int wg_tiles = PP ? (g.tiles_x * g.tiles_y + 1) / 2 : g.tiles_x * g.tiles_y;
     const int nblocks = l.a.cout_pad / (16 * NT);
+    if constexpr (PP && TILE2D && (N2 == 0 || N2 == 4)) {
+        if (l.a.tile_gate && l.a.tgate && nblocks == 1) {
+            static unsigned long long attr_bal = 0;
+            once_per_device(attr_bal, [] {
+                (void)hipFuncSetAttribute(reinterpret_cast<const void *>(conv3x3_lds_kernel<STRIDE, MT, NT, TILE2D, N2, PF, CM, NWV, WR, PP, true>), hipFuncAttributeMaxDynamicSharedMemorySize, 160 * 1024);
+            });
+            hipLaunchKernelGGL((conv3x3_lds_kernel<STRIDE, MT, NT, TILE2D, N2, PF, CM, NWV, WR, PP, true>), dim3(wg_tiles * groups), dim3(64 * NWV), g.bytes, s, l.a,
+                               l.w, g.tiles_x, g.tiles_y, g.twc_log2, g.patch_bytes, l.ipw, l.batch, nblocks, xcd_image_order() | (wres_stagger() << 1));
+            return;
+        }
+    }
     hipLaunchKernelGGL((conv3x3_lds_kernel<STRIDE, MT, NT, TILE2D, N2, PF, CM, NWV, WR, PP>), dim3(wg_tiles * groups * nblocks), dim3(64 * NWV), g.bytes, s, l.a,
                        l.w, g.tiles_x, g.tiles_y, g.twc_log2, g.patch_bytes, l.ipw, l.batch, nblocks, xcd_image_order() | (wres_stagger() << 1));
 }
@@ -1299,6 +1382,13 @@
     LdsGeom g = pp ? lds_geom(a, 1, 2, 4, 4, 2, true) : lds_geom(a, 1, 2, 4, 8, 2);
     if (pp && !g.tile2d) g.bytes = 0;
     return g;
+}
+int conv_wres_pp_blocks(const ConvArgs &a, int stride, TileMaskDesc &d)
+{
+    const LdsGeom g = wres_geom(a, stride, true);
+    if (!g.bytes || !g.tile2d) return 0;
+    d = tile_mask_desc(a.Hout / g.tiles_y, 1 << g.twc_log2, g.tiles_x, 0);
+    return g.tiles_x * g.tiles_y;
 }
 int conv_wres_tiles(const ConvArgs &a, int stride, bool pp)
 {
diff --git a/irmv_detection_amd/csrc/k_kpt.hip b/irmv_detection_amd/csrc/k_kpt.hip
--- a/irmv_detection_amd/csrc/k_kpt.hip
+++ b/irmv_detection_amd/csrc/k_kpt.hip
@@ -14,7 +14,7 @@
 typedef unsigned int u32x4 __attribute__((ext_vector_type(4)));
 }
 
-template <int STEPS>
+template <int STEPS, bool BAL = false>
 __global__ __launch_bounds__(KNT) __attribute__((amdgpu_waves_per_eu(3))) void kpt3_kernel(Kpt3Args a, int batch, int ipw, int xcd)
 {
     extern __shared__ __attribute__((aligned(16))) uint8_t smem[];
@@ -24,61 +24,97 @@
     const int tid = threadIdx.x, lane = tid & 63, wave = tid >> 6;
     const int g = lane >> 4, r = lane & 15;
     const int tiles = a.tiles_x * a.tiles_y, groups = (batch + ipw - 1) / ipw;
+    TileShare sh;
+    if constexpr (BAL) sh.load(a.tmask, a.tmask_stride, batch, lane);
     int tile, grp;
     tile_image(blockIdx.x, tiles, groups, xcd, tile, grp);
     const int img0 = grp * ipw, nimg = min(ipw, batch - img0);
-    const int tyi = tile / a.tiles_x, txi = tile - tyi * a.tiles_x;
-    const int oy0 = tyi * KT, ox0 = txi * KT;
     const int H = a.H, W = a.W;
     constexpr int KSTEPS = STEPS * 18;
 
     int src[KNP];
     static_assert(KNT % 8 == 0 && (KNP - 1) * KNT < K1N * 8, "piece i of a thread: pixel (tid >> 3) + i * KNT / 8, eighth tid & 7; only the last i can fall off the region");
-    const int dstA = (tid >> 3) * 64 + ((tid & 7) >> 2) * KPL + (tid & 3) * 16, dstB = dstA ^ 32;
-    bool odd[KNP];
+    const int dstA = (tid >> 3) * 64 + ((tid & 7) >> 2) * KPL + (tid & 3) * 16;
+    unsigned int odd = 0u;
     const bool last_piece = tid + (KNP - 1) * KNT < K1N * 8;
 #pragma unroll
     for (int i = 0; i < KNP; i++) {
-        const int e = tid + i * KNT, px = e >> 3, q = e & 7;
+        const int e = tid + i * KNT, px = e >> 3;
         const int ly = px / K1W, lx = px - ly * K1W;
-        const int gy = oy0 - 2 + ly, gx = ox0 - 2 + lx;
-        const bool in = e < K1N * 8 && (unsigned)gy < (unsigned)H && (unsigned)gx < (unsigned)W;
-        odd[i] = (ly & 1) != 0;
-        src[i] = in ? (((img0 * H + gy) * W + gx) * a.x_ld + q * 8) * 2 : 0x7fffffff;
-    }
-    const int img_stride = H * W * a.x_ld * 2;
+        odd |= (unsigned int)(ly & 1) << i;
+        (void)lx;
+    }
+    const int ld2 = a.x_ld * 2, img_stride = H * W * ld2;
+    int l_base = 0;
+    auto plan_entry = [&](int im, int t) {
+        const int ty = t / a.tiles_x, tx = t - ty * a.tiles_x;
+        const int py = ty * KT - 2, px = tx * KT - 2;
+        const int org = (py * W + px) * ld2 + (tid & 7) * 16;
+        int pix0 = tid >> 3;
+        if constexpr (BAL) asm volatile("" : "+v"(pix0));
+#pragma unroll
+        for (int i = 0; i < KNP; i++) {
+            const int pix = pix0 + i * (KNT / 8);
+            const int ly = (pix * 4682) >> 16, lx = pix - ly * K1W;
+            static_assert(K1W == 14 && (KNP * KNT / 8) * 4682 < (1 << 23), "pix / 14 as a multiply: exact below 2 ^ 16 / (4682 * 14 - 65536)");
+            const bool in = pix < K1N && (unsigned)(py + ly) < (unsigned)H && (unsigned)(px + lx) < (unsigned)W;
+            src[i] = in ? org + (int)__umul24(__umul24(ly, W) + lx, ld2) : 0x7fffffff;
+        }
+        l_base = im * img_stride;
+    };
     const auto rs_x = __builtin_amdgcn_make_buffer_rsrc(const_cast<half_t *>(a.x), 0, batch * img_stride, 0x00020000);
     const auto rs_w = __builtin_amdgcn_make_buffer_rsrc(const_cast<half_t *>(a.w1), 0, KSTEPS * 1024, 0x00020000);
     auto load_w = [&](int k) { return __builtin_bit_cast(half8, __builtin_amdgcn_raw_buffer_load_b128(rs_w, lane * 16, k * 1024, 0)); };
     u32x4 v[KNP];
     unsigned int amask = nimg >= 32 ? 0xffffffffu : (1u << nimg) - 1u;
-    if (a.tile_gate && a.cand_bits) {
-        const int rows = min(KT, H - oy0), cols = min(KT, W - ox0);
-        const int row = lane >> 1, bl = a.abase + (oy0 + row) * W + ox0, wd = (bl >> 5) + (lane & 1);
-        const int s0 = max(bl - wd * 32, 0), s1 = min(bl + cols - wd * 32, 32);
-        const bool item = row < rows && s1 > s0;
-        const unsigned int bm = item ? (0xffffffffu >> (32 - (s1 - s0))) << s0 : 0u;
-        unsigned int cwd[8];
-#pragma unroll
-        for (int i = 0; i < 8; i++) cwd[i] = i < nimg ? a.cand_bits[(unsigned int)((img0 + i) * a.cand_words + (item ? wd : 0))] : 0u;
-        amask = 0u;
-#pragma unroll
-        for (int i = 0; i < 8; i++) amask |= __ballot((cwd[i] & bm) != 0u) != 0ull ? 1u << i : 0u;
-        amask = __builtin_amdgcn_readfirstlane(amask);
-        if (amask == 0u) return;
-    }
-    int l_im = __builtin_ctz(amask), l_s = 0;
-    unsigned int l_rest = amask & (amask - 1u);
+    int n_ent;
+    if constexpr (BAL) {
+        sh.count(lane);
+        n_ent = sh.begin(share_of_workgroup(blockIdx.x, gridDim.x, xcd), gridDim.x);
+        if (n_ent == 0) return;
+    } else {
+        if (a.tile_gate && a.cand_bits) {
+            const int tyi = tile / a.tiles_x, oy0 = tyi * KT, ox0 = (tile - tyi * a.tiles_x) * KT;
+            const int rows = min(KT, H - oy0), cols = min(KT, W - ox0);
+            const int row = lane >> 1, bl = a.abase + (oy0 + row) * W + ox0, wd = (bl >> 5) + (lane & 1);
+            const int s0 = max(bl - wd * 32, 0), s1 = min(bl + cols - wd * 32, 32);
+            const bool item = row < rows && s1 > s0;
+            const unsigned int bm = item ? (0xffffffffu >> (32 - (s1 - s0))) << s0 : 0u;
+            unsigned int cwd[8];
+#pragma unroll
+            for (int i = 0; i < 8; i++) cwd[i] = i < nimg ? a.cand_bits[(unsigned int)((img0 + i) * a.cand_words + (item ? wd : 0))] : 0u;
+            amask = 0u;
+#pragma unroll
+            for (int i = 0; i < 8; i++) amask |= __ballot((cwd[i] & bm) != 0u) != 0ull ? 1u << i : 0u;
+            amask = __builtin_amdgcn_readfirstlane(amask);
+            if (amask == 0u) return;
+        }
+        n_ent = __builtin_popcount(amask);
+    }
+    int l_ent = 0, l_s = STEPS - 1, l_im = 0, l_t = tile;
+    if constexpr (!BAL) plan_entry(0, tile);
     auto issue_slab = [&]() {
-        const int off = __builtin_amdgcn_readfirstlane(l_im * img_stride + l_s * 128);
+        if (!(l_ent == n_ent && l_s == STEPS - 1)) {
+            if (++l_s == STEPS) {
+                l_s = 0; l_ent++;
+                if constexpr (BAL) {
+                    sh.next(l_im, l_t);
+                    l_im = __builtin_amdgcn_readfirstlane(l_im); l_t = __builtin_amdgcn_readfirstlane(l_t);
+                    plan_entry(l_im, l_t);
+                } else {
+                    l_im = img0 + __builtin_ctz(amask); amask &= amask - 1u;
+                    l_base = l_im * img_stride;
+                }
+            }
+        }
+        const int off = __builtin_amdgcn_readfirstlane(l_base + l_s * 128);
 #pragma unroll
         for (int i = 0; i < KNP; i++) v[i] = __builtin_bit_cast(u32x4, __builtin_amdgcn_raw_buffer_load_b128(rs_x, src[i], off, 0));
-        if (!(l_rest == 0u && l_s == STEPS - 1)) { if (++l_s == STEPS) { l_s = 0; l_im = __builtin_ctz(l_rest); l_rest &= l_rest - 1u; } }
     };
     auto write_slab = [&]() {
 #pragma unroll
         for (int i = 0; i < KNP; i++)
-            if (i + 1 < KNP || last_piece) *reinterpret_cast<u32x4 *>(s_in + (odd[i] ? dstB : dstA) + i * (KNT / 8) * 64) = v[i];
+            if (i + 1 < KNP || last_piece) *reinterpret_cast<u32x4 *>(s_in + (dstA ^ (((odd >> i) & 1u) << 5)) + i * (KNT / 8) * 64) = v[i];
     };
 
     issue_slab();
@@ -117,15 +153,15 @@
         for (int i = 0; i < 3; i++) B[i] = *reinterpret_cast<const half8 *>(s_in + (kh == 1 ? baseO : baseE) + off + i * 256);
     };
 
-    for (unsigned int c_rest = amask; c_rest; c_rest &= c_rest - 1u) {
-        const int im = __builtin_ctz(c_rest);
+    for (int ent = 0; ent < n_ent; ent++) {
+        const int im = l_im, tyi = l_t / a.tiles_x, oy0 = tyi * KT, ox0 = (l_t - tyi * a.tiles_x) * KT;
         unsigned int cw[3];
 #pragma unroll
         for (int i = 0; i < 3; i++) {
             const int gy = oy0 + bly, gx = ox0 + i * 4 + blx;
             const int an = a.abase + ((gy < H && gx < W) ? gy * W + gx : 0);
             const unsigned int *cb = a.cand_bits ? a.cand_bits : reinterpret_cast<const unsigned int *>(a.b3);
-            const unsigned int w = cb[a.cand_bits ? (unsigned int)((img0 + im) * a.cand_words + (an >> 5)) : 0u];
+            const unsigned int w = cb[a.cand_bits ? (unsigned int)(im * a.cand_words + (an >> 5)) : 0u];
             cw[i] = a.cand_bits ? (w >> (an & 31)) & 1u : 1u;
         }
         f32x4 acc[3] = {b1, b1, b1};
@@ -180,28 +216,54 @@
             const f32x4 c2 = __builtin_amdgcn_mfma_f32_16x16x16f16(w3f, o, (f32x4){0.f, 0.f, 0.f, 0.f}, 0, 0, 0);
             const f32x4 v2 = (f32x4){c2[0] * kActUnscale + b3[0], c2[1] * kActUnscale + b3[1], c2[2] * kActUnscale + b3[2], c2[3] * kActUnscale + b3[3]};
             const int gy = oy0 + ly, gx = ox0 + lx;
-            if (valid && gy < H && gx < W && cw[i]) *reinterpret_cast<f32x4 *>(a.out + ((size_t)((img0 + im) * H + gy) * W + gx) * a.out_ld + g * 4) = v2;
-        }
-    }
-}
-
-bool kpt3_eligible(int cin) { return cin == 64 || cin == 128 || cin == 256; }
-
-bool launch_kpt3(const Kpt3Args &a, int cin, int batch, hipStream_t s)
+            if (valid && gy < H && gx < W && cw[i]) *reinterpret_cast<f32x4 *>(a.out + ((size_t)(im * H + gy) * W + gx) * a.out_ld + g * 4) = v2;
+        }
+    }
+}
+
+static void kpt3_grid(const Kpt3Args &a, int batch, int &ipw, dim3 &grid)
 {
     const int tiles = a.tiles_x * a.tiles_y;
-    int ipw = 1;
+    ipw = 1;
     while (ipw < 8 && (long long)tiles * batch >= 2048LL * ipw) ipw *= 2;
-    const dim3 grid(tiles * ((batch + ipw - 1) / ipw)), block(KNT);
-    constexpr size_t lds = (size_t)2 * KPL + (size_t)K2N * KQS + 4608;
-    static_assert(lds <= 40 * 1024, "four workgroups per CU");
+    grid = dim3(tiles * ((batch + ipw - 1) / ipw));
+}
+constexpr size_t kKpt3Lds = (size_t)2 * KPL + (size_t)K2N * KQS + 4608;
+static_assert(kKpt3Lds <= 40 * 1024, "four workgroups per CU");
+
+#ifdef IRMV_KPT3_BALANCED
+bool launch_kpt3_balanced(const Kpt3Args &a, int cin, int batch, hipStream_t s)
+{
+    int ipw;
+    dim3 grid;
+    kpt3_grid(a, batch, ipw, grid);
+    const dim3 block(KNT);
     const int xcd = xcd_image_order();
     switch (cin) {
-    case 64: hipLaunchKernelGGL((kpt3_kernel<1>), grid, block, lds, s, a, batch, ipw, xcd); return true;
-    case 128: hipLaunchKernelGGL((kpt3_kernel<2>), grid, block, lds, s, a, batch, ipw, xcd); return true;
-    case 256: hipLaunchKernelGGL((kpt3_kernel<4>), grid, block, lds, s, a, batch, ipw, xcd); return true;
+    case 64: hipLaunchKernelGGL((kpt3_kernel<1, true>), grid, block, kKpt3Lds, s, a, batch, ipw, xcd); return true;
+    case 128: hipLaunchKernelGGL((kpt3_kernel<2, true>), grid, block, kKpt3Lds, s, a, batch, ipw, xcd); return true;
+    case 256: hipLaunchKernelGGL((kpt3_kernel<4, true>), grid, block, kKpt3Lds, s, a, batch, ipw, xcd); return true;
     default: return false;
     }
 }
-
-}
+#else
+bool kpt3_eligible(int cin) { return cin == 64 || cin == 128 || cin == 256; }
+
+bool launch_kpt3(const Kpt3Args &a, int cin, int batch, hipStream_t s)
+{
+    if (a.tile_gate && a.tmask) return launch_kpt3_balanced(a, cin, batch, s);
+    int ipw;
+    dim3 grid;
+    kpt3_grid(a, batch, ipw, grid);
+    const dim3 block(KNT);
+    const int xcd = xcd_image_order();
+    switch (cin) {
+    case 64: hipLaunchKernelGGL((kpt3_kernel<1>), grid, block, kKpt3Lds, s, a, batch, ipw, xcd); return true;
+    case 128: hipLaunchKernelGGL((kpt3_kernel<2>), grid, block, kKpt3Lds, s, a, batch, ipw, xcd); return true;
+    case 256: hipLaunchKernelGGL((kpt3_kernel<4>), grid, block, kKpt3Lds, s, a, batch, ipw, xcd); return true;
+    default: return false;
+    }
+}
+#endif
+
+}
diff --git a/irmv_detection_amd/csrc/k_kpt_bal.hip b/irmv_detection_amd/csrc/k_kpt_bal.hip
--- /dev/null
+++ b/irmv_detection_amd/csrc/k_kpt_bal.hip
@@ -0,0 +1,2 @@
+#define IRMV_KPT3_BALANCED 1
+#include "k_kpt.hip"
diff --git a/irmv_detection_amd/csrc/k_post.hip b/irmv_detection_amd/csrc/k_post.hip
--- a/irmv_detection_amd/csrc/k_post.hip
+++ b/irmv_detection_amd/csrc/k_post.hip
@@ -361,6 +361,7 @@
         if (tid == 0) { s_ncand = n; a.counts[b] = 0; }
         if (a.cand_bits)
             for (int i = tid; i < a.cand_words; i += blockDim.x) a.cand_bits[(size_t)b * a.cand_words + i] = 0u;
+        if (a.tile_masks && tid < a.tile_mask_words) a.tile_masks[(size_t)b * a.tile_mask_words + tid] = 0ull;
     } else {
     {
         constexpr int U = 8;
diff --git a/irmv_detection_amd/engine.py b/irmv_detection_amd/engine.py
--- a/irmv_detection_amd/engine.py
+++ b/irmv_detection_amd/engine.py
@@ -361,6 +361,21 @@
                                                                  C.byref(n), C.byref(sparse)))
         return bool(sparse.value), words
 
+    def debug_gate_plan(self, count: int):
+        n = C.c_int(0)
+        capi.check(self._L.irmv_engine_debug_gate_plan(self._h, count, None, 0, C.byref(n)))
+        flags = np.zeros(n.value, np.int32)
+        capi.check(self._L.irmv_engine_debug_gate_plan(self._h, count, flags.ctypes.data_as(C.POINTER(C.c_int32)), n.value, C.byref(n)))
+        return [dict(sparse=bool(f & 1), gate=int(f >> 1) & 3, balanced=bool(f & 8)) for f in flags]
+
+    def debug_tile_masks(self, slot: int = 0) -> np.ndarray:
+        n = C.c_int(0)
+        capi.check(self._L.irmv_engine_debug_read_tile_masks(self._h, slot, None, 0, C.byref(n)))
+        masks = np.zeros(n.value, np.uint64)
+        if n.value:
+            capi.check(self._L.irmv_engine_debug_read_tile_masks(self._h, slot, masks.ctypes.data_as(C.POINTER(C.c_uint64)), n.value, C.byref(n)))
+        return masks.reshape(-1, 3)
+
     def debug_head_rows(self, slot: int = 0) -> np.ndarray:
         out = np.empty((self.num_anchors, 96), np.float32)
         capi.check(self._L.irmv_engine_debug_read_head_rows(self._h, slot, out.ctypes.data_as(C.POINTER(C.c_float)), out.nbytes))
```

Result: no change. 65490 (-0.8%).
